# alipay/MMLRec-A-Unified-Multi-Task-and-Multi-Scenario-Learning-Benchmark-for-Recommendation

Hardware: AMD Instinct MI355X
Metric: train-step samples/sec, MMoE AliExpress-shape batch (higher is better)
Workload: dtype f32 (GEMMs: fp32-equivalent emulation on the 16-bit MFMA pipe with f32 accumulate -- two scaled fp16 planes per operand where the operand magnitudes travel with the tensors (batches >= 32 768), else three bf16 planes; max-norm error vs float64 3.3e-7 / 4.7e-7, fp32 MFMA 4.3e-7); 1 GPU; mmoe_ae30: 30 sparse fields, 12.49M rows (1e+07-row top table), E=8, mmoe 4 experts, experts [256, 128], gates [64], towers [64], adam lr 0.005; batch_per_gpu=65536, global_batch=65536, index_dist=zipf, table_update=dense_exact, dense_update_schedule=one launch after the scatter, gradients read for marked rows only, hip_graph=True, scatter_mode=deterministic, streams=1, early_fork=0, tables=single GPU

## Files before the change

include/mmlrec.h:

```cpp
#ifndef MMLREC_H
#define MMLREC_H

#include <stdint.h>

#ifdef __cplusplus
extern "C" {
#endif

#define MML_OK 0
#define MML_ERR_ARG (-1)
#define MML_ERR_HIP (-2)
#define MML_ERR_UNSUPPORTED (-3)

#define MML_MAX_FIELDS 64
#define MML_MAX_GROUP 16
#define MML_MAX_SRC 8
#define MML_MAX_EXPERTS 16
#define MML_MAX_GATES 8
#define MML_MAX_HEADS 8
#define MML_MAX_OPT_TENSORS 32
#define MML_AMAX_WORDS 8
#define MML_MAX_AMAX 64

typedef void* mml_stream_t;
// ... 277 lines not shown
  int64_t ldh, lddh;
  int32_t H;
  int32_t h_relu;
  int32_t n_bias2;
  int32_t mask_col;
  const float* gate;
  float* dgate;
  int64_t ldgate, lddgate;
  int32_t gate_act;
  int32_t kind;
} mml_head_desc;
typedef struct {
  int32_t n_heads;
  int32_t dh_bf16;
  int64_t B;
  float* prob;
  int64_t ldprob;
  const float* y;
  int64_t ldy;
  const float* mask;
  int64_t ldmask;
  float* loss;
  const float* dprob;
  int64_t lddprob;
  mml_head_desc head[MML_MAX_HEADS];
  uint32_t* amax_dH;
  uint32_t* amax_dG;
} mml_head_group;
int64_t mml_head_workspace_bytes(const mml_head_group* grp);
int mml_head_fwd(const mml_head_group* grp, mml_stream_t stream);
int mml_head_bce_fwd_bwd(const mml_head_group* grp, void* workspace, int64_t workspace_bytes, mml_stream_t stream);
int mml_head_bce_fwd_bwd_phase(const mml_head_group* grp, void* workspace, int64_t workspace_bytes, int32_t phase,
                               mml_stream_t stream);
#define MML_ROWS_REDUCE_HEAD 0
#define MML_ROWS_REDUCE_GATE 1
#define MML_ROWS_REDUCE_TOWER_HEAD 2
typedef struct {
  int32_t kind;
  int32_t pad_;
  const void* group;
  void* workspace;
  int64_t workspace_bytes;
} mml_rows_reduce_item;
int mml_rows_reduce_batch(const mml_rows_reduce_item* items, int32_t n, mml_stream_t stream);

typedef struct {
  const float* A;
  int64_t lda;
  const uint32_t* amax_a;
  const uint32_t* w_planes_fwd;
  const uint32_t* w_planes_bwd;
  int64_t ldpf, ldpb;
  const int32_t* kexp_fwd;
  const int32_t* kexp_bwd;
  const float* bias1;
  const float* w;
  const float* hbias;
  const float* hbias2;
  float* dH;
  float* dA;
  int64_t lddh, ldda;
  float* dw;
  float* dhbias;
  uint32_t* amax_dH;
  uint32_t* amax_dA;
  int32_t K, N, n_hbias2;
  int32_t mask_col;
  int32_t head;
  int32_t kind;
} mml_tower_head_desc;
typedef struct {
  int32_t n;
  int32_t pad_;
  int64_t M;
  float* prob;
  int64_t ldprob;
  const float* y;
  int64_t ldy;
  const float* mask;
  int64_t ldmask;
  float* loss;
  mml_tower_head_desc t[MML_MAX_HEADS];
} mml_tower_head_group;
int mml_tower_head_serves(const mml_tower_head_group* grp);
int64_t mml_tower_head_workspace_bytes(const mml_tower_head_group* grp);
int mml_tower_head_fwd_bwd(const mml_tower_head_group* grp, void* workspace, int64_t workspace_bytes, int32_t phase,
                           mml_stream_t stream);


typedef struct {
  const float* src;
  uint16_t* dst;
  int64_t rows, lds, ldd;
  int32_t cols, transpose;
} mml_cast16_desc;
int mml_cast16_batch(const mml_cast16_desc* descs, int32_t n, mml_stream_t stream);
int mml_gather16_fwd(const float* const* tables, const int64_t* vocab, const int32_t* col, int32_t F, int32_t E,
                     const float* X, int64_t ldX, int32_t dense_col0, int32_t Nd, int64_t B, uint16_t* out, int64_t ldo,
                     int32_t* status, mml_stream_t stream);
typedef struct {
  int32_t M, N;
  int32_t n_src;
  int32_t act;
  const uint16_t* A[MML_MAX_SRC];
  const uint16_t* B[MML_MAX_SRC];
  int64_t lda[MML_MAX_SRC], ldb[MML_MAX_SRC];
  int32_t K[MML_MAX_SRC];
  const float* bias;
  void* C;
  int64_t ldc;
  int32_t c_bf16;
  int32_t accumulate;
  uint32_t* mask_out;
  const uint32_t* mask_in;
  int64_t ldmask;
} mml_g16_tn_desc;
int mml_g16_tn(const mml_g16_tn_desc* descs, int32_t n, mml_stream_t stream);
typedef struct {
  const uint16_t* dC;
  const uint16_t* A;
  float* dW;
  float* dbias;
  int64_t lddc, lda, lddw;
  int32_t M, N, K;
  int32_t accumulate;
} mml_g16_wgrad_desc;
int64_t mml_g16_wgrad_workspace_bytes(const mml_g16_wgrad_desc* descs, int32_t n);
int mml_g16_wgrad(const mml_g16_wgrad_desc* descs, int32_t n, void* workspace, int64_t workspace_bytes, int32_t phase,
                  mml_stream_t stream);
const char* mml_g16_last_kernel(void);

int mml_ew_mul(const float* a, const float* b, float* out, int64_t n, mml_stream_t stream);
int mml_ew_mul_bwd(const float* dout, const float* a, const float* b, float* da, float* db, int32_t acc_a,
                   int32_t acc_b, int64_t n, mml_stream_t stream);
int mml_ew_mul_bwd_act(const float* dout, const float* a, const float* b, float* da, float* db, int32_t acc_a,
                       int32_t acc_b, int64_t n, int32_t act_a, int32_t act_b, mml_stream_t stream);
int mml_ew_add_n(const float* const* in, int32_t n_in, float* out, int64_t n, mml_stream_t stream);
#define MML_SUMPROD_TERMS 8
#define MML_SUMPROD_BATCH 16
typedef struct mml_sumprod_desc {
  float* out;
  const float* x[MML_SUMPROD_TERMS];
  const float* y[MML_SUMPROD_TERMS];
  int64_t n;
  int32_t n_terms;
  int32_t accumulate;
  const float* deriv_of;
  int32_t act;
  int32_t pad_;
  uint32_t* amax_out;
} mml_sumprod_desc;
int mml_sumprod_batch(const mml_sumprod_desc* d, int32_t n, mml_stream_t stream);
int mml_dropout(const float* x, int64_t ldx, float* out, int64_t ldo, int64_t rows, int32_t cols, int64_t row0, float p,
                uint64_t seed, uint32_t site, const int32_t* step_dev, int32_t step, int32_t accumulate,
                mml_stream_t stream);
int mml_copy2d(const float* src, int64_t lds, float* dst, int64_t ldd, int64_t rows, int32_t cols, int32_t accumulate,
               mml_stream_t stream);
typedef struct mml_copy2d_desc {
  const float* src;
  int64_t lds;
  float* dst;
  int64_t ldd;
  int64_t rows;
  int32_t cols;
  int32_t accumulate;
  uint32_t* amax_out;
} mml_copy2d_desc;
int mml_copy2d_batch(const mml_copy2d_desc* d, int32_t n, mml_stream_t stream);
int mml_copy_cols(const float* const* src, const int64_t* lds, float* const* dst, const int64_t* ldd,
                  const int32_t* width, int32_t n_seg, int64_t rows, int32_t accumulate, mml_stream_t stream);
int64_t mml_bn_workspace_bytes(int64_t B, int32_t n);
int mml_bn_fwd(const float* z, int64_t ldz, const float* gamma, const float* beta, float* running_mean, float* running_var,
               int64_t* num_batches_tracked, float* mean, float* rstd, float* y, int64_t ldy, int64_t B, int32_t n,
               int32_t act, int32_t training, float eps, float momentum, void* workspace, int64_t workspace_bytes,
               mml_stream_t stream);
int mml_bn_bwd(const float* dy, int64_t lddy, const float* z, int64_t ldz, const float* gamma, const float* mean,
               const float* rstd, float* dz, int64_t lddz, float* dgamma, float* dbeta, int32_t accumulate, int64_t B,
               int32_t n, void* workspace, int64_t workspace_bytes, mml_stream_t stream);
typedef struct mml_prelu_desc {
  const float* z;
  int64_t ldz;
  float* y;
  int64_t ldy;
  int64_t rows;
  int32_t cols;
  int32_t pad_;
  const float* alpha;
  uint32_t* amax_out;
} mml_prelu_desc;
typedef struct mml_prelu_bwd_desc {
  const float* dy;
  int64_t lddy;
  const float* z;
  int64_t ldz;
  float* dz;
  int64_t lddz;
  int64_t rows;
  int32_t cols;
  int32_t pad_;
  const float* alpha;
  float* dalpha;
  int32_t accumulate_dz;
  int32_t accumulate_dalpha;
  uint32_t* amax_out;
} mml_prelu_bwd_desc;
int32_t mml_prelu_max_batch(void);
int mml_prelu_batch_fwd(const mml_prelu_desc* d, int32_t n, mml_stream_t stream);
int64_t mml_prelu_workspace_bytes(int32_t n);
int mml_prelu_batch_bwd(const mml_prelu_bwd_desc* d, int32_t n, void* workspace, int64_t workspace_bytes,
                        mml_stream_t stream);
#define MML_PCGRAD_MAX_TASKS 8
typedef struct mml_pcgrad_seg {
  const float* bank[MML_PCGRAD_MAX_TASKS];
  float* out;
  int64_t rows;
  int64_t ld;
  int32_t cols;
  int32_t pad_;
  const uint8_t* row_marks;
} mml_pcgrad_seg;
int64_t mml_pcgrad_workspace_bytes(const mml_pcgrad_seg* s, int32_t n, int32_t T);
int mml_pcgrad_gram(const mml_pcgrad_seg* s, int32_t n, int32_t T, double* gram, void* workspace,
                    int64_t workspace_bytes, mml_stream_t stream);
int mml_pcgrad_weights(const double* gram, const int32_t* order, int32_t T, float* w, int32_t* fired,
                       mml_stream_t stream);
int mml_pcgrad_combine(const mml_pcgrad_seg* s, int32_t n, int32_t T, const float* w, mml_stream_t stream);
int mml_pcgrad_stash(const mml_pcgrad_seg* s, int32_t n, int32_t clear, mml_stream_t stream);
int mml_domain_bn_update(const float* x, int64_t ldx, const float* mask, int64_t ldm, int64_t B, int32_t n, int32_t D,
                         float* pop_mean, float* pop_var, float decay, mml_stream_t stream);
int mml_domain_bn_eval(const float* x, int64_t ldx, const float* mask, int64_t ldm, const float* pop_mean,
                       const float* pop_var, float* y, int64_t ldy, int64_t B, int32_t n, int32_t D, float eps,
                       mml_stream_t stream);
int mml_snr_gate_weights_fwd(const float* u, const float* alpha, const float* M, float* W, int32_t n_blocks,
                             int64_t block, int32_t zw, float beta, float gamma, float eps, mml_stream_t stream);
int mml_snr_gate_weights_bwd(const float* dW, const float* M, const float* u, const float* alpha, float* du,
                             float* dalpha, int32_t acc_u, int32_t acc_alpha, int32_t n_blocks, int64_t block,
                             int32_t zw, float beta, float gamma, float eps, float* workspace ,
                             mml_stream_t stream);
typedef struct mml_attn2_desc {
  const float* V[2];
  const float* K[2];
  const float* Q[2];
  int64_t ldv[2], ldk[2], ldq[2];
  float* out;
  int64_t ldo;
  float* A;
  const float* dout;
  int64_t lddo;
  float* dV[2];
  float* dK[2];
  float* dQ[2];
  int64_t lddv[2], lddk[2], lddq[2];
  int64_t B;
  int32_t H;
  float sqrt_h;
} mml_attn2_desc;
int mml_attn2_fwd(const mml_attn2_desc* d, mml_stream_t stream);
int mml_attn2_bwd(const mml_attn2_desc* d, mml_stream_t stream);
int mml_esmm_combine(const float* p_raw, int64_t ldr, const float* y, int64_t ldy, const float* d_out, int64_t lddo,
                     float* p_out, int64_t ldo, float* d_raw, int64_t lddr, float* loss, int64_t B, mml_stream_t stream);
int mml_apg_features_fwd(const float* o1, int64_t ldo1, const float* s, int64_t lds, float* z, int64_t ldz, int64_t B,
                         int32_t k, int32_t E, int32_t Kf, mml_stream_t stream);
int mml_apg_features_bwd(const float* dz, int64_t lddz, const float* s, int64_t lds, float* do1, int64_t lddo1,
                         int64_t B, int32_t k, int32_t E, int32_t accumulate, mml_stream_t stream);
int mml_apg_weights(float* Wkk, float* bkk, float* Wb, float* Wcat, int64_t ldw, int32_t k, int32_t E, int32_t dir,
                    int32_t acc_kk, int32_t acc_bkk, int32_t acc_wb, mml_stream_t stream);
int mml_escm_combine(const float* p_raw, int64_t ldr, const float* y, int64_t ldy, const float* d_out, int64_t lddo,
                     float* p_out, int64_t ldo, float* d_raw, int64_t lddr, float* loss, int64_t B, float cf_w,
                     float global_w, mml_stream_t stream);
int mml_auc_segments(const float* pred, int64_t ldp, const float* y, int64_t ldy, int64_t n, int32_t cols, int32_t seg,
                     double* auc, mml_stream_t stream);
int32_t mml_auc_sorted_tile(void);
int64_t mml_auc_sorted_workspace_bytes(int64_t n, int32_t cols, int64_t seg);
int mml_auc_sorted(const float* pred, int64_t ldp, const float* y, int64_t ldy, const float* mask, int64_t ldm,
                   int32_t mask_cols, int64_t n, int32_t cols, int64_t seg, void* workspace, int64_t workspace_bytes,
                   double* auc, int64_t* counts, int32_t* status, mml_stream_t stream);
int mml_act_bwd(const float* y, const float* dy, float* dst, int64_t n, int32_t act, mml_stream_t stream);

typedef struct {
  float* param; const float* grad;
  float* state1;
  float* state2;
  int64_t n;
  float l1, l2;
  const uint32_t* skip_rows;
  int32_t row_elems;
  int32_t zero_grads;
  uint8_t* grad_marks;
  int64_t* acc64;
  const uint32_t* acc_amax;
  int32_t acc_shift;
  int32_t acc_pad_;
  uint8_t* warm_rows;
} mml_opt_tensor;
typedef struct {
  int32_t kind;
  int32_t step;
  const int32_t* step_dev;
  float lr, beta1, beta2, eps, alpha;
  int32_t zero_grad;
  int32_t max_blocks;
  int32_t cold_loop;
} mml_opt_hyper;
int mml_opt_step_dense(const mml_opt_tensor* tensors, int32_t n, const mml_opt_hyper* hyper, mml_stream_t stream);
int mml_opt_step_rows(float* const* tables, float* const* grad_tables, float* const* state1, float* const* state2,
                      uint32_t* const* seen, const int64_t* rowbase, int32_t F, int32_t E,
                      const int32_t* touched, const int32_t* touched_count, int32_t touched_cap,
                      int32_t* const* last ,
                      const mml_opt_hyper* hyper, mml_stream_t stream);
int mml_opt_catchup_rows(float* const* tables, float* const* state1, float* const* state2, int32_t* const* last,
                         const int64_t* rowbase, int32_t F, int32_t E, const int32_t* touched,
                         const int32_t* touched_count, int32_t touched_cap, const mml_opt_hyper* hyper,
                         mml_stream_t stream);
int mml_opt_catchup_dense(float* table, float* state1, float* state2, int32_t* last, int64_t V, int32_t E,
                          const mml_opt_hyper* hyper, mml_stream_t stream);
int mml_counter_update(int32_t* counter, int32_t delta, int32_t reset, mml_stream_t stream);

#ifdef __cplusplus
}
#endif
#endif
```

mmlrec-a-unified-multi-task-and-multi-scenario-learning-benchmark-for-recommendation_amd/_lib.py:

```python
import ctypes as C
import os

import torch

from . import build as _build

MAX_FIELDS, MAX_GROUP, MAX_SRC, MAX_EXPERTS, MAX_GATES, MAX_HEADS, MAX_OPT_TENSORS = 64, 16, 8, 16, 8, 8, 32
OPT_STREAM_MIN_PARAMS, OPT_HUGE_MIN_PARAMS, OPT_STREAM_MAX_TENSORS = 1 << 24, 1 << 22, 4
MAX_POOLED, POOL_MAX_LEN = 16, 256
POOL_COMBINERS = {"sum": 0, "mean": 1, "max": 2}
ACT_NONE, ACT_RELU, ACT_SIGMOID, ACT_SIGMOID2 = 0, 1, 2, 3
HEAD_OUT_SIGMOID, HEAD_OUT_IDENTITY = 0, 1
HEAD_LOSS_BCE, HEAD_LOSS_MSE, HEAD_LOSS_MAE = 0, 1, 2


def head_kind(out=HEAD_OUT_SIGMOID, loss=HEAD_LOSS_BCE):
    return (int(loss) << 8) | int(out)


ERR_ARG = -1
SCATTER_DET_CLEAR_MARKS, SCATTER_DET_AMAX_SUPPLIED, SCATTER_DET_DEFER_TOTALS = 1, 2, 4
OPT_SGD, OPT_ADAM, OPT_ADAGRAD, OPT_RMSPROP = 0, 1, 2, 3
OPT_KINDS = {"sgd": OPT_SGD, "adam": OPT_ADAM, "adagrad": OPT_ADAGRAD, "rmsprop": OPT_RMSPROP}

fp = C.c_void_p
i32, i64 = C.c_int32, C.c_int64


class GemmFwdDesc(C.Structure):
    _fields_ = [("A", fp), ("W", fp), ("bias", fp), ("C", fp), ("lda", i64), ("ldw", i64), ("ldc", i64),
                ("M", i32), ("N", i32), ("K", i32), ("act", i32), ("w_kn", i32), ("pad_", i32),
                ("relu_mask", fp), ("ldmask", i64), ("amax_a", fp), ("amax_w", fp), ("amax_out", fp),
                ("w_planes", fp), ("w_kexp", fp),
                ("mul", fp), ("prod", fp), ("ldmul", i64), ("ldprod", i64), ("amax_prod", fp)]


class PoolDesc(C.Structure):
    _fields_ = [("n_tables", i32), ("E", i32), ("n_single", i32), ("n_pooled", i32),
                ("table", fp * MAX_FIELDS), ("vocab", i64 * MAX_FIELDS), ("s_col", i32 * MAX_FIELDS),
                ("s_table", i32 * MAX_FIELDS), ("p_col0", i32 * MAX_POOLED), ("p_maxlen", i32 * MAX_POOLED),
                ("p_len_col", i32 * MAX_POOLED), ("p_combiner", i32 * MAX_POOLED), ("p_table", i32 * MAX_POOLED)]


class AmaxDesc(C.Structure):
    _fields_ = [("x", fp), ("rows", i64), ("ld", i64), ("cols", i32), ("pad_", i32), ("slot", fp)]


class GemmDgradDesc(C.Structure):
    _fields_ = [("dA", fp), ("Y", fp), ("ldda", i64), ("ldy", i64), ("M", i32), ("K", i32), ("act", i32),
                ("n_src", i32), ("accumulate", i32), ("pad_", i32),
                ("dC", fp * MAX_SRC), ("W", fp * MAX_SRC), ("lddc", i64 * MAX_SRC), ("ldw", i64 * MAX_SRC),
                ("N", i32 * MAX_SRC), ("w_kn", i32 * MAX_SRC), ("relu_mask", fp), ("ldmask", i64),
                ("amax_dc", fp * MAX_SRC), ("amax_w", fp * MAX_SRC), ("amax_out", fp),
                ("w_planes", fp * MAX_SRC), ("w_kexp", fp * MAX_SRC),
                ("gate_h", fp), ("gate_g", fp), ("d_h", fp), ("d_g", fp),
                ("ld_h", i64), ("ld_g", i64), ("ld_dh", i64), ("ld_dg", i64),
                ("act_h", i32), ("act_g", i32), ("acc_h", i32), ("acc_g", i32), ("amax_dh", fp), ("amax_dg", fp)]


class PlanesDesc(C.Structure):
    _fields_ = [("W", fp), ("planes", fp), ("rows", i64), ("ld", i64), ("cols", i32), ("layout", i32),
                ("n_amax", i32), ("pad_", i32), ("amax", fp * MAX_SRC), ("kexp", fp), ("ldp", i64),
                ("W2", fp), ("ld2", i64)]


class GemmWgradDesc(C.Structure):
    _fields_ = [("dC", fp), ("A", fp), ("dW", fp), ("dbias", fp), ("lddc", i64), ("lda", i64), ("lddw", i64),
                ("M", i32), ("N", i32), ("K", i32), ("accumulate", i32), ("w_kn", i32), ("pad_", i32),
                ("amax_dc", fp), ("amax_a", fp)]


class Cast16Desc(C.Structure):
    _fields_ = [("src", fp), ("dst", fp), ("rows", i64), ("lds", i64), ("ldd", i64), ("cols", i32), ("transpose", i32)]


class G16TnDesc(C.Structure):
    _fields_ = [("M", i32), ("N", i32), ("n_src", i32), ("act", i32), ("A", fp * MAX_SRC), ("B", fp * MAX_SRC),
                ("lda", i64 * MAX_SRC), ("ldb", i64 * MAX_SRC), ("K", i32 * MAX_SRC), ("bias", fp), ("C", fp),
                ("ldc", i64), ("c_bf16", i32), ("accumulate", i32), ("mask_out", fp), ("mask_in", fp), ("ldmask", i64)]


class G16WgradDesc(C.Structure):
    _fields_ = [("dC", fp), ("A", fp), ("dW", fp), ("dbias", fp), ("lddc", i64), ("lda", i64), ("lddw", i64),
                ("M", i32), ("N", i32), ("K", i32), ("accumulate", i32)]


G16_MAX_GROUP = 8


class RowsReduceItem(C.Structure):
    _fields_ = [("kind", i32), ("pad_", i32), ("group", fp), ("workspace", fp), ("workspace_bytes", i64)]


ROWS_REDUCE_HEAD, ROWS_REDUCE_GATE, ROWS_REDUCE_TOWER_HEAD = 0, 1, 2
MAX_REDUCE_SEGS = 40
NT_MAX_GROUP = 48
GATE_MIX_BF16, GATE_DE_BF16, GATE_DG_BF16, GATE_E_BF16 = 1, 2, 4, 8


class GateDesc(C.Structure):
    _fields_ = [("G", fp), ("Wg", fp), ("P", fp), ("mix", fp), ("dmix", fp), ("dG", fp), ("dWg", fp),
                ("ldg", i64), ("ldp", i64), ("ldmix", i64), ("lddmix", i64), ("lddg", i64),
                ("Gd", i32), ("ne", i32), ("g_relu", i32), ("active", i32), ("expert", i32 * MAX_EXPERTS)]


class GateGroup(C.Structure):
    _fields_ = [("E", fp * MAX_EXPERTS), ("dE", fp * MAX_EXPERTS), ("lde", i64 * MAX_EXPERTS),
                ("ldde", i64 * MAX_EXPERTS), ("n_experts", i32), ("n_gates", i32), ("H", i32), ("e_relu", i32),
                ("B", i64), ("gate", GateDesc * MAX_GATES), ("amax_mix", fp), ("amax_dE", fp), ("amax_dG", fp),
                ("out_bf16", i32), ("pad_", i32)]


class HeadDesc(C.Structure):
    _fields_ = [("Hin", fp), ("w", fp), ("w2", fp), ("bias", fp), ("bias2", fp), ("dH", fp), ("dw", fp),
                ("dbias", fp), ("ldh", i64), ("lddh", i64), ("H", i32), ("h_relu", i32), ("n_bias2", i32),
                ("mask_col", i32), ("gate", fp), ("dgate", fp), ("ldgate", i64), ("lddgate", i64),
                ("gate_act", i32), ("kind", i32)]


class HeadGroup(C.Structure):
    _fields_ = [("n_heads", i32), ("dh_bf16", i32), ("B", i64), ("prob", fp), ("ldprob", i64), ("y", fp),
                ("ldy", i64), ("mask", fp), ("ldmask", i64), ("loss", fp), ("dprob", fp), ("lddprob", i64),
                ("head", HeadDesc * MAX_HEADS), ("amax_dH", fp), ("amax_dG", fp)]


class TowerHeadDesc(C.Structure):
    _fields_ = [("A", fp), ("lda", i64), ("amax_a", fp), ("w_planes_fwd", fp), ("w_planes_bwd", fp), ("ldpf", i64),
                ("ldpb", i64), ("kexp_fwd", fp), ("kexp_bwd", fp), ("bias1", fp), ("w", fp), ("hbias", fp),
                ("hbias2", fp), ("dH", fp), ("dA", fp), ("lddh", i64), ("ldda", i64), ("dw", fp), ("dhbias", fp),
                ("amax_dH", fp), ("amax_dA", fp), ("K", i32), ("N", i32), ("n_hbias2", i32), ("mask_col", i32),
                ("head", i32), ("kind", i32)]


class TowerHeadGroup(C.Structure):
    _fields_ = [("n", i32), ("pad_", i32), ("M", i64), ("prob", fp), ("ldprob", i64), ("y", fp), ("ldy", i64),
                ("mask", fp), ("ldmask", i64), ("loss", fp), ("t", TowerHeadDesc * MAX_HEADS)]


class OptTensor(C.Structure):
    _fields_ = [("param", fp), ("grad", fp), ("state1", fp), ("state2", fp), ("n", i64), ("l1", C.c_float),
                ("l2", C.c_float), ("skip_rows", fp), ("row_elems", i32), ("zero_grads", i32), ("grad_marks", fp),
                ("acc64", fp), ("acc_amax", fp), ("acc_shift", i32), ("acc_pad_", i32), ("warm_rows", fp)]


class Copy2dDesc(C.Structure):
    _fields_ = [("src", fp), ("lds", i64), ("dst", fp), ("ldd", i64), ("rows", i64), ("cols", i32),
                ("accumulate", i32), ("amax_out", fp)]


class PreluDesc(C.Structure):
    _fields_ = [("z", fp), ("ldz", i64), ("y", fp), ("ldy", i64), ("rows", i64), ("cols", i32), ("pad_", i32),
                ("alpha", fp), ("amax_out", fp)]


class PreluBwdDesc(C.Structure):
    _fields_ = [("dy", fp), ("lddy", i64), ("z", fp), ("ldz", i64), ("dz", fp), ("lddz", i64), ("rows", i64),
                ("cols", i32), ("pad_", i32), ("alpha", fp), ("dalpha", fp), ("accumulate_dz", i32),
                ("accumulate_dalpha", i32), ("amax_out", fp)]


PCGRAD_MAX_TASKS = 8


class PcgradSeg(C.Structure):
    _fields_ = [("bank", fp * PCGRAD_MAX_TASKS), ("out", fp), ("rows", i64), ("ld", i64), ("cols", i32), ("pad_", i32),
                ("row_marks", fp)]


class SumProdDesc(C.Structure):
    _fields_ = [("out", fp), ("x", fp * 8), ("y", fp * 8), ("n", i64), ("n_terms", i32), ("accumulate", i32),
                ("deriv_of", fp), ("act", i32), ("pad_", i32), ("amax_out", fp)]


class Attn2Desc(C.Structure):
    _fields_ = [("V", fp * 2), ("K", fp * 2), ("Q", fp * 2), ("ldv", i64 * 2), ("ldk", i64 * 2), ("ldq", i64 * 2),
                ("out", fp), ("ldo", i64), ("A", fp), ("dout", fp), ("lddo", i64), ("dV", fp * 2), ("dK", fp * 2),
                ("dQ", fp * 2), ("lddv", i64 * 2), ("lddk", i64 * 2), ("lddq", i64 * 2), ("B", i64), ("H", i32),
                ("sqrt_h", C.c_float)]


class OptHyper(C.Structure):
    _fields_ = [("kind", i32), ("step", i32), ("step_dev", fp), ("lr", C.c_float), ("beta1", C.c_float),
                ("beta2", C.c_float), ("eps", C.c_float), ("alpha", C.c_float), ("zero_grad", i32), ("max_blocks", i32),
                ("cold_loop", i32)]


_PP = C.POINTER
_SIGS = {
    "mml_version": (C.c_int, []),
    "mml_last_error": (C.c_char_p, []),
    "mml_device_caps": (C.c_int, [C.c_int, _PP(i64)]),
    "mml_stream_create_cu_range": (C.c_int, [C.c_int, C.c_int, C.c_int, _PP(C.c_void_p)]),
    "mml_stream_destroy": (C.c_int, [C.c_void_p]),
    "mml_gather_fwd": (C.c_int, [_PP(fp), _PP(i64), _PP(i32), i32, i32, fp, i64, i32, i32, i64, fp, i64, fp, fp]),
    "mml_gather_wgmax_len": (i64, [i32, i32, i32, i64]),
    "mml_gather_fwd_wgmax": (C.c_int, [_PP(fp), _PP(i64), _PP(i32), i32, i32, fp, i64, i32, i32, i64, fp, i64, fp, i64, fp, fp]),
    "mml_gather_fwd_mark": (C.c_int, [_PP(fp), _PP(i64), _PP(i32), i32, i32, fp, i64, i32, i32, i64, fp, i64, fp, fp, fp]),
    "mml_rows_compact": (C.c_int, [_PP(fp), _PP(i64), _PP(i64), i32, fp, fp, i32, fp, fp]),
    "mml_gather_fwd_idx32": (C.c_int, [_PP(fp), _PP(i64), i32, i32, fp, i64, fp, i64, i32, i64, fp, i64, fp, fp]),
    "mml_scatter_bwd": (C.c_int, [_PP(fp), _PP(i64), _PP(i32), i32, i32, fp, i64, i64, fp, i64, _PP(fp), _PP(i64),
                                  fp, fp, i32, fp, fp, fp]),
    "mml_scatter_bwd_det": (C.c_int, [_PP(fp), _PP(i64), _PP(i32), i32, i32, fp, i64, i64, fp, i64, _PP(fp), fp, fp, i32,
                                      fp, fp]),
    "mml_scatter_det_shift": (i32, [i64]),
    "mml_scatter_bwd_idx32": (C.c_int, [_PP(fp), _PP(i64), i32, i32, fp, i64, i64, fp, i64, _PP(fp), _PP(i64),
                                        fp, fp, i32, fp, fp, fp]),
    "mml_index_unique_idx32": (C.c_int, [_PP(i64), i32, i32, fp, i64, i64, _PP(fp), _PP(i64), fp, fp, i32, fp, fp, fp]),
    "mml_route_count": (C.c_int, [fp, i64, fp, i64, _PP(i32), _PP(i64), i32, i64, i32, fp, fp, fp]),
    "mml_route_place": (C.c_int, [fp, i64, fp, i64, _PP(i32), _PP(i64), _PP(i64), i32, i64, i32, fp, fp, fp, fp, fp]),
    "mml_rows_permute": (C.c_int, [fp, i64, fp, i32, i32, i64, fp, fp]),
    "mml_route_list_count": (C.c_int, [fp, fp, i32, _PP(i64), _PP(i64), i32, i32, fp, fp]),
    "mml_route_list_place": (C.c_int, [fp, fp, i32, _PP(i64), _PP(i64), _PP(i64), i32, i32, fp, fp, fp, fp]),
    "mml_lookup_slots": (C.c_int, [fp, i64, _PP(i32), _PP(i64), _PP(i64), i32, i64, fp, fp, fp, fp]),
    "mml_rows_clear": (C.c_int, [fp, fp, i32, _PP(i64), _PP(fp), i32, fp]),
    "mml_shard_rows": (C.c_int, [fp, i64, fp, i64, i32, i32, i32, i32, fp]),
    "mml_amax_batch": (C.c_int, [_PP(AmaxDesc), i32, fp]),
    "mml_amax_reset": (C.c_int, [fp, i64, fp]),
    "mml_gemm_planes_cut": (C.c_int, [C.POINTER(PlanesDesc), i32, fp]),
    "mml_gemm_set_mode": (C.c_int, [i32]),
    "mml_gemm_get_mode": (C.c_int, []),
    "mml_gemm_set_panel": (C.c_int, [i32]),
    "mml_gemm_set_ws": (C.c_int, [i32]),
    "mml_gemm_set_nt": (C.c_int, [i32]),
    "mml_gemm_nt_serves": (C.c_int, [_PP(GemmWgradDesc)]),
    "mml_gemm_os_serves": (C.c_int, [_PP(GemmDgradDesc), i32]),
    "mml_tower_head_serves": (C.c_int, [_PP(TowerHeadGroup)]),
    "mml_tower_head_workspace_bytes": (i64, [_PP(TowerHeadGroup)]),
    "mml_tower_head_fwd_bwd": (C.c_int, [_PP(TowerHeadGroup), fp, i64, i32, fp]),
    "mml_gemm_last_kernel": (C.c_char_p, []),
    "mml_gather_last_kernel": (C.c_char_p, []),
    "mml_gemm_set_wgrad_lds_pad": (C.c_int, [i32]),
    "mml_cast16_batch": (C.c_int, [_PP(Cast16Desc), i32, fp]),
    "mml_gather16_fwd": (C.c_int, [_PP(fp), _PP(i64), _PP(i32), i32, i32, fp, i64, i32, i32, i64, fp, i64, fp, fp]),
    "mml_g16_tn": (C.c_int, [_PP(G16TnDesc), i32, fp]),
    "mml_g16_wgrad_workspace_bytes": (i64, [_PP(G16WgradDesc), i32]),
    "mml_g16_wgrad": (C.c_int, [_PP(G16WgradDesc), i32, fp, i64, i32, fp]),
    "mml_g16_last_kernel": (C.c_char_p, []),
    "mml_gemm_grouped_fwd": (C.c_int, [_PP(GemmFwdDesc), i32, fp]),
    "mml_gemm_grouped_dgrad": (C.c_int, [_PP(GemmDgradDesc), i32, fp]),
    "mml_pep_gate_fwd": (C.c_int, [_PP(GemmFwdDesc), i32, fp]),
    "mml_pep_gate_bwd": (C.c_int, [_PP(GemmDgradDesc), i32, fp]),
    "mml_star_linear_fwd": (C.c_int, [_PP(GemmFwdDesc), i32, fp]),
    "mml_star_linear_bwd": (C.c_int, [_PP(GemmDgradDesc), i32, fp]),
    "mml_gemm_grouped_wgrad_workspace_bytes": (i64, [_PP(GemmWgradDesc), i32]),
    "mml_gemm_grouped_wgrad": (C.c_int, [_PP(GemmWgradDesc), i32, fp, i64, fp]),
    "mml_gemm_grouped_wgrad_phase": (C.c_int, [_PP(GemmWgradDesc), i32, fp, i64, i32, fp]),
    "mml_gate_mix_fwd": (C.c_int, [_PP(GateGroup), fp]),
    "mml_gate_mix_bwd_workspace_bytes": (i64, [_PP(GateGroup)]),
    "mml_gate_mix_bwd": (C.c_int, [_PP(GateGroup), fp, i64, fp]),
    "mml_gate_mix_bwd_phase": (C.c_int, [_PP(GateGroup), fp, i64, i32, fp]),
    "mml_head_workspace_bytes": (i64, [_PP(HeadGroup)]),
    "mml_head_fwd": (C.c_int, [_PP(HeadGroup), fp]),
    "mml_head_bce_fwd_bwd": (C.c_int, [_PP(HeadGroup), fp, i64, fp]),
    "mml_head_bce_fwd_bwd_phase": (C.c_int, [_PP(HeadGroup), fp, i64, i32, fp]),
    "mml_rows_reduce_batch": (C.c_int, [_PP(RowsReduceItem), i32, fp]),
    "mml_ew_mul": (C.c_int, [fp, fp, fp, i64, fp]),
    "mml_ew_mul_bwd": (C.c_int, [fp, fp, fp, fp, fp, i32, i32, i64, fp]),
    "mml_ew_mul_bwd_act": (C.c_int, [fp, fp, fp, fp, fp, i32, i32, i64, i32, i32, fp]),
    "mml_ew_add_n": (C.c_int, [_PP(fp), i32, fp, i64, fp]),
    "mml_sumprod_batch": (C.c_int, [_PP(SumProdDesc), i32, fp]),
    "mml_copy2d": (C.c_int, [fp, i64, fp, i64, i64, i32, i32, fp]),
    "mml_dropout": (C.c_int, [fp, i64, fp, i64, i64, i32, i64, C.c_float, C.c_uint64, C.c_uint32, fp, i32, i32, fp]),
    "mml_copy2d_batch": (C.c_int, [_PP(Copy2dDesc), i32, fp]),
    "mml_prelu_max_batch": (i32, []),
    "mml_prelu_batch_fwd": (C.c_int, [_PP(PreluDesc), i32, fp]),
    "mml_prelu_workspace_bytes": (i64, [i32]),
    "mml_prelu_batch_bwd": (C.c_int, [_PP(PreluBwdDesc), i32, fp, i64, fp]),
    "mml_pcgrad_workspace_bytes": (i64, [_PP(PcgradSeg), i32, i32]),
    "mml_pcgrad_gram": (C.c_int, [_PP(PcgradSeg), i32, i32, fp, fp, i64, fp]),
    "mml_pcgrad_weights": (C.c_int, [fp, fp, i32, fp, fp, fp]),
    "mml_pcgrad_combine": (C.c_int, [_PP(PcgradSeg), i32, i32, fp, fp]),
    "mml_pcgrad_stash": (C.c_int, [_PP(PcgradSeg), i32, i32, fp]),
    "mml_auc_segments": (C.c_int, [fp, i64, fp, i64, i64, i32, i32, fp, fp]),
    "mml_auc_sorted_tile": (i32, []),
    "mml_auc_sorted_workspace_bytes": (i64, [i64, i32, i64]),
    "mml_auc_sorted": (C.c_int, [fp, i64, fp, i64, fp, i64, i32, i64, i32, i64, fp, i64, fp, fp, fp, fp]),
    "mml_bn_workspace_bytes": (C.c_int64, [i64, i32]),
    "mml_bn_fwd": (C.c_int, [fp, i64, fp, fp, fp, fp, fp, fp, fp, fp, i64, i64, i32, i32, i32, C.c_float, C.c_float, fp,
                             i64, fp]),
    "mml_bn_bwd": (C.c_int, [fp, i64, fp, i64, fp, fp, fp, fp, i64, fp, fp, i32, i64, i32, fp, i64, fp]),
    "mml_domain_bn_update": (C.c_int, [fp, i64, fp, i64, i64, i32, i32, fp, fp, C.c_float, fp]),
    "mml_domain_bn_eval": (C.c_int, [fp, i64, fp, i64, fp, fp, fp, i64, i64, i32, i32, C.c_float, fp]),
    "mml_snr_gate_weights_fwd": (C.c_int, [fp, fp, fp, fp, i32, i64, i32, C.c_float, C.c_float, C.c_float, fp]),
    "mml_snr_gate_weights_bwd": (C.c_int, [fp, fp, fp, fp, fp, fp, i32, i32, i32, i64, i32, C.c_float, C.c_float,
                                           C.c_float, fp, fp]),
    "mml_attn2_fwd": (C.c_int, [_PP(Attn2Desc), fp]),
    "mml_attn2_bwd": (C.c_int, [_PP(Attn2Desc), fp]),
    "mml_esmm_combine": (C.c_int, [fp, i64, fp, i64, fp, i64, fp, i64, fp, i64, fp, i64, fp]),
    "mml_apg_features_fwd": (C.c_int, [fp, i64, fp, i64, fp, i64, i64, i32, i32, i32, fp]),
    "mml_apg_features_bwd": (C.c_int, [fp, i64, fp, i64, fp, i64, i64, i32, i32, i32, fp]),
    "mml_apg_weights": (C.c_int, [fp, fp, fp, fp, i64, i32, i32, i32, i32, i32, i32, fp]),
    "mml_escm_combine": (C.c_int, [fp, i64, fp, i64, fp, i64, fp, i64, fp, i64, fp, i64, C.c_float, C.c_float, fp]),
    "mml_act_bwd": (C.c_int, [fp, fp, fp, i64, i32, fp]),
    "mml_copy_cols": (C.c_int, [_PP(fp), _PP(i64), _PP(fp), _PP(i64), _PP(i32), i32, i64, i32, fp]),
    "mml_opt_step_dense": (C.c_int, [_PP(OptTensor), i32, _PP(OptHyper), fp]),
    "mml_opt_step_rows": (C.c_int, [_PP(fp), _PP(fp), _PP(fp), _PP(fp), _PP(fp), _PP(i64), i32, i32, fp, fp, i32,
                                    _PP(fp), _PP(OptHyper), fp]),
    "mml_opt_catchup_rows": (C.c_int, [_PP(fp), _PP(fp), _PP(fp), _PP(fp), _PP(i64), i32, i32, fp, fp, i32,
                                       _PP(OptHyper), fp]),
    "mml_opt_catchup_dense": (C.c_int, [fp, fp, fp, fp, i64, i32, _PP(OptHyper), fp]),
    "mml_index_unique": (C.c_int, [_PP(i64), _PP(i32), i32, i32, fp, i64, i64, _PP(fp), _PP(i64), fp, fp, i32, fp, fp,
                                   fp]),
    "mml_counter_update": (C.c_int, [fp, i32, i32, fp]),
    "mml_gather_pool_wgmax_len": (i64, [_PP(PoolDesc), i32, i64]),
    "mml_gather_pool_fwd": (C.c_int, [_PP(PoolDesc), fp, i64, i32, i32, i64, fp, i64, fp, i64, fp, i64, fp, fp]),
    "mml_scatter_pool_bwd": (C.c_int, [_PP(PoolDesc), fp, i64, i64, fp, i64, fp, i64, _PP(fp), _PP(i64), fp, fp, i32,
                                       fp, fp, fp]),
    "mml_index_unique_pool": (C.c_int, [_PP(PoolDesc), fp, i64, i64, _PP(fp), _PP(i64), fp, fp, i32, fp, fp, fp]),
}
EXPORTS = tuple(_SIGS)

_lib = None


class MMLError(RuntimeError):
    pass


def library_path():
    return _build.LIBPATH


def load():
    global _lib
    if _lib is not None:
        return _lib
    path = os.environ.get("MMLREC_LIB") or _build.LIBPATH
    if path == _build.LIBPATH and (not os.path.exists(path) or _build.needs_build()) and os.path.exists(_build.HIPCC):
        _build.build_library(verbose=False)
    if not os.path.exists(path):
        raise MMLError(f"HIP extension {path} is missing and cannot be built (no hipcc): the MI355X path has no "
                       "CPU fallback")
    lib = C.CDLL(path)
    for name, (res, args) in _SIGS.items():
        fn = getattr(lib, name)
        fn.restype = res
        fn.argtypes = args
    _lib = lib
    return lib


def check(rc, what=""):
    if rc != 0:
        msg = load().mml_last_error()
        raise MMLError(f"{what} failed with code {rc}: {msg.decode() if msg else ''}")


def ptr(t):
    return None if t is None else t.data_ptr()


def opt_dense_streams(numel, ntensors, all_marked):
    return numel >= OPT_STREAM_MIN_PARAMS and (ntensors <= OPT_STREAM_MAX_TENSORS or all_marked)


def opt_takes_det_totals(numels, all_marked, split=False):
    return (all_marked and not split and len(numels) <= MAX_OPT_TENSORS and
            opt_dense_streams(sum(numels), len(numels), True))
```

mmlrec-a-unified-multi-task-and-multi-scenario-learning-benchmark-for-recommendation_amd/csrc/optim_ew.hip:

```cpp
#include "common.hpp"
#include "fold_fixed.hpp"

#include <stdlib.h>

#ifndef MML_OPT_COLD_CB
#define MML_OPT_COLD_CB 8
#endif

namespace mml {

struct OptLaunch {
  mml_opt_tensor t[MML_MAX_OPT_TENSORS];
  int32_t n;
  int32_t variant;
  mml_opt_hyper h;
  int64_t chunk0[MML_MAX_OPT_TENSORS + 1];
  int32_t blk0[MML_MAX_OPT_TENSORS + 1];
  int32_t prop;
};
static_assert(sizeof(OptLaunch) <= 4096, "OptLaunch travels by value: the kernel-argument block holds 4 KB");

struct StepConsts {
  float step_size;
  float inv_bc2s;
};

__device__ __forceinline__ StepConsts step_consts(const mml_opt_hyper& h) {
  __shared__ StepConsts sc;
  if (threadIdx.x == 0) {
    StepConsts c{h.lr, 1.f};
    if (h.kind == MML_OPT_ADAM) {
      const int t = h.step_dev ? *h.step_dev : h.step;
      const double bc1 = 1.0 - pow((double)h.beta1, (double)t);
      const double bc2 = 1.0 - pow((double)h.beta2, (double)t);
      c.step_size = (float)((double)h.lr / bc1);
      c.inv_bc2s = (float)(1.0 / sqrt(bc2));
    }
    sc = c;
  }
  __syncthreads();
  return sc;
}

__device__ __forceinline__ void opt_update(const mml_opt_hyper& h, const StepConsts& c, float& p, float g, float& s1,
                                           float& s2) {
  switch (h.kind) {
    case MML_OPT_SGD:
      p -= h.lr * g;
      break;
    case MML_OPT_ADAM: {
      s1 = s1 + (1.f - h.beta1) * (g - s1);
      s2 = h.beta2 * s2 + (1.f - h.beta2) * g * g;
      const float denom = sqrtf(s2) * c.inv_bc2s + h.eps;
      p -= c.step_size * (s1 / denom);
      break;
    }
    case MML_OPT_ADAGRAD:
      s1 += g * g;
      p -= h.lr * (g / (sqrtf(s1) + h.eps));
      break;
    case MML_OPT_RMSPROP:
      s1 = h.alpha * s1 + (1.f - h.alpha) * g * g;
      p -= h.lr * (g / (sqrtf(s1) + h.eps));
      break;
  }
}

__device__ __forceinline__ float reg_grad(float g, float p, float l1, float l2) {
  if (l2 != 0.f) g += (2.f * l2) * p;
  if (l1 != 0.f) g += l1 * (p > 0.f ? 1.f : (p < 0.f ? -1.f : 0.f));
  return g;
}

enum { OPT_PLAIN = 0, OPT_UNROLL2 = 1, OPT_SKIP_U = 2, OPT_MARK_U = 3, OPT_MARK_ACC_U = 4 };
template <bool STREAM, int PATH, int U>
__global__ __launch_bounds__(256) void opt_dense_kernel(const OptLaunch L) {
  int ti = blockIdx.y, nblk = gridDim.x, lblk = blockIdx.x;
  if (L.prop) {
    ti = 0;
    while (ti + 1 < L.n && (int)blockIdx.x >= L.blk0[ti + 1]) ++ti;
    nblk = L.blk0[ti + 1] - L.blk0[ti];
    lblk = (int)blockIdx.x - L.blk0[ti];
  }
  const mml_opt_tensor& T = L.t[ti];
  const mml_opt_hyper& h = L.h;
  const StepConsts c = step_consts(h);
  const int64_t n4 = T.n >> 2;
  const bool vec = aligned16(T.param) && aligned16(T.grad) && (!T.state1 || aligned16(T.state1)) &&
                   (!T.state2 || aligned16(T.state2));
  const int64_t stride = (int64_t)nblk * blockDim.x;
  const int64_t tid = (int64_t)lblk * blockDim.x + threadIdx.x;
  float* gw = const_cast<float*>(T.grad);
  const bool reg = T.l1 != 0.f || T.l2 != 0.f;
  if (vec) {
    typedef float f4 __attribute__((ext_vector_type(4)));
    const bool nt = (L.variant & 1) != 0;
    f4* P = reinterpret_cast<f4*>(T.param);
    f4* G = reinterpret_cast<f4*>(gw);
    f4* S1 = reinterpret_cast<f4*>(T.state1);
    f4* S2 = reinterpret_cast<f4*>(T.state2);
    const f4 zero = {0.f, 0.f, 0.f, 0.f};
    auto ld = [&](const f4* q) { return nt ? __builtin_nontemporal_load(q) : *q; };
    auto st = [&](f4* q, const f4& v) {
      if (nt) __builtin_nontemporal_store(v, q);
      else *q = v;
    };
    auto one = [&](f4& p, const f4& g, f4& a, f4& b) {
#pragma unroll
      for (int e = 0; e < 4; ++e) {
        float pe = p[e], ae = a[e], be = b[e];
        opt_update(h, c, pe, reg ? reg_grad(g[e], pe, T.l1, T.l2) : g[e], ae, be);
        p[e] = pe;
        a[e] = ae;
        b[e] = be;
      }
    };
    const uint32_t* skip = T.skip_rows;
    const int re = T.row_elems > 0 ? T.row_elems : 1;
    const int rsh = (re & (re - 1)) == 0 ? __builtin_ctz((unsigned)re) : -1;
    auto row_of = [&](int64_t c) { return rsh >= 0 ? ((c << 2) >> rsh) : ((c << 2) / re); };
    auto skipped = [&](int64_t c) {
      const int64_t row = row_of(c);
      return (skip[row >> 5] >> (row & 31)) & 1u;
    };
    const bool zg = T.zero_grads != 0;
    uint8_t* const gm = T.grad_marks;
    typedef long long l2 __attribute__((ext_vector_type(2)));
    l2* const A64 = PATH == OPT_MARK_ACC_U ? reinterpret_cast<l2*>(T.acc64) : nullptr;
    const l2 lzero = {0, 0};
    int emax = 1;
    if (PATH == OPT_MARK_ACC_U && A64) {
      uint32_t m = 0;
      for (int w = 0; w < MML_AMAX_WORDS; ++w) m = T.acc_amax[w] > m ? T.acc_amax[w] : m;
      emax = (int)(m >> 23);
      emax = emax < 1 ? 1 : (emax > 254 ? 254 : emax);
    }
    auto add_totals = [&](f4& g, const l2& t0, const l2& t1, int64_t c) {
      if (t0.x) g.x += from_fixed(t0.x, emax, T.acc_shift);
      if (t0.y) g.y += from_fixed(t0.y, emax, T.acc_shift);
      if (t1.x) g.z += from_fixed(t1.x, emax, T.acc_shift);
      if (t1.y) g.w += from_fixed(t1.y, emax, T.acc_shift);
      if (t0.x | t0.y) A64[2 * c] = lzero;
      if (t1.x | t1.y) A64[2 * c + 1] = lzero;
    };
    int64_t i = tid;
    if (PATH == OPT_UNROLL2 && !skip && !gm) {
      for (; i + stride < n4; i += 2 * stride) {
        const int64_t j = i + stride;
        f4 p0 = ld(P + i), p1 = ld(P + j);
        const f4 g0 = ld(G + i), g1 = ld(G + j);
        f4 a0 = S1 ? ld(S1 + i) : zero, a1 = S1 ? ld(S1 + j) : zero;
        f4 b0 = S2 ? ld(S2 + i) : zero, b1 = S2 ? ld(S2 + j) : zero;
        one(p0, g0, a0, b0);
        one(p1, g1, a1, b1);
        st(P + i, p0);
        st(P + j, p1);
        if (S1) { st(S1 + i, a0); st(S1 + j, a1); }
        if (S2) { st(S2 + i, b0); st(S2 + j, b1); }
        if (h.zero_grad && (g0.x != 0.f || g0.y != 0.f || g0.z != 0.f || g0.w != 0.f)) G[i] = zero;
        if (h.zero_grad && (g1.x != 0.f || g1.y != 0.f || g1.z != 0.f || g1.w != 0.f)) G[j] = zero;
      }
    }
    if (PATH == OPT_SKIP_U && skip) {
      for (; i + (U - 1) * stride < n4; i += U * stride) {
        f4 p[U], a[U], b[U];
        uint32_t w[U];
#pragma unroll
        for (int k = 0; k < U; ++k) {
          const int64_t row = row_of(i + k * stride);
          w[k] = (skip[row >> 5] >> (row & 31)) & 1u;
        }
#pragma unroll
        for (int k = 0; k < U; ++k) {
          const int64_t j = i + k * stride;
          if (!w[k]) {
            p[k] = ld(P + j);
            a[k] = S1 ? ld(S1 + j) : zero;
            b[k] = S2 ? ld(S2 + j) : zero;
          }
        }
#pragma unroll
        for (int k = 0; k < U; ++k) {
          if (w[k]) continue;
          const int64_t j = i + k * stride;
          const f4 g = zg ? zero : ld(G + j);
          one(p[k], g, a[k], b[k]);
          st(P + j, p[k]);
          if (S1) st(S1 + j, a[k]);
          if (S2) st(S2 + j, b[k]);
          if (h.zero_grad && (g.x != 0.f || g.y != 0.f || g.z != 0.f || g.w != 0.f)) G[j] = zero;
        }
      }
    }
    uint8_t* const wr = gm ? T.warm_rows : nullptr;
    const bool compact = !(L.variant & 8) && wr &&
                         ((reinterpret_cast<uintptr_t>(gm) | reinterpret_cast<uintptr_t>(wr)) & 3) == 0;
    if ((PATH == OPT_MARK_U || PATH == OPT_MARK_ACC_U) && compact && !skip) {
      constexpr int RPL = 4, SPAN = 64 * RPL;
      constexpr int DENSE_PCT = 15;
      constexpr int WAVES = 4;
      __shared__ uint16_t live_rows[WAVES][SPAN];
      const int lane = threadIdx.x & 63;
      const int wv = __builtin_amdgcn_readfirstlane((int)(threadIdx.x >> 6));
      uint16_t* const lst = live_rows[wv];
      const int csh = rsh - 2;
      const int64_t rows = T.n >> rsh;
      const int64_t nspan = (rows + SPAN - 1) / SPAN, nwv = (int64_t)nblk * WAVES;
      auto nz80 = [](uint32_t x) { return (x | ((x & 0x7f7f7f7fu) + 0x7f7f7f7fu)) & 0x80808080u; };
      auto pack4 = [](uint32_t t) { return ((t >> 7) & 1u) | ((t >> 14) & 2u) | ((t >> 21) & 4u) | ((t >> 28) & 8u); };
      auto scan = [&](int64_t s, uint32_t& mk, uint32_t& wk) {
        const int64_t r0 = s * SPAN + lane * RPL;
        mk = wk = 0u;
        if (r0 + RPL <= rows) {
          mk = *reinterpret_cast<const uint32_t*>(gm + r0);
          wk = *reinterpret_cast<const uint32_t*>(wr + r0);
        } else {
#pragma unroll
          for (int k = 0; k < RPL; ++k)
            if (r0 + k < rows) {
              mk |= (uint32_t)gm[r0 + k] << (8 * k);
              wk |= (uint32_t)wr[r0 + k] << (8 * k);
            }
        }
      };
      int64_t s = (int64_t)lblk * WAVES + wv;
      uint32_t mk = 0, wk = 0;
      if (s < nspan) scan(s, mk, wk);
      for (; s < nspan; s += nwv) {
        uint32_t mkn = 0, wkn = 0;
        if (s + nwv < nspan) scan(s + nwv, mkn, wkn);
        const uint32_t lm = pack4(nz80(mk)), wm = pack4(nz80(wk));
        const uint32_t act = lm | wm;
        if (__builtin_amdgcn_ballot_w64(act != 0) != 0) {
          const int64_t row0 = s * SPAN;
          const uint32_t cnt = (uint32_t)__builtin_popcount(act);
          uint32_t pre = 0;
          int nlive = 0;
#pragma unroll
          for (int bit = 0; (1 << bit) <= RPL; ++bit) {
            const uint64_t bal = __builtin_amdgcn_ballot_w64(((cnt >> bit) & 1u) != 0);
            pre += __builtin_amdgcn_mbcnt_hi((uint32_t)(bal >> 32), __builtin_amdgcn_mbcnt_lo((uint32_t)bal, 0u)) << bit;
            nlive += __builtin_popcountll(bal) << bit;
          }
          const bool dense = nlive * 100 >= SPAN * DENSE_PCT;
          if (!dense) {
            __builtin_amdgcn_fence(__ATOMIC_RELEASE, "wavefront");
            __builtin_amdgcn_wave_barrier();
#pragma unroll
            for (int k = 0; k < RPL; ++k)
              if ((act >> k) & 1u)
                lst[pre++] = (uint16_t)((lane * RPL + k) | (((lm >> k) & 1u) << 14) | (((wm >> k) & 1u) << 15));
            __builtin_amdgcn_fence(__ATOMIC_RELEASE, "wavefront");
            __builtin_amdgcn_wave_barrier();
          }
          if (lm) {
            const int64_t r0 = row0 + lane * RPL;
            if (r0 + RPL <= rows) {
              *reinterpret_cast<uint32_t*>(gm + r0) = 0u;
              const uint32_t set = (nz80(mk) & ~nz80(wk)) >> 7;
              if (set) *reinterpret_cast<uint32_t*>(wr + r0) = wk | set;
            } else {
#pragma unroll
              for (int k = 0; k < RPL; ++k)
                if ((lm >> k) & 1u) {
                  gm[r0 + k] = 0;
                  if (!((wm >> k) & 1u)) wr[r0 + k] = 1;
                }
            }
          }
          const int items = (dense ? SPAN : nlive) << csh;
#pragma unroll 1
          for (int b0 = 0; b0 < items; b0 += 128) {
            f4 p[2], a[2], b[2], g[2];
            l2 t0[2], t1[2];
            int64_t jj[2];
            bool on[2], lv[2];
#pragma unroll
            for (int k = 0; k < 2; ++k) {
              const int it = b0 + 64 * k + lane;
              const int ent = it >> csh;
              on[k] = it < items;
              uint32_t e;
              if (dense) {
                const uint32_t src = (uint32_t)__shfl((int)(lm | (act << 16)), (ent / RPL) & 63);
                on[k] = on[k] && ((src >> (16 + (ent & (RPL - 1)))) & 1u);
                e = (uint32_t)ent | (((src >> (ent & (RPL - 1))) & 1u) << 14);
              } else {
                e = on[k] ? lst[ent] : 0u;
              }
              lv[k] = on[k] && ((e >> 14) & 1u);
              const int64_t j = ((row0 + (int64_t)(e & 0x3fffu)) << csh) | (int64_t)(it & ((1 << csh) - 1));
              jj[k] = j;
              p[k] = a[k] = b[k] = g[k] = zero;
              t0[k] = t1[k] = lzero;
              if (on[k]) {
                p[k] = ld(P + j);
                if (S1) a[k] = ld(S1 + j);
                if (S2) b[k] = ld(S2 + j);
              }
              if (lv[k]) {
                if (!zg) g[k] = ld(G + j);
                if (PATH == OPT_MARK_ACC_U && A64) {
                  t0[k] = A64[2 * j];
                  t1[k] = A64[2 * j + 1];
                }
              }
            }
#pragma unroll
            for (int k = 0; k < 2; ++k) {
              if (!on[k]) continue;
              const int64_t j = jj[k];
              f4 gs = g[k];
              if (PATH == OPT_MARK_ACC_U && A64 && lv[k]) add_totals(gs, t0[k], t1[k], j);
              one(p[k], gs, a[k], b[k]);
              st(P + j, p[k]);
              if (S1) st(S1 + j, a[k]);
              if (S2) st(S2 + j, b[k]);
              if (h.zero_grad && (g[k].x != 0.f || g[k].y != 0.f || g[k].z != 0.f || g[k].w != 0.f)) G[j] = zero;
            }
          }
        }
        mk = mkn;
        wk = wkn;
      }
      i = n4;
    }
    if ((PATH == OPT_MARK_U || PATH == OPT_MARK_ACC_U) && wr && !skip && !compact) {
      constexpr int CB = MML_OPT_COLD_CB;
      for (; i < n4; i += CB * stride) {
        uint32_t lm = 0, wm = 0;
#pragma unroll
        for (int k = 0; k < CB; ++k) {
          const int64_t j = i + k * stride;
          const bool in = j < n4;
          const int64_t row = row_of(in ? j : i);
          const uint8_t mk = gm[row], wk = wr[row];
          lm |= (uint32_t)(in && mk != 0) << k;
          wm |= (uint32_t)(in && wk != 0) << k;
        }
        const uint32_t act = lm | wm;
        if (__builtin_amdgcn_ballot_w64(act != 0) == 0) continue;
#pragma unroll 1
        for (int kk = 0; kk < CB; kk += 2) {
          if (__builtin_amdgcn_ballot_w64(((act >> kk) & 3u) != 0) == 0) continue;
          f4 p[2], a[2], b[2], g[2];
          l2 t0[2], t1[2];
#pragma unroll
          for (int k = 0; k < 2; ++k) {
            const int64_t j = i + (kk + k) * stride;
            const bool on = (act >> (kk + k)) & 1u, lv = (lm >> (kk + k)) & 1u;
            p[k] = a[k] = b[k] = g[k] = zero;
            t0[k] = t1[k] = lzero;
            if (on) {
              p[k] = ld(P + j);
              if (S1) a[k] = ld(S1 + j);
              if (S2) b[k] = ld(S2 + j);
            }
            if (lv) {
              if (!zg) g[k] = ld(G + j);
              if (PATH == OPT_MARK_ACC_U && A64) {
                t0[k] = A64[2 * j];
                t1[k] = A64[2 * j + 1];
              }
            }
          }
#pragma unroll
          for (int k = 0; k < 2; ++k) {
            const int64_t j = i + (kk + k) * stride;
            const bool on = (act >> (kk + k)) & 1u, lv = (lm >> (kk + k)) & 1u;
            if (!on) continue;
            f4 gs = g[k];
            if (PATH == OPT_MARK_ACC_U && A64 && lv) add_totals(gs, t0[k], t1[k], j);
            one(p[k], gs, a[k], b[k]);
            st(P + j, p[k]);
            if (S1) st(S1 + j, a[k]);
            if (S2) st(S2 + j, b[k]);
            if (h.zero_grad && (g[k].x != 0.f || g[k].y != 0.f || g[k].z != 0.f || g[k].w != 0.f)) G[j] = zero;
            const int64_t row = row_of(j);
            if (lv && (j << 2) == row * re) {
              gm[row] = 0;
              if (!((wm >> (kk + k)) & 1u)) wr[row] = 1;
            }
          }
        }
      }
    }
    if (PATH == OPT_MARK_U && gm && !skip) {
      for (; i + (U - 1) * stride < n4; i += U * stride) {
        f4 p[U], a[U], b[U], g[U];
        bool lv[U];
        int64_t rw[U];
#pragma unroll
        for (int k = 0; k < U; ++k) {
          rw[k] = row_of(i + k * stride);
          lv[k] = gm[rw[k]] != 0;
        }
#pragma unroll
        for (int k = 0; k < U; ++k) {
          const int64_t j = i + k * stride;
          p[k] = ld(P + j);
          a[k] = S1 ? ld(S1 + j) : zero;
          b[k] = S2 ? ld(S2 + j) : zero;
          g[k] = (zg || !lv[k]) ? zero : ld(G + j);
        }
#pragma unroll
        for (int k = 0; k < U; ++k) {
          const int64_t j = i + k * stride;
          one(p[k], g[k], a[k], b[k]);
          st(P + j, p[k]);
          if (S1) st(S1 + j, a[k]);
          if (S2) st(S2 + j, b[k]);
          if (h.zero_grad && (g[k].x != 0.f || g[k].y != 0.f || g[k].z != 0.f || g[k].w != 0.f)) G[j] = zero;
          if (lv[k] && (j << 2) == rw[k] * re) gm[rw[k]] = 0;
        }
      }
    }
    if (PATH == OPT_MARK_ACC_U && gm && !skip) {
      for (; i + (U - 1) * stride < n4; i += U * stride) {
        f4 p[U], a[U], b[U], g[U];
        l2 t0[U], t1[U];
        bool lv[U];
        int64_t rw[U];
#pragma unroll
        for (int k = 0; k < U; ++k) {
          rw[k] = row_of(i + k * stride);
          lv[k] = gm[rw[k]] != 0;
        }
#pragma unroll
        for (int k = 0; k < U; ++k) {
          const int64_t j = i + k * stride;
          p[k] = ld(P + j);
          a[k] = S1 ? ld(S1 + j) : zero;
          b[k] = S2 ? ld(S2 + j) : zero;
          g[k] = (zg || !lv[k]) ? zero : ld(G + j);
          t0[k] = (A64 && lv[k]) ? A64[2 * j] : lzero;
          t1[k] = (A64 && lv[k]) ? A64[2 * j + 1] : lzero;
        }
#pragma unroll
        for (int k = 0; k < U; ++k) {
          const int64_t j = i + k * stride;
          f4 gs = g[k];
          if (A64 && lv[k]) add_totals(gs, t0[k], t1[k], j);
          one(p[k], gs, a[k], b[k]);
          st(P + j, p[k]);
          if (S1) st(S1 + j, a[k]);
          if (S2) st(S2 + j, b[k]);
          if (h.zero_grad && (g[k].x != 0.f || g[k].y != 0.f || g[k].z != 0.f || g[k].w != 0.f)) G[j] = zero;
          if (lv[k] && (j << 2) == rw[k] * re) gm[rw[k]] = 0;
        }
      }
    }
    for (; i < n4; i += stride) {
      if (skip && skipped(i)) continue;
      bool live = true, warm = true;
      int64_t row = 0;
      if (gm) {
        row = row_of(i);
        live = gm[row] != 0;
        if (wr) {
          warm = wr[row] != 0;
          if (!live && !warm) continue;
        }
      }
      f4 p = ld(P + i);
      const f4 g = (zg || !live) ? zero : ld(G + i);
      f4 a = S1 ? ld(S1 + i) : zero;
      f4 b = S2 ? ld(S2 + i) : zero;
      if (PATH == OPT_MARK_ACC_U) {
        f4 gs = g;
        if (A64 && gm && live) add_totals(gs, A64[2 * i], A64[2 * i + 1], i);
        one(p, gs, a, b);
      } else {
        one(p, g, a, b);
      }
      st(P + i, p);
      if (S1) st(S1 + i, a);
      if (S2) st(S2 + i, b);
      if (h.zero_grad && (g.x != 0.f || g.y != 0.f || g.z != 0.f || g.w != 0.f)) G[i] = zero;
      if (gm && live && (i << 2) == row * re) {
        gm[row] = 0;
        if (!warm) wr[row] = 1;
      }
    }
  }
  const int64_t tail0 = vec ? (n4 << 2) : 0;
  for (int64_t i = tail0 + tid; i < T.n; i += stride) {
    if (T.skip_rows) {
      const int64_t row = i / (T.row_elems > 0 ? T.row_elems : 1);
      if ((T.skip_rows[row >> 5] >> (row & 31)) & 1u) continue;
    }
    float p = T.param[i], a = T.state1 ? T.state1[i] : 0.f, b = T.state2 ? T.state2[i] : 0.f;
    opt_update(h, c, p, reg_grad(T.zero_grads ? 0.f : T.grad[i], p, T.l1, T.l2), a, b);
    T.param[i] = p;
    if (T.state1) T.state1[i] = a;
    if (T.state2) T.state2[i] = b;
    if (h.zero_grad && T.grad[i] != 0.f) gw[i] = 0.f;
  }
}

__global__ __launch_bounds__(256) void opt_flat_kernel(const OptLaunch L) {
  __shared__ mml_opt_tensor ts[MML_MAX_OPT_TENSORS];
  __shared__ int64_t pre[MML_MAX_OPT_TENSORS + 1];
  for (int i = threadIdx.x; i < L.n; i += 256) ts[i] = L.t[i];
  for (int i = threadIdx.x; i <= L.n; i += 256) pre[i] = L.chunk0[i];
  const mml_opt_hyper& h = L.h;
  const StepConsts c = step_consts(h);
  const int64_t total = pre[L.n];
  const int64_t stride = (int64_t)gridDim.x * blockDim.x;
  for (int64_t ch = (int64_t)blockIdx.x * blockDim.x + threadIdx.x; ch < total; ch += stride) {
    int lo = 0, hi = L.n;
    while (hi - lo > 1) {
      const int mid = (lo + hi) >> 1;
      if (pre[mid] <= ch) lo = mid;
      else hi = mid;
    }
    const mml_opt_tensor T = ts[lo];
    const int64_t e0 = (ch - pre[lo]) << 2;
    float* gw = const_cast<float*>(T.grad);
    const int re = T.row_elems > 0 ? T.row_elems : 1;
    if (T.skip_rows && re % 4 == 0) {
      const int64_t row = e0 / re;
      if ((T.skip_rows[row >> 5] >> (row & 31)) & 1u) continue;
    }
    const bool vec = (e0 + 4 <= T.n) && aligned16(T.param) && aligned16(T.grad) && (!T.state1 || aligned16(T.state1)) &&
                     (!T.state2 || aligned16(T.state2));
    if (vec) {
      float4 p = *reinterpret_cast<float4*>(T.param + e0);
      const float4 g = T.zero_grads ? make_float4(0, 0, 0, 0) : *reinterpret_cast<const float4*>(T.grad + e0);
      float4 a = T.state1 ? *reinterpret_cast<float4*>(T.state1 + e0) : make_float4(0, 0, 0, 0);
      float4 b = T.state2 ? *reinterpret_cast<float4*>(T.state2 + e0) : make_float4(0, 0, 0, 0);
      opt_update(h, c, p.x, reg_grad(g.x, p.x, T.l1, T.l2), a.x, b.x);
      opt_update(h, c, p.y, reg_grad(g.y, p.y, T.l1, T.l2), a.y, b.y);
      opt_update(h, c, p.z, reg_grad(g.z, p.z, T.l1, T.l2), a.z, b.z);
      opt_update(h, c, p.w, reg_grad(g.w, p.w, T.l1, T.l2), a.w, b.w);
      *reinterpret_cast<float4*>(T.param + e0) = p;
      if (T.state1) *reinterpret_cast<float4*>(T.state1 + e0) = a;
      if (T.state2) *reinterpret_cast<float4*>(T.state2 + e0) = b;
      if (h.zero_grad && (g.x != 0.f || g.y != 0.f || g.z != 0.f || g.w != 0.f))
        *reinterpret_cast<float4*>(gw + e0) = make_float4(0, 0, 0, 0);
    } else {
      for (int64_t i = e0; i < e0 + 4 && i < T.n; ++i) {
        if (T.skip_rows) {
          const int64_t row = i / re;
          if ((T.skip_rows[row >> 5] >> (row & 31)) & 1u) continue;
        }
        float p = T.param[i], a = T.state1 ? T.state1[i] : 0.f, b = T.state2 ? T.state2[i] : 0.f;
        const float g = T.zero_grads ? 0.f : T.grad[i];
        opt_update(h, c, p, reg_grad(g, p, T.l1, T.l2), a, b);
        T.param[i] = p;
        if (T.state1) T.state1[i] = a;
        if (T.state2) T.state2[i] = b;
        if (h.zero_grad && g != 0.f) gw[i] = 0.f;
      }
    }
  }
}

struct RowsLaunch {
  float* tab[MML_MAX_FIELDS];
  float* grad[MML_MAX_FIELDS];
  float* s1[MML_MAX_FIELDS];
  float* s2[MML_MAX_FIELDS];
  uint32_t* seen[MML_MAX_FIELDS];
  int64_t rowbase[MML_MAX_FIELDS + 1];
  int32_t F, E;
  int32_t* last[MML_MAX_FIELDS];
  const int32_t* touched;
  const int32_t* touched_count;
  int32_t cap;
  int32_t pad_;
  mml_opt_hyper h;
};

__device__ __forceinline__ int field_of_row(const int64_t* rb_lds, int F, int64_t grow) {
  int lo = 0, hi = F;
  while (hi - lo > 1) {
    const int mid = (lo + hi) >> 1;
    if (rb_lds[mid] <= grow) lo = mid;
    else hi = mid;
  }
  return lo;
}

template <int VEC>
__global__ __launch_bounds__(256) void opt_rows_kernel(const RowsLaunch L) {
  const mml_opt_hyper& h = L.h;
  __shared__ int64_t rb_lds[MML_MAX_FIELDS + 1];
  __shared__ float* tab_l[MML_MAX_FIELDS];
  __shared__ float* grad_l[MML_MAX_FIELDS];
  __shared__ float* s1_l[MML_MAX_FIELDS];
  __shared__ float* s2_l[MML_MAX_FIELDS];
  __shared__ uint32_t* seen_l[MML_MAX_FIELDS];
  __shared__ int32_t* last_l[MML_MAX_FIELDS];
  for (int i = threadIdx.x; i <= L.F; i += 256) rb_lds[i] = L.rowbase[i];
  for (int i = threadIdx.x; i < L.F; i += 256) {
    tab_l[i] = L.tab[i]; grad_l[i] = L.grad[i]; s1_l[i] = L.s1[i]; s2_l[i] = L.s2[i]; seen_l[i] = L.seen[i];
    last_l[i] = L.last[i];
  }
  const StepConsts c = step_consts(h);
  int32_t cnt = *L.touched_count;
  if (cnt > L.cap) cnt = L.cap;
  const int per_row = L.E / VEC;
  const int64_t total = (int64_t)cnt * per_row;
  const int64_t stride = (int64_t)gridDim.x * blockDim.x;
  for (int64_t item = (int64_t)blockIdx.x * blockDim.x + threadIdx.x; item < total; item += stride) {
    const int32_t li = (int32_t)(item / per_row);
    const int e = (int)(item - (int64_t)li * per_row) * VEC;
    const int64_t grow = L.touched[li];
    const int f = field_of_row(rb_lds, L.F, grow);
    const int64_t row = grow - rb_lds[f];
    const int64_t o = row * L.E + e;
    float* const T_ = tab_l[f];
    float* const G_ = grad_l[f];
    float* const S1 = s1_l[f];
    float* const S2 = s2_l[f];
    float p[VEC], g[VEC], a[VEC], b[VEC];
    if (VEC == 4) {
      *reinterpret_cast<float4*>(p) = *reinterpret_cast<const float4*>(T_ + o);
      *reinterpret_cast<float4*>(g) = *reinterpret_cast<const float4*>(G_ + o);
      if (S1) *reinterpret_cast<float4*>(a) = *reinterpret_cast<const float4*>(S1 + o);
      if (S2) *reinterpret_cast<float4*>(b) = *reinterpret_cast<const float4*>(S2 + o);
    } else {
      p[0] = T_[o];
      g[0] = G_[o];
      if (S1) a[0] = S1[o];
      if (S2) b[0] = S2[o];
    }
#pragma unroll
    for (int k = 0; k < VEC; ++k) {
      if (!S1) a[k] = 0.f;
      if (!S2) b[k] = 0.f;
      opt_update(h, c, p[k], g[k], a[k], b[k]);
    }
    if (VEC == 4) {
      *reinterpret_cast<float4*>(T_ + o) = *reinterpret_cast<float4*>(p);
      if (S1) *reinterpret_cast<float4*>(S1 + o) = *reinterpret_cast<float4*>(a);
      if (S2) *reinterpret_cast<float4*>(S2 + o) = *reinterpret_cast<float4*>(b);
      *reinterpret_cast<float4*>(G_ + o) = make_float4(0.f, 0.f, 0.f, 0.f);
    } else {
      T_[o] = p[0];
      if (S1) S1[o] = a[0];
      if (S2) S2[o] = b[0];
      G_[o] = 0.f;
    }
    if (e == 0) {
      atomicAnd(seen_l[f] + (row >> 5), ~(1u << (row & 31)));
      if (last_l[f]) last_l[f][row] = h.step_dev ? *h.step_dev : h.step;
    }
  }
}

__device__ __forceinline__ void catchup_element(const mml_opt_hyper& h, int from, int to, float& p, float& m, float& v) {
  if (to <= from) return;
  if (h.kind == MML_OPT_ADAM) {
    if (m == 0.f) {
      v *= powf(h.beta2, (float)(to - from));
      return;
    }
    float b1p = powf(h.beta1, (float)from), b2p = powf(h.beta2, (float)from);
    int j = from;
    while (j < to) {
      ++j;
      b1p *= h.beta1;
      b2p *= h.beta2;
      StepConsts c;
      c.step_size = h.lr / (1.f - b1p);
      c.inv_bc2s = rsqrtf(1.f - b2p);
      const float before = p;
      opt_update(h, c, p, 0.f, m, v);
      if (p == before && j - from > 16) {
        const float rem = (float)(to - j);
        m *= powf(h.beta1, rem);
        v *= powf(h.beta2, rem);
        return;
      }
    }
  } else if (h.kind == MML_OPT_RMSPROP) {
    m *= powf(h.alpha, (float)(to - from));
  }
}

struct CatchupLaunch {
  float* tab[MML_MAX_FIELDS];
  float* s1[MML_MAX_FIELDS];
  float* s2[MML_MAX_FIELDS];
  int32_t* last[MML_MAX_FIELDS];
  int64_t rowbase[MML_MAX_FIELDS + 1];
  int32_t F, E;
  const int32_t* touched;
  const int32_t* touched_count;
  int32_t cap;
  int32_t dense;
  int64_t V;
  mml_opt_hyper h;
};

__global__ __launch_bounds__(256) void opt_catchup_kernel(const CatchupLaunch L) {
  __shared__ int64_t rb_lds[MML_MAX_FIELDS + 1];
  if (!L.dense) {
    for (int i = threadIdx.x; i <= L.F; i += 256) rb_lds[i] = L.rowbase[i];
    __syncthreads();
  }
  const mml_opt_hyper& h = L.h;
  const int target = (h.step_dev ? *h.step_dev : h.step) - (L.dense ? 0 : 1);
  int64_t nrows;
  if (L.dense) {
    nrows = L.V;
  } else {
    int32_t cnt = *L.touched_count;
    nrows = cnt > L.cap ? L.cap : cnt;
  }
  const int64_t total = nrows * L.E;
  const int64_t stride = (int64_t)gridDim.x * blockDim.x;
  for (int64_t item = (int64_t)blockIdx.x * blockDim.x + threadIdx.x; item < total; item += stride) {
    const int64_t li = item / L.E;
    const int e = (int)(item - li * L.E);
    int f = 0;
    int64_t row = li;
    if (!L.dense) {
      const int64_t grow = L.touched[li];
      f = field_of_row(rb_lds, L.F, grow);
      row = grow - rb_lds[f];
    }
    const int from = L.last[f][row];
    if (from >= target) continue;
    const int64_t o = row * L.E + e;
    float p = L.tab[f][o];
    float m = L.s1[f] ? L.s1[f][o] : 0.f, v = L.s2[f] ? L.s2[f][o] : 0.f;
    catchup_element(h, from, target, p, m, v);
    L.tab[f][o] = p;
    if (L.s1[f]) L.s1[f][o] = m;
    if (L.s2[f]) L.s2[f][o] = v;
    __builtin_amdgcn_wave_barrier();
    if (e == 0) L.last[f][row] = target;
  }
}

__global__ void counter_kernel(int32_t* c, int32_t delta, int32_t reset) {
  if (threadIdx.x == 0 && blockIdx.x == 0) *c = reset ? 0 : (*c + delta);
}

__global__ __launch_bounds__(256) void ew_mul_kernel(const float* a, const float* b, float* out, int64_t n) {
  const int64_t stride = (int64_t)gridDim.x * blockDim.x;
  for (int64_t i = (int64_t)blockIdx.x * blockDim.x + threadIdx.x; i < n; i += stride) out[i] = a[i] * b[i];
}

__device__ __forceinline__ float act_deriv_from_output(float y, int act) {
  if (act == MML_ACT_RELU) return y > 0.f ? 1.f : 0.f;
  if (act == MML_ACT_SIGMOID) return y * (1.f - y);
  if (act == MML_ACT_SIGMOID2) return y * (1.f - 0.5f * y);
  return 1.f;
}
__global__ __launch_bounds__(256) void ew_mul_bwd_kernel(const float* dout, const float* a, const float* b, float* da,
                                                         float* db, int acc_a, int acc_b, int64_t n, int act_a,
                                                         int act_b) {
  const int64_t stride = (int64_t)gridDim.x * blockDim.x;
  for (int64_t i = (int64_t)blockIdx.x * blockDim.x + threadIdx.x; i < n; i += stride) {
    const float d = dout[i];
    const float av = (db || act_a) ? a[i] : 0.f;
    const float bv = (da || act_b) ? b[i] : 0.f;
    if (da) {
      const float v = d * bv * act_deriv_from_output(av, act_a);
      da[i] = acc_a ? da[i] + v : v;
    }
    if (db) {
      const float v = d * av * act_deriv_from_output(bv, act_b);
      db[i] = acc_b ? db[i] + v : v;
    }
  }
}

struct AddN {
  const float* in[16];
  int32_t n_in;
};
__global__ __launch_bounds__(256) void ew_add_n_kernel(const AddN A, float* out, int64_t n) {
  const int64_t stride = (int64_t)gridDim.x * blockDim.x;
  for (int64_t i = (int64_t)blockIdx.x * blockDim.x + threadIdx.x; i < n; i += stride) {
    float s = 0.f;
    for (int k = 0; k < A.n_in; ++k) s += A.in[k][i];
    out[i] = s;
  }
}

struct SumProdBatch {
  mml_sumprod_desc d[MML_SUMPROD_BATCH];
};
__global__ __launch_bounds__(256) void sumprod_batch_kernel(const SumProdBatch Bt) {
  const mml_sumprod_desc& D = Bt.d[blockIdx.y];
  const int64_t stride = (int64_t)gridDim.x * blockDim.x;
  const int64_t tid = (int64_t)blockIdx.x * blockDim.x + threadIdx.x;
  bool vec = (D.n & 3) == 0 && aligned16(D.out) && (!D.deriv_of || aligned16(D.deriv_of));
  for (int k = 0; k < D.n_terms; ++k) vec = vec && aligned16(D.x[k]) && (!D.y[k] || aligned16(D.y[k]));
  float am = 0.f;
  if (vec) {
    const int64_t n4 = D.n >> 2;
    for (int64_t i = tid; i < n4; i += stride) {
      float4 s = D.accumulate ? reinterpret_cast<const float4*>(D.out)[i] : make_float4(0.f, 0.f, 0.f, 0.f);
      for (int k = 0; k < D.n_terms; ++k) {
        const float4 x = reinterpret_cast<const float4*>(D.x[k])[i];
        if (D.y[k]) {
          const float4 y = reinterpret_cast<const float4*>(D.y[k])[i];
          s.x += x.x * y.x; s.y += x.y * y.y; s.z += x.z * y.z; s.w += x.w * y.w;
        } else {
          s.x += x.x; s.y += x.y; s.z += x.z; s.w += x.w;
        }
      }
      if (D.act != MML_ACT_NONE) {
        const float4 o = reinterpret_cast<const float4*>(D.deriv_of)[i];
        s.x *= act_deriv_from_output(o.x, D.act); s.y *= act_deriv_from_output(o.y, D.act);
        s.z *= act_deriv_from_output(o.z, D.act); s.w *= act_deriv_from_output(o.w, D.act);
      }
      reinterpret_cast<float4*>(D.out)[i] = s;
      amax_acc(am, s);
    }
    amax_flush(am, D.amax_out);
    return;
  }
  for (int64_t i = tid; i < D.n; i += stride) {
    float s = D.accumulate ? D.out[i] : 0.f;
    for (int k = 0; k < D.n_terms; ++k) s += D.x[k][i] * (D.y[k] ? D.y[k][i] : 1.f);
    if (D.act != MML_ACT_NONE) s *= act_deriv_from_output(D.deriv_of[i], D.act);
    D.out[i] = s;
    amax_acc(am, s);
  }
  amax_flush(am, D.amax_out);
}

__global__ __launch_bounds__(256) void copy2d_kernel(const float* src, int64_t lds_, float* dst, int64_t ldd, int64_t rows,
                                                     int cols, int accumulate) {
  const int64_t total = rows * cols;
  const int64_t stride = (int64_t)gridDim.x * blockDim.x;
  for (int64_t i = (int64_t)blockIdx.x * blockDim.x + threadIdx.x; i < total; i += stride) {
    const int64_t r = i / cols;
    const int c = (int)(i - r * cols);
    const float v = src[r * lds_ + c];
    float* d = dst + r * ldd + c;
    *d = accumulate ? *d + v : v;
  }
}

constexpr int COPY2D_BATCH = 32;
struct Copy2dBatch {
  mml_copy2d_desc d[COPY2D_BATCH];
};
__global__ __launch_bounds__(256) void copy2d_batch_kernel(const Copy2dBatch Bt) {
  const mml_copy2d_desc& D = Bt.d[blockIdx.y];
  const int nb = D.amax_out ? ((int)gridDim.x < 256 ? (int)gridDim.x : 256) : (int)gridDim.x;
  const bool mine = (int)blockIdx.x < nb;
  float amf = 0.f;
  if (mine) {
    const int64_t stride = (int64_t)nb * 256;
    const int64_t tid = (int64_t)blockIdx.x * 256 + threadIdx.x;
    const bool vec = D.cols % 4 == 0 && D.lds % 4 == 0 && D.ldd % 4 == 0 && aligned16(D.src) && aligned16(D.dst);
    if (vec) {
      const int c4 = D.cols >> 2;
      const int64_t total = D.rows * c4;
      const bool small = total < 0x7fffffff;
      auto off = [&](int64_t i, int64_t& so, int64_t& dof) __attribute__((always_inline)) {
        const int64_t r = small ? (int64_t)((uint32_t)i / (uint32_t)c4) : i / c4;
        const int64_t c = (i - r * c4) << 2;
        so = r * D.lds + c;
        dof = r * D.ldd + c;
      };
      auto fin = [&](float4 v, int64_t dof) __attribute__((always_inline)) {
        float4* q = reinterpret_cast<float4*>(D.dst + dof);
        if (D.accumulate) {
          const float4 o = *q;
          v.x += o.x; v.y += o.y; v.z += o.z; v.w += o.w;
        }
        *q = v;
        amax_acc(amf, v);
      };
      int64_t i = tid;
      for (; i + 3 * stride < total; i += 4 * stride) {
        int64_t s0, s1, s2, s3, d0, d1, d2, d3;
        off(i, s0, d0); off(i + stride, s1, d1); off(i + 2 * stride, s2, d2); off(i + 3 * stride, s3, d3);
        const float4 v0 = *reinterpret_cast<const float4*>(D.src + s0), v1 = *reinterpret_cast<const float4*>(D.src + s1);
        const float4 v2 = *reinterpret_cast<const float4*>(D.src + s2), v3 = *reinterpret_cast<const float4*>(D.src + s3);
        fin(v0, d0); fin(v1, d1); fin(v2, d2); fin(v3, d3);
      }
      for (; i < total; i += stride) {
        int64_t s0, d0;
        off(i, s0, d0);
        fin(*reinterpret_cast<const float4*>(D.src + s0), d0);
      }
    } else {
      const int64_t total = D.rows * D.cols;
      for (int64_t i = tid; i < total; i += stride) {
        const int64_t r = i / D.cols;
        const int c = (int)(i - r * D.cols);
        float v = D.src[r * D.lds + c];
        float* q = D.dst + r * D.ldd + c;
        if (D.accumulate) v += *q;
        *q = v;
        amax_acc(amf, v);
      }
    }
  }
  amax_flush<true>(amf, mine ? D.amax_out : nullptr);
}

struct ColSegs {
  const float* src[MML_MAX_FIELDS];
  float* dst[MML_MAX_FIELDS];
  int64_t lds_[MML_MAX_FIELDS], ldd[MML_MAX_FIELDS];
  int32_t width[MML_MAX_FIELDS];
  int32_t start[MML_MAX_FIELDS + 1];
  int32_t n;
};
__global__ __launch_bounds__(256) void copy_cols_kernel(const ColSegs S, int64_t rows, int accumulate) {
  const int W = S.start[S.n];
  const int64_t total = rows * W;
  const int64_t stride = (int64_t)gridDim.x * blockDim.x;
  for (int64_t i = (int64_t)blockIdx.x * blockDim.x + threadIdx.x; i < total; i += stride) {
    const int64_t r = i / W;
    const int c = (int)(i - r * W);
    int s = 0;
    while (c >= S.start[s + 1]) ++s;
    const int cc = c - S.start[s];
    const float v = S.src[s][r * S.lds_[s] + cc];
    float* d = S.dst[s] + r * S.ldd[s] + cc;
    *d = accumulate ? *d + v : v;
  }
}

constexpr int COPY_COLS_MAX_W4 = 1024;
__global__ __launch_bounds__(256) void copy_cols_vec4_kernel(const ColSegs S, int64_t rows, int accumulate) {
  typedef float f4 __attribute__((ext_vector_type(4)));
  __shared__ const float* s_src[MML_MAX_FIELDS];
  __shared__ float* s_dst[MML_MAX_FIELDS];
  __shared__ int64_t s_lds[MML_MAX_FIELDS], s_ldd[MML_MAX_FIELDS];
  __shared__ int32_t s_start[MML_MAX_FIELDS + 1];
  __shared__ uint8_t seg_of[COPY_COLS_MAX_W4];
  const int W4 = S.start[S.n] >> 2;
  for (int k = threadIdx.x; k < S.n; k += 256) {
    s_src[k] = S.src[k]; s_dst[k] = S.dst[k]; s_lds[k] = S.lds_[k]; s_ldd[k] = S.ldd[k];
  }
  for (int k = threadIdx.x; k <= S.n; k += 256) s_start[k] = S.start[k];
  __syncthreads();
  for (int c = threadIdx.x; c < W4; c += 256) {
    int lo = 0, hi = S.n - 1;
    while (lo < hi) {
      const int mid = (lo + hi + 1) >> 1;
      if (s_start[mid] <= 4 * c) lo = mid; else hi = mid - 1;
    }
    seg_of[c] = (uint8_t)lo;
  }
  __syncthreads();
  const int64_t total = rows * W4;
  const int64_t stride = (int64_t)gridDim.x * blockDim.x;
  for (int64_t i = (int64_t)blockIdx.x * blockDim.x + threadIdx.x; i < total; i += stride) {
    int64_t r;
    int c;
    if (total < 0x7fffffff) {
      const uint32_t ri = (uint32_t)i / (uint32_t)W4;
      r = ri;
      c = (int)((uint32_t)i - ri * (uint32_t)W4);
    } else {
      r = i / W4;
      c = (int)(i - r * W4);
    }
    const int sg = seg_of[c];
    const int cc = 4 * c - s_start[sg];
    const f4 v = *reinterpret_cast<const f4*>(s_src[sg] + r * s_lds[sg] + cc);
    f4* d = reinterpret_cast<f4*>(s_dst[sg] + r * s_ldd[sg] + cc);
    *d = accumulate ? *d + v : v;
  }
}

__global__ __launch_bounds__(256) void act_bwd_kernel(const float* y, const float* dy, float* dst, int64_t n, int act) {
  const int64_t stride = (int64_t)gridDim.x * blockDim.x;
  for (int64_t i = (int64_t)blockIdx.x * blockDim.x + threadIdx.x; i < n; i += stride) {
    const float v = y[i];
    float d = 1.f;
    if (act == MML_ACT_RELU) d = v > 0.f ? 1.f : 0.f;
    else if (act == MML_ACT_SIGMOID) d = v * (1.f - v);
    else if (act == MML_ACT_SIGMOID2) d = v * (1.f - 0.5f * v);
    dst[i] = d * dy[i];
  }
}

static unsigned ew_grid(int64_t n) {
  int64_t b = cdiv(n, 256);
  if (b > 256 * 8) b = 256 * 8;
  if (b < 1) b = 1;
  return (unsigned)b;
}

}

using namespace mml;

static int check_hyper(const mml_opt_hyper* h, const char* who) {
  MML_REQUIRE(h, "%s: null hyper", who);
  MML_REQUIRE(h->kind >= MML_OPT_SGD && h->kind <= MML_OPT_RMSPROP, "%s: unknown optimizer kind %d", who, h->kind);
  MML_REQUIRE(h->kind != MML_OPT_ADAM || h->step_dev || h->step >= 1, "%s: Adam needs step >= 1", who);
  return MML_OK;
}

extern "C" int mml_opt_step_dense(const mml_opt_tensor* tensors, int32_t n, const mml_opt_hyper* hyper,
                                  mml_stream_t stream) {
  int rc = check_hyper(hyper, "mml_opt_step_dense");
  if (rc) return rc;
  MML_REQUIRE(n >= 0 && (n == 0 || tensors), "mml_opt_step_dense: bad tensor array");
  int i = 0;
  while (i < n) {
    OptLaunch L{};
    L.h = *hyper;
    int64_t total = 0, chunks = 0;
    while (i < n && L.n < MML_MAX_OPT_TENSORS) {
      const mml_opt_tensor& t = tensors[i];
      MML_REQUIRE(t.param && t.grad && t.n >= 0, "mml_opt_step_dense: tensor %d malformed", i);
      MML_REQUIRE(hyper->kind == MML_OPT_SGD || t.state1, "mml_opt_step_dense: tensor %d needs state1", i);
      MML_REQUIRE(hyper->kind != MML_OPT_ADAM || t.state2, "mml_opt_step_dense: tensor %d needs state2 (Adam)", i);
      MML_REQUIRE(!t.skip_rows || (t.row_elems > 0 && t.row_elems % 4 == 0 && t.n % t.row_elems == 0 &&
                                   aligned16(t.param)),
                  "mml_opt_step_dense: tensor %d: skip_rows needs row_elems %% 4 == 0 dividing n and a 16-byte aligned "
                  "parameter (16-byte chunks must lie inside one row)", i);
      if (t.acc64) {
        MML_REQUIRE(t.grad_marks && !t.skip_rows && t.acc_amax && aligned16(t.acc64) && t.acc_shift >= 4 &&
                        t.acc_shift <= 28,
                    "mml_opt_step_dense: tensor %d: acc64 (deferred totals of mml_scatter_bwd_det) needs grad_marks, no "
                    "skip_rows, a 16-byte aligned int64 array, acc_amax and acc_shift = mml_scatter_det_shift(B)", i);
      }
      if (t.grad_marks) {
        const int cpr = t.row_elems / 4;
        MML_REQUIRE(t.row_elems > 0 && t.row_elems % 4 == 0 && cpr <= 64 && (cpr & (cpr - 1)) == 0 &&
                        t.n % t.row_elems == 0 && !t.skip_rows && aligned16(t.param) && aligned16(t.grad) &&
                        (!t.state1 || aligned16(t.state1)) && (!t.state2 || aligned16(t.state2)),
                    "mml_opt_step_dense: tensor %d: grad_marks needs 16-byte aligned [rows, row_elems] tensors with "
                    "row_elems / 4 a power of two <= 64 and no skip_rows", i);
      }
      if (t.warm_rows) {
        MML_REQUIRE(t.grad_marks && t.l1 == 0.f && t.l2 == 0.f,
                    "mml_opt_step_dense: tensor %d: warm_rows needs grad_marks and no regulariser (a regulariser moves a "
                    "row whose moments and gradient are zero)", i);
      }
      L.chunk0[L.n] = chunks;
      L.t[L.n++] = t;
      total += t.n;
      chunks += cdiv(t.n, 4);
      ++i;
    }
    L.chunk0[L.n] = chunks;
    if (total == 0) continue;
    static int variant = -1;
    if (variant < 0) {
      const char* e = getenv("MMLREC_OPT_VARIANT");
      variant = e ? atoi(e) : 0;
    }
    L.variant = variant | (hyper->max_blocks > 0 ? 4 : 0) | (hyper->cold_loop == 1 ? 8 : 0);
    int64_t nmax = 0;
    for (int k = 0; k < L.n; ++k) nmax = L.t[k].n > nmax ? L.t[k].n : nmax;
    bool all_gm = true, all_skip = true, none = true, any_acc = false;
    for (int k = 0; k < L.n; ++k) {
      any_acc = any_acc || L.t[k].acc64;
      all_gm = all_gm && L.t[k].grad_marks && !L.t[k].skip_rows;
      all_skip = all_skip && L.t[k].skip_rows;
      none = none && !L.t[k].grad_marks && !L.t[k].skip_rows;
    }
    const bool many = L.n > 4 && all_gm;
    MML_REQUIRE(!any_acc || all_gm, "mml_opt_step_dense: a launch with acc64 tensors takes grad_marks on every tensor");
    if (total >= ((int64_t)1 << 24) && (L.n <= 4 || many)) {
      int64_t bx = cdiv(cdiv(nmax, 4), 256);
      if (bx > 256 * 8) bx = 256 * 8;
      if (hyper->max_blocks > 0 && bx * L.n > hyper->max_blocks) bx = cdiv(hyper->max_blocks, L.n);
      dim3 grid((unsigned)bx, (unsigned)L.n);
      bool all_warm = true;
      for (int k = 0; k < L.n; ++k) all_warm = all_warm && L.t[k].warm_rows;
      static int cold_wgs = -1;
      if (cold_wgs < 0) {
        const char* e = getenv("MMLREC_OPT_COLD_WGS");
        cold_wgs = e ? atoi(e) : 256 * 8;
        if (cold_wgs < 1 || cold_wgs > 256 * 8) cold_wgs = 256 * 8;
      }
      const int64_t wg_cap = all_warm ? cold_wgs : 256 * 8;
      if (many) {
        int64_t want = 0;
        for (int k = 0; k < L.n; ++k) {
          const int64_t need = cdiv(cdiv(L.t[k].n, 4), 256);
          want += need > wg_cap ? wg_cap : (need < 1 ? 1 : need);
        }
        const bool capped = hyper->max_blocks > 0 && want > hyper->max_blocks;
        int64_t tb = capped ? hyper->max_blocks : want;
        if (tb < L.n) tb = L.n;
        int64_t at = 0;
        for (int k = 0; k < L.n; ++k) {
          L.blk0[k] = (int32_t)at;
          const int64_t need = cdiv(cdiv(L.t[k].n, 4), 256);
          int64_t nb = capped ? tb * L.t[k].n / total : (need > wg_cap ? wg_cap : need);
          if (nb > need) nb = need;
          if (nb < 1) nb = 1;
          at += nb;
        }
        L.blk0[L.n] = (int32_t)at;
        L.prop = 1;
        grid = dim3((unsigned)at, 1);
      }
      static int u_mark = -1;
      if (u_mark < 0) {
        const char* e = getenv("MMLREC_OPT_U");
        u_mark = e ? atoi(e) : 2;
      }
      hipStream_t st = to_stream(stream);
      if (any_acc) {
        if (u_mark == 4) MML_LAUNCH((opt_dense_kernel<true, OPT_MARK_ACC_U, 4>), grid, dim3(256), 0, st, L);
        else MML_LAUNCH((opt_dense_kernel<true, OPT_MARK_ACC_U, 2>), grid, dim3(256), 0, st, L);
      } else if ((L.variant & 4) && all_gm) {
        if (u_mark == 4) MML_LAUNCH((opt_dense_kernel<true, OPT_MARK_U, 4>), grid, dim3(256), 0, st, L);
        else if (u_mark == 8) MML_LAUNCH((opt_dense_kernel<true, OPT_MARK_U, 8>), grid, dim3(256), 0, st, L);
        else MML_LAUNCH((opt_dense_kernel<true, OPT_MARK_U, 2>), grid, dim3(256), 0, st, L);
      } else if ((L.variant & 4) && all_skip) {
        MML_LAUNCH((opt_dense_kernel<true, OPT_SKIP_U, 4>), grid, dim3(256), 0, st, L);
      } else if ((L.variant & 2) && none) {
        MML_LAUNCH((opt_dense_kernel<true, OPT_UNROLL2, 1>), grid, dim3(256), 0, st, L);
      } else {
        MML_LAUNCH((opt_dense_kernel<true, OPT_PLAIN, 1>), grid, dim3(256), 0, st, L);
      }
    } else {
      for (int k = 0; k < L.n; ++k)
        MML_REQUIRE(!L.t[k].grad_marks, "mml_opt_step_dense: grad_marks (and acc64) is only honoured by the streaming "
                    "launch (>= 2^24 parameters in <= 4 tensors, or any number of marked tensors)");
      int64_t bx = cdiv(chunks, 256);
      if (bx > 256 * 8) bx = 256 * 8;
      if (hyper->max_blocks > 0 && bx > hyper->max_blocks) bx = hyper->max_blocks;
      MML_LAUNCH(opt_flat_kernel, dim3((unsigned)bx), dim3(256), 0, to_stream(stream), L);
    }
    rc = check_launch("mml_opt_step_dense");
    if (rc) return rc;
  }
  return MML_OK;
}

static int launch_catchup(CatchupLaunch& L, int64_t max_items, hipStream_t st, const char* who) {
  int64_t blocks = cdiv(max_items, 256);
  if (blocks > 256 * 8) blocks = 256 * 8;
  if (blocks < 1) blocks = 1;
  MML_LAUNCH(opt_catchup_kernel, dim3((unsigned)blocks), dim3(256), 0, st, L);
  return check_launch(who);
}

extern "C" int mml_opt_catchup_rows(float* const* tables, float* const* state1, float* const* state2,
                                    int32_t* const* last, const int64_t* rowbase, int32_t F, int32_t E,
                                    const int32_t* touched, const int32_t* touched_count, int32_t touched_cap,
                                    const mml_opt_hyper* hyper, mml_stream_t stream) {
  int rc = check_hyper(hyper, "mml_opt_catchup_rows");
  if (rc) return rc;
  MML_REQUIRE(F >= 1 && F <= MML_MAX_FIELDS && E > 0 && tables && last && rowbase && touched && touched_count &&
                  touched_cap > 0, "mml_opt_catchup_rows: bad arguments");
  if (hyper->kind == MML_OPT_SGD || hyper->kind == MML_OPT_ADAGRAD) return MML_OK;
  CatchupLaunch L{};
  for (int f = 0; f < F; ++f) {
    MML_REQUIRE(tables[f] && last[f] && state1 && state1[f], "mml_opt_catchup_rows: field %d null", f);
    MML_REQUIRE(hyper->kind != MML_OPT_ADAM || (state2 && state2[f]), "mml_opt_catchup_rows: field %d needs state2", f);
    L.tab[f] = tables[f]; L.s1[f] = state1[f]; L.s2[f] = state2 ? state2[f] : nullptr; L.last[f] = last[f];
    L.rowbase[f] = rowbase[f];
  }
  L.rowbase[F] = rowbase[F];
  L.F = F; L.E = E; L.touched = touched; L.touched_count = touched_count; L.cap = touched_cap; L.h = *hyper;
  return launch_catchup(L, (int64_t)touched_cap * E, to_stream(stream), "mml_opt_catchup_rows");
}

extern "C" int mml_opt_catchup_dense(float* table, float* state1, float* state2, int32_t* last, int64_t V, int32_t E,
                                     const mml_opt_hyper* hyper, mml_stream_t stream) {
  int rc = check_hyper(hyper, "mml_opt_catchup_dense");
  if (rc) return rc;
  MML_REQUIRE(table && last && V >= 0 && E > 0, "mml_opt_catchup_dense: bad arguments");
  if (V == 0 || hyper->kind == MML_OPT_SGD || hyper->kind == MML_OPT_ADAGRAD) return MML_OK;
  MML_REQUIRE(state1 && (hyper->kind != MML_OPT_ADAM || state2), "mml_opt_catchup_dense: optimizer state missing");
  CatchupLaunch L{};
  L.tab[0] = table; L.s1[0] = state1; L.s2[0] = state2; L.last[0] = last;
  L.F = 1; L.E = E; L.dense = 1; L.V = V; L.h = *hyper;
  return launch_catchup(L, V * E, to_stream(stream), "mml_opt_catchup_dense");
}

extern "C" int mml_opt_step_rows(float* const* tables, float* const* grad_tables, float* const* state1,
                                 float* const* state2, uint32_t* const* seen, const int64_t* rowbase, int32_t F,
                                 int32_t E, const int32_t* touched, const int32_t* touched_count, int32_t touched_cap,
                                 int32_t* const* last, const mml_opt_hyper* hyper, mml_stream_t stream) {
  int rc = check_hyper(hyper, "mml_opt_step_rows");
  if (rc) return rc;
  MML_REQUIRE(F >= 1 && F <= MML_MAX_FIELDS && E > 0, "mml_opt_step_rows: bad F/E");
  MML_REQUIRE(tables && grad_tables && seen && rowbase && touched && touched_count && touched_cap > 0,
              "mml_opt_step_rows: null argument");
  RowsLaunch L{};
  for (int f = 0; f < F; ++f) {
    MML_REQUIRE(tables[f] && grad_tables[f] && seen[f], "mml_opt_step_rows: field %d null", f);
    L.tab[f] = tables[f]; L.grad[f] = grad_tables[f]; L.seen[f] = seen[f];
    L.s1[f] = state1 ? state1[f] : nullptr;
    L.s2[f] = state2 ? state2[f] : nullptr;
    MML_REQUIRE(hyper->kind == MML_OPT_SGD || L.s1[f], "mml_opt_step_rows: field %d needs state1", f);
    MML_REQUIRE(hyper->kind != MML_OPT_ADAM || L.s2[f], "mml_opt_step_rows: field %d needs state2", f);
    L.rowbase[f] = rowbase[f];
    L.last[f] = last ? last[f] : nullptr;
  }
  L.rowbase[F] = rowbase[F];
  L.F = F; L.E = E; L.touched = touched; L.touched_count = touched_count; L.cap = touched_cap; L.h = *hyper;
  bool vec = (E % 4 == 0);
  for (int f = 0; f < F && vec; ++f)
    vec = aligned16(L.tab[f]) && aligned16(L.grad[f]) && (!L.s1[f] || aligned16(L.s1[f])) && (!L.s2[f] || aligned16(L.s2[f]));
  int64_t blocks = cdiv((int64_t)touched_cap * (vec ? E / 4 : E), 256);
  if (blocks > 256 * 8) blocks = 256 * 8;
  if (vec) MML_LAUNCH(opt_rows_kernel<4>, dim3((unsigned)blocks), dim3(256), 0, to_stream(stream), L);
  else MML_LAUNCH(opt_rows_kernel<1>, dim3((unsigned)blocks), dim3(256), 0, to_stream(stream), L);
  return check_launch("mml_opt_step_rows");
}

extern "C" int mml_counter_update(int32_t* counter, int32_t delta, int32_t reset, mml_stream_t stream) {
  MML_REQUIRE(counter, "mml_counter_update: null counter");
  MML_LAUNCH(counter_kernel, dim3(1), dim3(64), 0, to_stream(stream), counter, delta, reset);
  return check_launch("mml_counter_update");
}

extern "C" int mml_ew_mul(const float* a, const float* b, float* out, int64_t n, mml_stream_t stream) {
  MML_REQUIRE(n >= 0 && (n == 0 || (a && b && out)), "mml_ew_mul: null argument");
  if (n == 0) return MML_OK;
  MML_LAUNCH(ew_mul_kernel, dim3(ew_grid(n)), dim3(256), 0, to_stream(stream), a, b, out, n);
  return check_launch("mml_ew_mul");
}

extern "C" int mml_ew_mul_bwd_act(const float* dout, const float* a, const float* b, float* da, float* db,
                                  int32_t acc_a, int32_t acc_b, int64_t n, int32_t act_a, int32_t act_b,
                                  mml_stream_t stream) {
  MML_REQUIRE(n >= 0 && (n == 0 || dout), "mml_ew_mul_bwd: null dout");
  MML_REQUIRE(!da || b, "mml_ew_mul_bwd: da needs b");
  MML_REQUIRE(!db || a, "mml_ew_mul_bwd: db needs a");
  MML_REQUIRE(act_a >= MML_ACT_NONE && act_a <= MML_ACT_SIGMOID2 && act_b >= MML_ACT_NONE && act_b <= MML_ACT_SIGMOID2,
              "mml_ew_mul_bwd: unknown activation");
  MML_REQUIRE((!act_a || (a && da && !acc_a)) && (!act_b || (b && db && !acc_b)),
              "mml_ew_mul_bwd: a folded activation derivative needs the operand, its gradient, and no accumulation");
  if (n == 0) return MML_OK;
  MML_LAUNCH(ew_mul_bwd_kernel, dim3(ew_grid(n)), dim3(256), 0, to_stream(stream), dout, a, b, da, db, acc_a,
                     acc_b, n, act_a, act_b);
  return check_launch("mml_ew_mul_bwd");
}

extern "C" int mml_ew_mul_bwd(const float* dout, const float* a, const float* b, float* da, float* db, int32_t acc_a,
                              int32_t acc_b, int64_t n, mml_stream_t stream) {
  return mml_ew_mul_bwd_act(dout, a, b, da, db, acc_a, acc_b, n, MML_ACT_NONE, MML_ACT_NONE, stream);
}

extern "C" int mml_ew_add_n(const float* const* in, int32_t n_in, float* out, int64_t n, mml_stream_t stream) {
  MML_REQUIRE(in && n_in >= 1 && n_in <= 16 && out && n >= 0, "mml_ew_add_n: bad arguments");
  if (n == 0) return MML_OK;
  AddN A{};
  A.n_in = n_in;
  for (int i = 0; i < n_in; ++i) {
    MML_REQUIRE(in[i], "mml_ew_add_n: input %d null", i);
    A.in[i] = in[i];
  }
  MML_LAUNCH(ew_add_n_kernel, dim3(ew_grid(n)), dim3(256), 0, to_stream(stream), A, out, n);
  return check_launch("mml_ew_add_n");
}

extern "C" int mml_copy2d(const float* src, int64_t lds_, float* dst, int64_t ldd, int64_t rows, int32_t cols,
                          int32_t accumulate, mml_stream_t stream) {
  MML_REQUIRE(rows >= 0 && cols >= 0, "mml_copy2d: negative extent");
  if (rows == 0 || cols == 0) return MML_OK;
  MML_REQUIRE(src && dst && lds_ >= cols && ldd >= cols, "mml_copy2d: null pointer or leading dimension < cols");
  MML_LAUNCH(copy2d_kernel, dim3(ew_grid(rows * cols)), dim3(256), 0, to_stream(stream), src, lds_, dst, ldd,
                     rows, cols, accumulate);
  return check_launch("mml_copy2d");
}

extern "C" int mml_copy2d_batch(const mml_copy2d_desc* d, int32_t n, mml_stream_t stream) {
  MML_REQUIRE(n >= 0 && (n == 0 || d), "mml_copy2d_batch: null descriptor array");
  for (int i0 = 0; i0 < n; i0 += COPY2D_BATCH) {
    Copy2dBatch Bt{};
    int m = 0;
    int64_t most = 0;
    for (int i = i0; i < n && m < COPY2D_BATCH; ++i) {
      const mml_copy2d_desc& D = d[i];
      MML_REQUIRE(D.rows >= 0 && D.cols >= 0, "mml_copy2d_batch: item %d has a negative extent", i);
      if (D.rows == 0 || D.cols == 0) continue;
      MML_REQUIRE(D.src && D.dst && D.lds >= D.cols && D.ldd >= D.cols,
                  "mml_copy2d_batch: item %d: null pointer or leading dimension < cols", i);
      Bt.d[m++] = D;
      most = D.rows * D.cols > most ? D.rows * D.cols : most;
    }
    if (m == 0) continue;
    MML_LAUNCH(copy2d_batch_kernel, dim3(ew_grid(most), (unsigned)m), dim3(256), 0, to_stream(stream), Bt);
    int rc = check_launch("mml_copy2d_batch");
    if (rc) return rc;
  }
  return MML_OK;
}

extern "C" int mml_copy_cols(const float* const* src, const int64_t* lds_, float* const* dst, const int64_t* ldd,
                             const int32_t* width, int32_t n_seg, int64_t rows, int32_t accumulate,
                             mml_stream_t stream) {
  MML_REQUIRE(n_seg >= 0 && rows >= 0, "mml_copy_cols: negative extent");
  if (n_seg == 0 || rows == 0) return MML_OK;
  MML_REQUIRE(src && lds_ && dst && ldd && width, "mml_copy_cols: null array");
  for (int i0 = 0; i0 < n_seg; i0 += MML_MAX_FIELDS) {
    ColSegs S{};
    S.n = (n_seg - i0 < MML_MAX_FIELDS) ? (n_seg - i0) : MML_MAX_FIELDS;
    int acc = 0;
    for (int s = 0; s < S.n; ++s) {
      const int k = i0 + s;
      MML_REQUIRE(src[k] && dst[k] && width[k] > 0 && lds_[k] >= width[k] && ldd[k] >= width[k],
                  "mml_copy_cols: segment %d malformed", k);
      S.src[s] = src[k]; S.dst[s] = dst[k]; S.lds_[s] = lds_[k]; S.ldd[s] = ldd[k]; S.width[s] = width[k];
      S.start[s] = acc;
      acc += width[k];
    }
    S.start[S.n] = acc;
    bool v4 = (acc >> 2) <= COPY_COLS_MAX_W4;
    for (int s = 0; s < S.n && v4; ++s)
      v4 = S.width[s] % 4 == 0 && S.lds_[s] % 4 == 0 && S.ldd[s] % 4 == 0 && aligned16(S.src[s]) && aligned16(S.dst[s]);
    if (v4)
      MML_LAUNCH(copy_cols_vec4_kernel, dim3(ew_grid(rows * (acc >> 2))), dim3(256), 0, to_stream(stream), S, rows,
                 accumulate);
    else
      MML_LAUNCH(copy_cols_kernel, dim3(ew_grid(rows * acc)), dim3(256), 0, to_stream(stream), S, rows, accumulate);
    int rc = check_launch("mml_copy_cols");
    if (rc) return rc;
  }
  return MML_OK;
}

extern "C" int mml_act_bwd(const float* y, const float* dy, float* dst, int64_t n, int32_t act, mml_stream_t stream) {
  MML_REQUIRE(n >= 0 && (n == 0 || (y && dy && dst)), "mml_act_bwd: null argument");
  MML_REQUIRE(act >= MML_ACT_NONE && act <= MML_ACT_SIGMOID2, "mml_act_bwd: unknown activation %d", act);
  if (n == 0) return MML_OK;
  MML_LAUNCH(act_bwd_kernel, dim3(ew_grid(n)), dim3(256), 0, to_stream(stream), y, dy, dst, n, act);
  return check_launch("mml_act_bwd");
}

extern "C" int mml_sumprod_batch(const mml_sumprod_desc* d, int32_t n, mml_stream_t stream) {
  MML_REQUIRE(n >= 0 && (n == 0 || d), "mml_sumprod_batch: bad descriptor array");
  for (int i0 = 0; i0 < n; i0 += MML_SUMPROD_BATCH) {
    SumProdBatch Bt{};
    const int m = (n - i0 < MML_SUMPROD_BATCH) ? n - i0 : MML_SUMPROD_BATCH;
    int64_t nmax = 0;
    for (int i = 0; i < m; ++i) {
      const mml_sumprod_desc& D = d[i0 + i];
      MML_REQUIRE(D.out && D.n >= 0 && D.n_terms >= 0 && D.n_terms <= MML_SUMPROD_TERMS, "mml_sumprod_batch: item %d malformed", i0 + i);
      for (int k = 0; k < D.n_terms; ++k) MML_REQUIRE(D.x[k], "mml_sumprod_batch: item %d term %d is null", i0 + i, k);
      MML_REQUIRE(D.act >= MML_ACT_NONE && D.act <= MML_ACT_SIGMOID2 && (D.act == MML_ACT_NONE || (D.deriv_of && !D.accumulate)),
                  "mml_sumprod_batch: item %d: a folded activation derivative needs deriv_of and no accumulation", i0 + i);
      Bt.d[i] = D;
      nmax = D.n > nmax ? D.n : nmax;
    }
    if (nmax == 0) continue;
    unsigned gx = ew_grid(nmax);
    const unsigned cap = (unsigned)(2048 / m > 64 ? 2048 / m : 64);
    if (gx > cap) gx = cap;
    MML_LAUNCH(sumprod_batch_kernel, dim3(gx, (unsigned)m), dim3(256), 0, to_stream(stream), Bt);
    int rc = check_launch("mml_sumprod_batch");
    if (rc) return rc;
  }
  return MML_OK;
}
```

mmlrec-a-unified-multi-task-and-multi-scenario-learning-benchmark-for-recommendation_amd/ops.py:

```python
import ctypes as C

import os

import torch

from . import _lib as L

_workspaces = {}


def _stream():
    return torch.cuda.current_stream().cuda_stream


_masked_streams = {}


def cu_range_stream(device, cu_lo, cu_hi):
    idx = device.index if device.index is not None else torch.cuda.current_device()
    key = (idx, int(cu_lo), int(cu_hi))
    st = _masked_streams.get(key)
    if st is None:
        h = C.c_void_p()
        L.check(L.load().mml_stream_create_cu_range(idx, int(cu_lo), int(cu_hi), C.byref(h)))
# ... 604 lines not shown
def make_tower_head_group(tasks, prob, y, mask=None, loss=None):
    g = L.TowerHeadGroup()
    g.n, g.M = len(tasks), prob.shape[0]
    g.prob, g.ldprob = prob.data_ptr(), _ld(prob)
    g.y, g.ldy = y.data_ptr(), _ld(y)
    if mask is not None:
        g.mask, g.ldmask = mask.data_ptr(), _ld(mask)
    g.loss = L.ptr(loss)
    for t, q in enumerate(tasks):
        d = g.t[t]
        A = q["A"]
        d.A, d.lda, d.K = A.data_ptr(), _ld(A), A.shape[1]
        d.N = q["dH"].shape[1]
        d.amax_a = q["amax_a"].data_ptr()
        d.w_planes_fwd, d.ldpf, d.kexp_fwd = q["planes_fwd"].data_ptr(), _ld(q["planes_fwd"]), q["kexp_fwd"].data_ptr()
        d.w_planes_bwd, d.ldpb, d.kexp_bwd = q["planes_bwd"].data_ptr(), _ld(q["planes_bwd"]), q["kexp_bwd"].data_ptr()
        d.bias1 = L.ptr(q.get("bias1"))
        d.w, d.hbias = q["w"].data_ptr(), q["hbias"].data_ptr()
        b2 = q.get("hbias2")
        d.hbias2, d.n_hbias2 = L.ptr(b2), (0 if b2 is None else b2.numel())
        d.dH, d.lddh = q["dH"].data_ptr(), _ld(q["dH"])
        d.dA, d.ldda = q["dA"].data_ptr(), _ld(q["dA"])
        d.dw, d.dhbias = q["dw"].data_ptr(), q["dhbias"].data_ptr()
        d.amax_dH, d.amax_dA = L.ptr(q.get("amax_dH")), L.ptr(q.get("amax_dA"))
        d.mask_col, d.head = int(q.get("mask_col", -1)), int(q.get("head", t))
        d.kind = int(q.get("kind", 0))
    return g


def tower_head_fwd_bwd(group, device, phases=False):
    lib = L.load()
    n = int(lib.mml_tower_head_workspace_bytes(C.byref(group)))
    if n < 0:
        L.check(-1, "mml_tower_head_workspace_bytes")
    ws = torch.empty(max(n, 256), dtype=torch.uint8, device=device)
    for ph in ((1, 2) if phases else (0,)):
        L.check(lib.mml_tower_head_fwd_bwd(C.byref(group), ws.data_ptr(), ws.numel(), ph, _stream()), "mml_tower_head_fwd_bwd")
    return ws


def head_fwd(group):
    lib = L.load()
    L.check(lib.mml_head_fwd(C.byref(group), _stream()), "mml_head_fwd")


def head_bce_fwd_bwd(group, device, phases=False):
    lib = L.load()
    ws = workspace(lib.mml_head_workspace_bytes(C.byref(group)), device)
    if phases:
        for ph in (1, 2):
            L.check(lib.mml_head_bce_fwd_bwd_phase(C.byref(group), ws.data_ptr(), ws.numel(), ph, _stream()),
                    "mml_head_bce_fwd_bwd_phase")
        return
    L.check(lib.mml_head_bce_fwd_bwd(C.byref(group), ws.data_ptr(), ws.numel(), _stream()), "mml_head_bce_fwd_bwd")


def rows_phase1_then_batched_reduce(head_groups, gate_groups, device):
    lib = L.load()
    items = (L.RowsReduceItem * (len(head_groups) + len(gate_groups)))()
    keep, k = [], 0
    for kind, groups in ((L.ROWS_REDUCE_HEAD, head_groups), (L.ROWS_REDUCE_GATE, gate_groups)):
        for g in groups:
            if kind == L.ROWS_REDUCE_HEAD:
                ws = torch.empty(max(int(lib.mml_head_workspace_bytes(C.byref(g))), 256), dtype=torch.uint8, device=device)
                L.check(lib.mml_head_bce_fwd_bwd_phase(C.byref(g), ws.data_ptr(), ws.numel(), 1, _stream()),
                        "mml_head_bce_fwd_bwd_phase")
            else:
                ws = torch.empty(max(int(lib.mml_gate_mix_bwd_workspace_bytes(C.byref(g))), 256), dtype=torch.uint8,
                                 device=device)
                L.check(lib.mml_gate_mix_bwd_phase(C.byref(g), ws.data_ptr(), ws.numel(), 1, _stream()),
                        "mml_gate_mix_bwd_phase")
            keep.append(ws)
            items[k].kind, items[k].group = kind, C.addressof(g)
            items[k].workspace, items[k].workspace_bytes = ws.data_ptr(), ws.numel()
            k += 1
    L.check(lib.mml_rows_reduce_batch(items, k, _stream()), "mml_rows_reduce_batch")
    return keep


def ew_mul(a, b, out):
    L.check(L.load().mml_ew_mul(a.data_ptr(), b.data_ptr(), out.data_ptr(), out.numel(), _stream()), "mml_ew_mul")


def ew_mul_bwd(dout, a, b, da=None, db=None, acc_a=False, acc_b=False):
    L.check(L.load().mml_ew_mul_bwd(dout.data_ptr(), L.ptr(a), L.ptr(b), L.ptr(da), L.ptr(db), int(acc_a), int(acc_b),
                                    dout.numel(), _stream()), "mml_ew_mul_bwd")


def ew_add_n(inputs, out):
    L.check(L.load().mml_ew_add_n(_ptr_array(inputs), len(inputs), out.data_ptr(), out.numel(), _stream()),
            "mml_ew_add_n")


def dropout(x, out, p, seed, site=0, step=0, step_dev=None, accumulate=False, row0=0):
    L.check(L.load().mml_dropout(x.data_ptr(), _ld(x), out.data_ptr(), _ld(out), x.shape[0], x.shape[1], int(row0), float(p),
                                 int(seed) & ((1 << 64) - 1), int(site) & 0xffffffff, L.ptr(step_dev), int(step),
                                 int(accumulate), _stream()), "mml_dropout")


def copy2d(src, dst, accumulate=False):
    rows, cols = src.shape
    L.check(L.load().mml_copy2d(src.data_ptr(), _ld(src), dst.data_ptr(), _ld(dst), rows, cols, int(accumulate),
                                _stream()), "mml_copy2d")


def prelu_max_batch():
    return int(L.load().mml_prelu_max_batch())


def make_prelu_descs(items):
    arr = (L.PreluDesc * len(items))()
    for d, it in zip(arr, items):
        z, y = _f32_2d(it["z"], "prelu z"), _f32_2d(it["y"], "prelu y")
        if y.shape != z.shape or it["alpha"].dtype != torch.float32 or it["alpha"].numel() != 1:
            raise L.MMLError("prelu: y must have z's shape and alpha one float32 element")
        d.z, d.ldz, d.y, d.ldy, d.rows, d.cols = z.data_ptr(), _ld(z), y.data_ptr(), _ld(y), z.shape[0], z.shape[1]
        d.alpha, d.amax_out = it["alpha"].data_ptr(), L.ptr(it.get("amax"))
    return arr


def make_prelu_bwd_descs(items, seen=None):
    arr = (L.PreluBwdDesc * len(items))()
    for d, it in zip(arr, items):
        dy, z, dz = _f32_2d(it["dy"], "prelu dy"), _f32_2d(it["z"], "prelu z"), _f32_2d(it["dz"], "prelu dz")
        if dy.shape != z.shape or dz.shape != z.shape:
            raise L.MMLError("prelu backward: dy, z and dz must have one shape")
        for k in ("alpha", "dalpha"):
            if it[k].dtype != torch.float32 or it[k].numel() != 1:
                raise L.MMLError(f"prelu backward: {k} must be one float32 element")
        d.dy, d.lddy, d.z, d.ldz, d.dz, d.lddz = dy.data_ptr(), _ld(dy), z.data_ptr(), _ld(z), dz.data_ptr(), _ld(dz)
        d.rows, d.cols, d.alpha, d.dalpha = z.shape[0], z.shape[1], it["alpha"].data_ptr(), it["dalpha"].data_ptr()
        d.accumulate_dz = int(bool(it.get("acc_dz")))
        d.accumulate_dalpha = int(bool(it.get("acc_dalpha")) or (seen is not None and d.dalpha in seen))
        d.amax_out = L.ptr(it.get("amax"))
    return arr


def prelu_chunks(items):
    cap = prelu_max_batch()
    return [items[i:i + cap] for i in range(0, len(items), cap)]


def prelu_fwd(items):
    _need_gpu(*[it["z"] for it in items])
    for chunk in prelu_chunks(items):
        L.check(L.load().mml_prelu_batch_fwd(make_prelu_descs(chunk), len(chunk), _stream()), "mml_prelu_batch_fwd")


def prelu_bwd(items):
    _need_gpu(*[it["z"] for it in items])
    seen = set()
    for chunk in prelu_chunks(items):
        arr = make_prelu_bwd_descs(chunk, seen)
        first = {}
        for d in arr:
            d.accumulate_dalpha = first.setdefault(d.dalpha, d.accumulate_dalpha)
        nbytes = int(L.load().mml_prelu_workspace_bytes(len(chunk)))
        ws = workspace(nbytes, chunk[0]["z"].device)
        L.check(L.load().mml_prelu_batch_bwd(arr, len(chunk), ws.data_ptr(), nbytes, _stream()), "mml_prelu_batch_bwd")
        seen.update(d.dalpha for d in arr)


def make_pcgrad_segs(segs, T, need_out=False):
    arr = (L.PcgradSeg * max(len(segs), 1))()
    for d, sg in zip(arr, segs):
        banks = list(sg["banks"])
        if len(banks) != T:
            raise L.MMLError(f"pcgrad: a segment has {len(banks)} banks for T = {T}")
        have = [b for b in banks if b is not None] + ([sg["out"]] if sg.get("out") is not None else [])
        if not have:
            raise L.MMLError("pcgrad: a segment whose banks are all None")
        _need_gpu(*have)
        ref = have[0]
        for b in have:
            if (b.dtype != torch.float32 or b.dim() not in (1, 2) or b.shape != ref.shape or b.stride() != ref.stride() or
                    (b.shape[-1] > 1 and b.stride(-1) != 1)):
                raise L.MMLError("pcgrad: banks and out of a segment must be float32 views of one shape and pitch")
        rows, cols = (1, ref.shape[0]) if ref.dim() == 1 else ref.shape
        for k, b in enumerate(banks):
            d.bank[k] = b.data_ptr() if b is not None else None
        d.out = L.ptr(sg.get("out"))
        d.rows, d.cols, d.ld = rows, cols, (cols if ref.dim() == 1 else _ld(ref))
        marks = sg.get("marks")
        if marks is not None and (marks.dtype != torch.uint8 or marks.numel() < rows or not marks.is_contiguous()):
            raise L.MMLError("pcgrad: marks must be a contiguous uint8 tensor with one byte per row")
        d.row_marks = L.ptr(marks)
        if need_out and sg.get("out") is None:
            raise L.MMLError("pcgrad combine: a segment without `out`")
    return arr


def pcgrad_gram(segs, T, gram=None):
    arr = make_pcgrad_segs(segs, T)
    dev = next(b for b in segs[0]["banks"] if b is not None).device
    if gram is None:
        gram = torch.empty((T, T), dtype=torch.float64, device=dev)
    nbytes = int(L.load().mml_pcgrad_workspace_bytes(arr, len(segs), T))
    ws = workspace(nbytes, dev)
    L.check(L.load().mml_pcgrad_gram(arr, len(segs), T, gram.data_ptr(), ws.data_ptr(), nbytes, _stream()),
            "mml_pcgrad_gram")
    return gram


def pcgrad_weights(gram, order, w=None, fired=None):
    _need_gpu(gram, order)
    T = gram.shape[0]
    if gram.dtype != torch.float64 or order.dtype != torch.int32 or order.numel() != T * T or gram.numel() != T * T \
            or not gram.is_contiguous() or not order.is_contiguous():
        raise L.MMLError("pcgrad_weights: gram [T, T] float64 and order [T, T] int32, contiguous")
    if w is None:
        w = torch.empty(2 * T, dtype=torch.float32, device=gram.device)
    if fired is None:
        fired = torch.empty((T, T), dtype=torch.int32, device=gram.device)
    L.check(L.load().mml_pcgrad_weights(gram.data_ptr(), order.data_ptr(), T, w.data_ptr(), fired.data_ptr(), _stream()),
            "mml_pcgrad_weights")
    return w, fired


def pcgrad_combine(segs, T, w):
    _need_gpu(w)
    arr = make_pcgrad_segs(segs, T, need_out=True)
    L.check(L.load().mml_pcgrad_combine(arr, len(segs), T, w.data_ptr(), _stream()), "mml_pcgrad_combine")


def act_bwd(y, dy, dst, act):
    L.check(L.load().mml_act_bwd(y.data_ptr(), dy.data_ptr(), dst.data_ptr(), y.numel(), act, _stream()), "mml_act_bwd")


def make_hyper(kind, lr, step=1, step_dev=None, zero_grad=False, max_blocks=0, cold_loop=0):
    h = L.OptHyper()
    h.cold_loop = int(cold_loop)
    h.kind = L.OPT_KINDS[kind] if isinstance(kind, str) else int(kind)
    h.step = int(step)
    h.step_dev = L.ptr(step_dev)
    h.lr = float(lr)
    h.beta1, h.beta2 = 0.9, 0.999
    h.eps = {L.OPT_ADAM: 1e-8, L.OPT_ADAGRAD: 1e-10, L.OPT_RMSPROP: 1e-8}.get(h.kind, 0.0)
    h.alpha = 0.99
    h.zero_grad = int(zero_grad)
    h.max_blocks = int(max_blocks)
    return h


def make_opt_tensors(entries):
    arr = (L.OptTensor * len(entries))()
    for d, ent in zip(arr, entries):
        p, g, s1, s2 = ent[:4]
        d.param, d.grad, d.state1, d.state2, d.n = p.data_ptr(), g.data_ptr(), L.ptr(s1), L.ptr(s2), p.numel()
        d.l1, d.l2 = ent[4] if len(ent) > 4 and ent[4] else (0.0, 0.0)
        if len(ent) > 5 and ent[5] is not None:
            d.skip_rows, d.row_elems, d.zero_grads = ent[5].data_ptr(), p.shape[1], 1
        if len(ent) > 6 and ent[6] is not None:
            d.grad_marks, d.row_elems = ent[6].data_ptr(), p.shape[1]
        if len(ent) > 7 and ent[7] is not None:
            d.acc64, d.acc_amax, d.acc_shift = ent[7][0].data_ptr(), ent[7][1].data_ptr(), int(ent[7][2])
        if len(ent) > 8 and ent[8] is not None:
            d.warm_rows = ent[8].data_ptr()
    return arr


def opt_step_dense(entries, hyper):
    arr = make_opt_tensors(entries)
    L.check(L.load().mml_opt_step_dense(arr, len(entries), C.byref(hyper), _stream()), "mml_opt_step_dense")


def opt_step_rows(tables, grad_tables, state1, state2, seen, rowbase, touched, touched_count, hyper, last=None):
    F, E = len(tables), tables[0].shape[1]
    rb = (L.i64 * (F + 1))(*rowbase)
    L.check(L.load().mml_opt_step_rows(_ptr_array(tables), _ptr_array(grad_tables),
                                       _ptr_array(state1) if state1 is not None else None,
                                       _ptr_array(state2) if state2 is not None else None,
                                       _ptr_array(seen), rb, F, E, touched.data_ptr(), touched_count.data_ptr(),
                                       touched.numel(), _ptr_array(last) if last is not None else None,
                                       C.byref(hyper), _stream()), "mml_opt_step_rows")


def index_unique(vocab, cols, E, X, seen, rowbase, touched, touched_count, status=None, marks=None):
    F = len(vocab)
    L.check(L.load().mml_index_unique((L.i64 * F)(*vocab), (L.i32 * F)(*cols), F, E, X.data_ptr(), _ld(X), X.shape[0],
                                      _ptr_array(seen), (L.i64 * (F + 1))(*rowbase), touched.data_ptr(),
                                      touched_count.data_ptr(), touched.numel(), L.ptr(marks), L.ptr(status), _stream()),
            "mml_index_unique")


def opt_catchup_rows(tables, state1, state2, last, rowbase, touched, touched_count, hyper):
    F, E = len(tables), tables[0].shape[1]
    L.check(L.load().mml_opt_catchup_rows(_ptr_array(tables), _ptr_array(state1),
                                          _ptr_array(state2) if state2 is not None else None, _ptr_array(last),
                                          (L.i64 * (F + 1))(*rowbase), F, E, touched.data_ptr(),
                                          touched_count.data_ptr(), touched.numel(), C.byref(hyper), _stream()),
            "mml_opt_catchup_rows")


def opt_catchup_dense(table, state1, state2, last, hyper):
    L.check(L.load().mml_opt_catchup_dense(table.data_ptr(), L.ptr(state1), L.ptr(state2), last.data_ptr(),
                                           table.shape[0], table.shape[1], C.byref(hyper), _stream()),
            "mml_opt_catchup_dense")


def counter_update(counter, delta=1, reset=False):
    L.check(L.load().mml_counter_update(counter.data_ptr(), int(delta), int(reset), _stream()), "mml_counter_update")


def auc_segments(pred, y, seg):
    lib = L.load()
    n, c = pred.shape
    out = torch.empty(((n + seg - 1) // seg, c), dtype=torch.float64, device=pred.device)
    L.check(lib.mml_auc_segments(pred.data_ptr(), pred.stride(0), y.data_ptr(), y.stride(0), n, c, int(seg),
                                 out.data_ptr(), _stream()), "mml_auc_segments")
    return out


AUC_STATUS_NONFINITE = 16


def auc_key_image(score):
    import struct
    u, = struct.unpack("<I", struct.pack("<f", float(score)))
    if u == 0x80000000:
        u = 0
    return (~u & 0xffffffff) if u & 0x80000000 else (u | 0x80000000)


_auc_workspaces = {}


def _auc_workspace(device, n, cols, seg):
    nbytes = L.load().mml_auc_sorted_workspace_bytes(int(n), int(cols), int(seg))
    if nbytes < 0:
        raise L.MMLError(f"mml_auc_sorted: n * cols = {n} * {cols} keys, the call takes fewer than 2^31")
    if torch.cuda.is_current_stream_capturing():
        return torch.empty(max(int(nbytes), 8), dtype=torch.uint8, device=device)
    key = (device.type, device.index, _stream(), int(n), int(cols), int(seg))
    ws = _auc_workspaces.get(key)
    if ws is None:
        if len(_auc_workspaces) >= 8:
            _auc_workspaces.pop(next(iter(_auc_workspaces)))
        ws = torch.empty(max(int(nbytes), 8), dtype=torch.uint8, device=device)
        _auc_workspaces[key] = ws
    return ws


def auc_sorted(pred, y, seg=0, mask=None, return_counts=False, status=None):
    _need_gpu(pred, y, mask, status)
    lib = L.load()
    pred, y = _f32_2d(pred, "pred"), _f32_2d(y, "y")
    n, c = pred.shape
    if tuple(y.shape) != (n, c):
        raise L.MMLError(f"auc_sorted: pred {tuple(pred.shape)} and y {tuple(y.shape)} differ")
    seg = int(seg)
    if seg <= 0 or seg >= n:
        seg = 0
    nseg = 1 if seg == 0 else (n + seg - 1) // seg
    mask_cols = 0
    if mask is not None:
        mask = _f32_2d(mask, "mask")
        mask_cols = mask.shape[1]
        if mask.shape[0] != n:
            raise L.MMLError(f"auc_sorted: mask has {mask.shape[0]} rows, pred {n}")
    out = torch.empty((nseg, c), dtype=torch.float64, device=pred.device)
    counts = torch.empty((nseg, c, 3), dtype=torch.int64, device=pred.device) if return_counts else None
    if status is None:
        status = torch.zeros(1, dtype=torch.int32, device=pred.device)
    ws = _auc_workspace(pred.device, n, c, seg)
    L.check(lib.mml_auc_sorted(pred.data_ptr(), _ld(pred), y.data_ptr(), _ld(y), L.ptr(mask),
                               _ld(mask) if mask is not None else 0, mask_cols, n, c, seg, ws.data_ptr(), ws.numel(),
                               out.data_ptr(), L.ptr(counts), status.data_ptr(), _stream()), "mml_auc_sorted")
    return (out, counts) if return_counts else out


def _is16(t):
    return t.dtype == torch.bfloat16


def _need16(t, name):
    if t.dtype != torch.bfloat16 or t.dim() != 2 or t.stride(1) != 1:
        raise L.MMLError(f"{name}: expected a bf16 2-D tensor with unit inner stride, got {t.dtype} {tuple(t.shape)}")
    return t


def make_cast16_descs(items):
    arr = (L.Cast16Desc * len(items))()
    for d, (src, dst, tr) in zip(arr, items):
        _f32_2d(src, "cast16 source")
        _need16(dst, "cast16 destination")
        want = (src.shape[1], src.shape[0]) if tr else tuple(src.shape)
        if tuple(dst.shape) != want:
            raise L.MMLError(f"cast16: destination shape {tuple(dst.shape)}, expected {want}")
        d.src, d.dst, d.rows, d.cols = src.data_ptr(), dst.data_ptr(), src.shape[0], src.shape[1]
        d.lds, d.ldd, d.transpose = _ld(src), _ld(dst), int(bool(tr))
    return arr


def cast16(src, transpose=False, out=None):
    _need_gpu(src)
    if out is None:
        shape = (src.shape[1], src.shape[0]) if transpose else tuple(src.shape)
        out = torch.empty(shape, dtype=torch.bfloat16, device=src.device)
    arr = make_cast16_descs([(src, out, transpose)])
    L.check(L.load().mml_cast16_batch(arr, 1, _stream()), "mml_cast16_batch")
    return out


def gather16_fwd(tables, X, cols, dense_col0=0, nd=0, out=None, status=None):
    lib = L.load()
    _need_gpu(X, *tables)
    X = _f32_2d(X, "X")
    F, E, B = len(tables), tables[0].shape[1], X.shape[0]
    if out is None:
        out = torch.empty((B, F * E + nd), dtype=torch.bfloat16, device=X.device)
    vocab = (L.i64 * F)(*[t.shape[0] for t in tables])
    col = (L.i32 * F)(*cols)
    L.check(lib.mml_gather16_fwd(_ptr_array(tables), vocab, col, F, E, X.data_ptr(), _ld(X), dense_col0, nd, B,
                                 out.data_ptr(), _ld(out), L.ptr(status), _stream()), "mml_gather16_fwd")
    return out


def make_g16_tn_descs(problems):
    arr = (L.G16TnDesc * len(problems))()
    for d, q in zip(arr, problems):
        Cm = q["C"]
        d.M, d.N = Cm.shape
        d.n_src = len(q["srcs"])
        if not 1 <= d.n_src <= L.MAX_SRC:
            raise L.MMLError("g16_tn: 1 .. MAX_SRC sources")
        for s, (A, Bm) in enumerate(q["srcs"]):
            _need16(A, "g16_tn A")
            _need16(Bm, "g16_tn B")
            if A.shape[0] != d.M or Bm.shape[0] != d.N or A.shape[1] != Bm.shape[1]:
                raise L.MMLError(f"g16_tn: source {s} shapes {tuple(A.shape)} x {tuple(Bm.shape)} for C {tuple(Cm.shape)}")
            d.A[s], d.B[s], d.lda[s], d.ldb[s], d.K[s] = A.data_ptr(), Bm.data_ptr(), _ld(A), _ld(Bm), A.shape[1]
        d.act = int(q.get("act", L.ACT_NONE))
        d.bias = L.ptr(q.get("bias"))
        d.C, d.ldc, d.c_bf16 = Cm.data_ptr(), _ld(Cm), int(_is16(Cm))
        if not d.c_bf16 and Cm.dtype != torch.float32:
            raise L.MMLError("g16_tn: C must be bf16 or fp32")
        d.accumulate = int(q.get("accumulate", 0))
        mo, mi = q.get("mask_out"), q.get("mask_in")
        d.mask_out, d.mask_in = L.ptr(mo), L.ptr(mi)
        m = mo if mo is not None else mi
        d.ldmask = _ld(m) if m is not None else 0
    return arr


def g16_tn(problems):
    arr = make_g16_tn_descs(problems)
    L.check(L.load().mml_g16_tn(arr, len(problems), _stream()), "mml_g16_tn")


def make_g16_wgrad_descs(problems):
    arr = (L.G16WgradDesc * len(problems))()
    for d, q in zip(arr, problems):
        dC, A, dW = _need16(q["dC"], "g16_wgrad dC"), _need16(q["A"], "g16_wgrad A"), _f32_2d(q["dW"], "g16_wgrad dW")
        d.M, d.N, d.K = dC.shape[0], dC.shape[1], A.shape[1]
        if A.shape[0] != d.M or tuple(dW.shape) != (d.N, d.K):
            raise L.MMLError("g16_wgrad: shape mismatch")
        d.dC, d.A, d.dW, d.dbias = dC.data_ptr(), A.data_ptr(), dW.data_ptr(), L.ptr(q.get("dbias"))
        d.lddc, d.lda, d.lddw = _ld(dC), _ld(A), _ld(dW)
        d.accumulate = int(q.get("accumulate", 0))
    return arr


def g16_wgrad(problems, phases=False):
    lib = L.load()
    arr = make_g16_wgrad_descs(problems)
    n = int(lib.mml_g16_wgrad_workspace_bytes(arr, len(problems)))
    if n < 0:
        L.check(-1, "mml_g16_wgrad_workspace_bytes")
    ws = torch.empty(max(n, 16), dtype=torch.uint8, device=problems[0]["dW"].device)
    for ph in ((1, 2) if phases else (0,)):
        L.check(lib.mml_g16_wgrad(arr, len(problems), ws.data_ptr(), ws.numel(), ph, _stream()), "mml_g16_wgrad")
```

mmlrec-a-unified-multi-task-and-multi-scenario-learning-benchmark-for-recommendation_amd/optimizer.py:

```python
import ctypes as C
import dataclasses
import os
import typing

import torch

from . import _lib as L
from . import engine as E
from . import ops


@dataclasses.dataclass(frozen=True)
class OptKnobs:
    lazy_min_params: int = 1 << 22
    auto_table_update: str = "lazy_exact"
    early_blocks: int = 0
    tail_blocks: int = 1 << 20
    opt_u: typing.Optional[int] = None
    one_launch: bool = False
    variant: int = 0
    scatter_old: bool = False
    cold_rows: bool = True
    cold_compact: bool = True

    @classmethod
    def from_env(cls, env=None):
        env = os.environ if env is None else env
        u = env.get("MMLREC_OPT_U")
        return cls(lazy_min_params=int(env.get("MMLREC_LAZY_MIN_PARAMS", str(1 << 22))),
                   auto_table_update=env.get("MMLREC_AUTO_TABLE_UPDATE", "lazy_exact"),
                   early_blocks=int(env.get("MMLREC_EARLY_BLOCKS", "0")),
                   tail_blocks=int(env.get("MMLREC_TAIL_BLOCKS", str(1 << 20))),
                   opt_u=int(u) if u is not None else None,
                   one_launch=env.get("MMLREC_OPT_ONE_LAUNCH", "0") == "1",
                   variant=int(env.get("MMLREC_OPT_VARIANT", "0")),
                   scatter_old=bool(env.get("MMLREC_SCATTER_OLD")),
                   cold_rows=env.get("MMLREC_OPT_COLD_ROWS", "1") != "0",
                   cold_compact=env.get("MMLREC_OPT_COLD_COMPACT", "1") != "0")


TABLE_UPDATES = ("dense_exact", "sparse_rows", "lazy_exact")
BYTES_PER_PARAM = {"sgd": 12, "adam": 28, "adagrad": 20, "rmsprop": 20}


def resolve_table_update(kind, requested, widths, one_table_per_field, table_params, table_reg, knobs):
    mode = requested
    if requested == "auto":
        if kind in ("sgd", "adagrad"):
            mode = "sparse_rows"
        else:
            ok = (len(widths) == 1 and widths <= {4, 8, 16} and one_table_per_field and
                  table_params > knobs.lazy_min_params and knobs.auto_table_update == "lazy_exact")
            mode = "lazy_exact" if ok else "dense_exact"
        if table_reg:
            mode = "dense_exact"
    if mode == "lazy_exact" and kind in ("sgd", "adagrad"):
        mode = "sparse_rows"
    if mode not in TABLE_UPDATES:
        raise ValueError("table_update must be auto, dense_exact, sparse_rows or lazy_exact")
    return mode


def opt_dense_symbol(numel, ntensors, form=0, opt_u=None):
    if not L.opt_dense_streams(numel, ntensors, form in (3, 4)):
        return "opt_flat_kernel"
    u = {0: 1, 1: 1, 2: 4, 3: 2 if opt_u is None else opt_u, 4: 4 if opt_u == 4 else 2}[form]
    return "opt_dense_kernel<true, %d, %d>" % (form, u)


class DenseLaunch(typing.NamedTuple):
    tables: tuple
    marked: bool
    form: int
    bytes: float
    kernel: str


def dense_table_launches(kind, numels, rows, marks, split_dense, cap, det_deferred, knobs, det_exact=True):
    n = len(numels)
    big = [i for i in range(n) if numels[i] >= L.OPT_HUGE_MIN_PARAMS]
    if len(big) > L.OPT_STREAM_MAX_TENSORS or sum(numels[i] for i in big) < L.OPT_STREAM_MIN_PARAMS:
        big = []
    small = [i for i in range(n) if i not in big]
    one_launch = bool(big and small and cap > 0 and n <= L.MAX_OPT_TENSORS and not split_dense and all(marks) and
                      knobs.one_launch)
    if det_deferred:
        if not (det_exact and L.opt_takes_det_totals(numels, all(marks), split_dense)):
            raise L.MMLError("the deterministic scatter deferred its totals to a marked dense update of exactly its "
                             "tables")
        one_launch = True
    if one_launch:
        big, small = small + big, []
    per = BYTES_PER_PARAM[kind] - (4 if split_dense else 0)
    out = []
    for grp in (big, small):
        if not grp:
            continue
        marked = grp is big and all(marks[i] for i in grp)
        numel = sum(numels[i] for i in grp)
        nbytes = float(per) * numel
        form = (4 if det_deferred else 3 if (cap > 0 and marked) else 2 if (cap > 0 and split_dense) else
                1 if (knobs.variant & 2 and not marked and not split_dense) else 0)
        if marked:
            nbytes += sum(rows[i] - 4.0 * numels[i] for i in grp)
        out.append(DenseLaunch(tuple(grp), marked, form, nbytes, opt_dense_symbol(numel, len(grp), form, knobs.opt_u)))
    return out


WARM_KINDS = ("adam", "rmsprop", "adagrad")


def launch_trusts_warm_map(kind, marked, table_reg, knobs, sharded=False):
    return bool(marked and kind in WARM_KINDS and not table_reg and knobs.cold_rows and not sharded)


def cold_loop_of(knobs):
    return 0 if knobs.cold_compact else 1


class TableRows:

    def __init__(self, vocab, device, cap):
        self.rowbase = [0]
        for v in vocab:
            self.rowbase.append(self.rowbase[-1] + int(v))
        self.seen = [torch.zeros((int(v) + 31) // 32, dtype=torch.int32, device=device) for v in vocab]
        self.marks = torch.zeros(ops.marks_bytes(vocab), dtype=torch.uint8, device=device)
        self.touched = torch.zeros(max(int(cap), 1), dtype=torch.int32, device=device)
        self.count = torch.zeros(1, dtype=torch.int32, device=device)


class ParamStore:

    def __init__(self, model, device):
        self.device = device
        self.model = model
        tables, dense = [], []
        for name, p in model.named_parameters():
            (tables if name.startswith("embedding_dict.") else dense).append((name, p))
        self.sig = tuple(p.data_ptr() for _, p in tables + dense)
        total = sum(p.numel() for _, p in dense)
        self.arena = torch.zeros(max(total, 1), dtype=torch.float32, device=device)
        self.pvals = {}
        off = 0
        for name, p in dense:
            g = self.arena[off:off + p.numel()].view(p.shape)
            off += p.numel()
            self.pvals[name] = E.PVal(p.data, g, name)
            self.pvals[name].stable = True
        self.table_names = [n for n, _ in tables]
        for name, p in tables:
            self.pvals[name] = E.PVal(p.data, None, name, is_table=True)
        par = getattr(model, "_parallel", None)
        if par is not None and par.mode == "row_sharded":
            self.pvals["embedding_shard"] = E.PVal(par.shard, None, "embedding_shard", is_table=True)
            self.table_names = ["embedding_shard"]
        self.table_grads_ready = False
        self.opt = None
        self.rows = None
        self.rows_names = None
        self._grad_marks_key = self._det_key = None
        self.extra = {}

    def ensure_table_grads(self):
        if not self.table_grads_ready:
            for n in self.table_names:
                pv = self.pvals[n]
                pv.grad = torch.zeros_like(pv.data)
                pv.needs_grad = True
            self.table_grads_ready = True

    def ensure_rows(self, cap, names=None):
        names = list(self.table_names if names is None else names)
        if self.rows is None or self.rows.touched.numel() < cap or self.rows_names != names:
            self.rows = TableRows([self.pvals[n].data.shape[0] for n in names], self.device, cap)
            self.rows_names = names
        return self.rows

    def ensure_grad_marks(self, tables):
        vocab = [int(t.data.shape[0]) for t in tables]
        key = tuple(t.data.data_ptr() for t in tables)
        if self._grad_marks_key != key:
            self.grad_marks = torch.zeros(ops.marks_bytes(vocab), dtype=torch.uint8, device=self.device)
            self._grad_marks_key = key
        base, off = [], 0
        for v in vocab:
            base.append(off)
            off += (v + 31) // 32 * 32
        return self.grad_marks, base

    def grad_marks_by_table(self, gop):
        gm = getattr(gop, "grad_marks", None)
        if gm is None:
            return {}
        _, base = self.ensure_grad_marks(gop.tables)
        return {id(t): gm[base[f]:base[f] + t.data.shape[0]] for f, t in enumerate(gop.tables)}

    def ensure_det(self, tables):
        key = tuple(t.data.data_ptr() for t in tables)
        if self._det_key != key:
            uniq = {}
            for t in tables:
                uniq.setdefault(t.data.data_ptr(), torch.zeros(t.data.shape, dtype=torch.int64, device=self.device))
            self._det = dict(acc64=[uniq[t.data.data_ptr()] for t in tables],
                             marks=torch.zeros(ops.marks_bytes([int(t.data.shape[0]) for t in tables]), dtype=torch.uint8,
                                               device=self.device),
                             slot=ops.amax_slots(1, self.device)[0])
            self._det_key = key
        return self._det

    def stale(self):
        return self.sig != tuple(p.data_ptr() for _, p in self.model.named_parameters())

    def reset_written(self):
        for pv in self.pvals.values():
            pv.written = 0
        for pv in self.extra.values():
            pv.written = 0


class _OptState(dict):

    def __init__(self, store, kind):
        super().__init__()
        self.store, self.kind = store, kind
        self.warm = {}

    def __missing__(self, name):
        pv = self.store.pvals[name]
        s1 = torch.zeros_like(pv.data) if self.kind != "sgd" else None
        s2 = torch.zeros_like(pv.data) if self.kind == "adam" else None
        dict.__setitem__(self, name, (s1, s2))
        if pv.is_table and s1 is not None:
            self.warm[name] = torch.zeros(pv.data.shape[0], dtype=torch.uint8, device=pv.data.device)
        return (s1, s2)

    def __setitem__(self, name, value):
        self.warm.pop(name, None)
        dict.__setitem__(self, name, value)

    def __delitem__(self, name):
        self.warm.pop(name, None)
        dict.__delitem__(self, name)


class Optimizer:

    def __init__(self, store, kind, lr, table_update="auto"):
        self.store, self.kind, self.lr = store, kind, float(lr)
        if kind not in L.OPT_KINDS:
            raise NotImplementedError(kind)
        self.auto = table_update == "auto"
        tabs = [p for n, p in store.model.named_parameters() if n.startswith("embedding_dict.")]
        cols = store.model._sparse_cols() if hasattr(store.model, "_sparse_cols") else []
        self.table_update = resolve_table_update(
            kind, table_update, widths={int(p.shape[1]) for p in tabs},
            one_table_per_field=len({f.embedding_name for f in cols}) == len(cols),
            table_params=sum(p.numel() for p in tabs), table_reg=self.table_reg() if self.auto else None,
            knobs=OptKnobs.from_env())
        self.last = None
        self.dirty = False
        dev = store.device
        self.step_dev = torch.zeros(1, dtype=torch.int32, device=dev)
        self.state = _OptState(store, kind)
        self.warm = self.state.warm
        self.steps_done = 0

    def warm_map(self, name):
        self.state[name]
        return self.warm.get(name)

    def all_rows_warm(self, names):
        for n in names:
            self.state[n]
            if n in self.warm:
                self.warm[n].fill_(1)

    def calls(self, plan):
        c = self.calls_split(plan)
        return c["pre"] + c["early"] + c["mlp"] + c["tables"]

    def split_dense_ok(self, widths):
        return (self.table_update == "dense_exact" and not self.table_reg() and
                all(w <= 16 and w % 4 == 0 for w in widths))

    def can_split_dense(self, plan):
        gop = plan.ops[0] if plan.ops else None
        if not isinstance(gop, E.GatherOp) or isinstance(gop, E.PooledGatherOp):
            return False
        return self.split_dense_ok([t.data.shape[1] for t in gop.tables])

    def calls_split(self, plan, split_dense=False):
        knobs = OptKnobs.from_env()
        pre = [(L.load().mml_counter_update, (self.step_dev.data_ptr(), 1, 0))]
        if self.table_update == "lazy_exact":
            pre += self._lazy_pre_calls(plan)
        split_dense = bool(split_dense) and self.can_split_dense(plan)
        if split_dense and getattr(plan.ops[0], "mark_rows", None) is None:
            pre += self.index_pre_calls(plan)
        reg = self._reg_map()
        treg = self.table_reg(reg)
        names = [n for n in self.store.table_names if self.store.pvals[n].written]
        if treg and self.table_update != "dense_exact":
            raise NotImplementedError("l2_reg_embedding / l1 on the tables makes every row's gradient non-zero: use "
                                      "table_update='dense_exact' (the reference's own dense optimizer)")
        hyper = ops.make_hyper(self.kind, self.lr, step=0, step_dev=self.step_dev, zero_grad=False)
        plan.keep.append(hyper)
        mlp = self._mlp_calls(plan, reg, hyper)
        early, tables = [], []
        if names and self.table_update == "dense_exact":
            (early if split_dense else tables).extend(self._dense_table_calls(plan, names, treg, split_dense, knobs))
        if names and (self.table_update != "dense_exact" or split_dense):
            tables += self._row_update_calls(plan, names, hyper, knobs)
        return {"pre": pre, "early": early, "mlp": mlp, "tables": tables}

    def _mlp_calls(self, plan, reg, hyper):
        dense = [(pv, n) for n, pv in self.store.pvals.items()
                 if not pv.is_table and pv.grad is not None and (pv.written or pv.data.data_ptr() in reg)]
        if not dense:
            return []
        arr = ops.make_opt_tensors([(pv.data, pv.grad) + self.state[n] + (reg.get(pv.data.data_ptr()),)
                                    for pv, n in dense])
        plan.keep.append(arr)
        numel = sum(pv.data.numel() for pv, _ in dense)
        return [(L.load().mml_opt_step_dense, (arr, len(dense), C.byref(hyper)),
                 dict(kernel=opt_dense_symbol(numel, len(dense)), bytes=float(BYTES_PER_PARAM[self.kind]) * numel))]

    def _dense_table_calls(self, plan, names, treg, split_dense, knobs):
        st = self.store
        tabs = [st.pvals[n] for n in names]
        cap = knobs.early_blocks if split_dense else knobs.tail_blocks
        hz = ops.make_hyper(self.kind, self.lr, step=0, step_dev=self.step_dev, zero_grad=not split_dense,
                            max_blocks=cap, cold_loop=cold_loop_of(knobs))
        plan.keep.append(hz)
        seen_of = dict(zip(st.rows_names, st.rows.seen)) if split_dense else {}
        gop = plan.ops[0] if plan.ops else None
        marks_of = {} if split_dense else st.grad_marks_by_table(gop)
        dd = getattr(gop, "det_deferred", None)
        launches = dense_table_launches(
            self.kind, [t.data.numel() for t in tabs], [t.data.shape[0] for t in tabs],
            [id(t) in marks_of for t in tabs], split_dense, cap, dd is not None, knobs,
            det_exact=dd is None or {id(t) for t in tabs} == {id(t) for t in gop.tables})
        acc_of = {id(t): a for t, a in zip(gop.tables, gop.deterministic["acc64"])} if dd else {}
        calls = []
        for ln in launches:
            trust = launch_trusts_warm_map(self.kind, ln.marked, treg, knobs, sharded=not isinstance(gop, E.GatherOp))
            if not trust:
                self.all_rows_warm([names[i] for i in ln.tables])
            arr = ops.make_opt_tensors([(tabs[i].data, tabs[i].grad) + self.state[names[i]] +
                                        (treg, seen_of.get(names[i]), marks_of[id(tabs[i])] if ln.marked else None,
                                         (acc_of[id(tabs[i])], dd["slot"], dd["shift"]) if dd else None,
                                         self.warm_map(names[i]) if trust else None)
                                        for i in ln.tables])
            plan.keep.append(arr)
            m = dict(kernel=ln.kernel, bytes=ln.bytes)
            if dd:
                m.update(det_acc64=True, ptrs=[dd["slot"].data_ptr()] + [a.data_ptr() for a in acc_of.values()])
            calls.append((L.load().mml_opt_step_dense, (arr, len(ln.tables), C.byref(hz)), m))
        return calls

    def _row_update_calls(self, plan, names, hyper, knobs):
        rows = self.store.rows
        a = self._row_arrays(plan, names, grads=True, last=self.table_update == "lazy_exact")
        self.all_rows_warm(names)
        calls = [(L.load().mml_opt_step_rows, (a["param"], a["grad"], a["s1"], a["s2"], a["seen"], a["rowbase"], a["F"],
                                               a["E"], rows.touched.data_ptr(), rows.count.data_ptr(),
                                               rows.touched.numel(), a["last"], C.byref(hyper)),
                  dict(kernel="opt_rows_kernel"))]
        if a["E"] not in (4, 8, 16) or knobs.scatter_old:
            calls.append((L.load().mml_counter_update, (rows.count.data_ptr(), 0, 1)))
        return calls

    def _row_arrays(self, plan, names, grads=False, state=True, last=False):
        st, rows = self.store, self.store.rows
        tabs = [st.pvals[n] for n in names]
        F = len(tabs)
        a = dict(F=F, E=tabs[0].data.shape[1], vocab=(L.i64 * F)(*[t.data.shape[0] for t in tabs]),
                 param=ops._ptr_array([t.data for t in tabs]), seen=ops._ptr_array(rows.seen),
                 rowbase=(L.i64 * (F + 1))(*rows.rowbase),
                 grad=ops._ptr_array([t.grad for t in tabs]) if grads else None,
                 s1=ops._ptr_array([self.state[n][0] for n in names]) if state and self.kind != "sgd" else None,
                 s2=ops._ptr_array([self.state[n][1] for n in names]) if state and self.kind == "adam" else None,
                 last=ops._ptr_array([self.last[n] for n in names]) if last else None)
        plan.keep += [v for v in a.values() if isinstance(v, C.Array)]
        return a

    def _index_unique_call(self, plan, gop, a):
        rows = self.store.rows
        X, nrows = gop.index_view(plan)
        col = (L.i32 * a["F"])(*gop.cols)
        plan.keep.append(col)
        return (L.load().mml_index_unique, (a["vocab"], col, a["F"], a["E"], X.data_ptr(), ops._ld(X), nrows, a["seen"],
                                            a["rowbase"], rows.touched.data_ptr(), rows.count.data_ptr(),
                                            rows.touched.numel(), rows.marks.data_ptr(), plan.status.data_ptr()),
                dict(kernel="mark_rows_kernel+rows_compact_kernel", bytes=float(nrows) * a["F"] * 5))

    def index_pre_calls(self, plan):
        st, gop = self.store, plan.ops[0]
        if st.rows is None or list(st.rows_names) != list(st.table_names):
            raise L.MMLError("split dense update needs ParamStore.ensure_rows over every table")
        unique = self._index_unique_call(plan, gop, self._row_arrays(plan, st.table_names, state=False))
        return gop.pre_index_calls(plan) + [unique]

    def _reg_map(self):
        out = {}
        for weight_list, l1, l2 in getattr(self.store.model, "regularization_weight", []):
            if not (l1 > 0 or l2 > 0):
                continue
            for w in weight_list:
                p = w[1] if isinstance(w, tuple) else w
                a, b = out.get(p.data_ptr(), (0.0, 0.0))
                out[p.data_ptr()] = (a + float(l1), b + float(l2))
        return out

    def table_reg(self, reg=None):
        reg = self._reg_map() if reg is None else reg
        vals = {reg[p.data_ptr()] for n, p in self.store.model.named_parameters()
                if n.startswith("embedding_dict.") and p.data_ptr() in reg}
        if not vals:
            return None
        if len(vals) > 1:
            raise NotImplementedError("different regularisers on different embedding tables")
        return vals.pop()

    def _lazy_pre_calls(self, plan):
        lib, st = L.load(), self.store
        gop = plan.ops[0]
        names = st.table_names
        rows = st.rows
        if self.last is None:
            self.last = {n: torch.zeros(st.pvals[n].data.shape[0], dtype=torch.int32, device=st.device) for n in names}
        a = self._row_arrays(plan, names, last=True)
        self.all_rows_warm(names)
        hyper = ops.make_hyper(self.kind, self.lr, step=0, step_dev=self.step_dev)
        plan.keep.append(hyper)
        catchup = (lib.mml_opt_catchup_rows, (a["param"], a["s1"], a["s2"], a["last"], a["rowbase"], a["F"], a["E"],
                                              rows.touched.data_ptr(), rows.count.data_ptr(), rows.touched.numel(),
                                              C.byref(hyper)), dict(kernel="opt_catchup_kernel"))
        if getattr(gop, "owns_lazy", False):
            if a["F"] != 1:
                raise L.MMLError("row-sharded lazy_exact expects the single flat shard")

            def launch(keys_ptr, n, stream):
                if n:
                    L.check(lib.mml_index_unique_idx32(a["vocab"], 1, a["E"], keys_ptr, 1, n, a["seen"], a["rowbase"],
                                                       rows.touched.data_ptr(), rows.count.data_ptr(),
                                                       rows.touched.numel(), rows.marks.data_ptr(),
                                                       plan.status.data_ptr(), stream), "mml_index_unique_idx32")
                    L.check(catchup[0](*catchup[1], stream), "mml_opt_catchup_rows")
            gop.lazy_launch = launch
            return []
        if not isinstance(gop, E.GatherOp):
            raise L.MMLError("lazy_exact table updates are not available on the table-wise sharded path")
        if isinstance(gop, E.PooledGatherOp):
            return gop.pre_index_calls(plan) + gop.unique_calls(plan, rows) + [catchup]
        unique = self._index_unique_call(plan, gop, a)
        return gop.pre_index_calls(plan) + [unique, catchup]

    def flush(self):
        if self.table_update != "lazy_exact" or not self.dirty or self.last is None:
            return
        hyper = ops.make_hyper(self.kind, self.lr, step=0, step_dev=self.step_dev)
        self.all_rows_warm(self.store.table_names)
        for n in self.store.table_names:
            s1, s2 = self.state[n]
            ops.opt_catchup_dense(self.store.pvals[n].data, s1, s2 if self.kind == "adam" else None, self.last[n], hyper)
        self.dirty = False
```

Before: 60.35 million samples/s.

## Precompute Adam step constants once and run marked-row optimizer as resident grid

```diff
diff --git a/include/mmlrec.h b/include/mmlrec.h
--- a/include/mmlrec.h
+++ b/include/mmlrec.h
@@ -603,6 +603,15 @@
   int32_t max_blocks;
   int32_t cold_loop;
 } mml_opt_hyper;
+typedef struct {
+  int32_t step;
+  float step_size;
+  float inv_bc2s;
+  int32_t pad_;
+} mml_opt_step_consts;
+int mml_opt_step_begin(int32_t* step_dev, int32_t delta, const mml_opt_hyper* hyper, mml_opt_step_consts* consts,
+                       mml_stream_t stream);
+int mml_opt_step_unbind(const int32_t* step_dev);
 int mml_opt_step_dense(const mml_opt_tensor* tensors, int32_t n, const mml_opt_hyper* hyper, mml_stream_t stream);
 int mml_opt_step_rows(float* const* tables, float* const* grad_tables, float* const* state1, float* const* state2,
                       uint32_t* const* seen, const int64_t* rowbase, int32_t F, int32_t E,
diff --git a/mmlrec-a-unified-multi-task-and-multi-scenario-learning-benchmark-for-recommendation_amd/_lib.py b/mmlrec-a-unified-multi-task-and-multi-scenario-learning-benchmark-for-recommendation_amd/_lib.py
--- a/mmlrec-a-unified-multi-task-and-multi-scenario-learning-benchmark-for-recommendation_amd/_lib.py
+++ b/mmlrec-a-unified-multi-task-and-multi-scenario-learning-benchmark-for-recommendation_amd/_lib.py
@@ -183,6 +183,10 @@
     _fields_ = [("kind", i32), ("step", i32), ("step_dev", fp), ("lr", C.c_float), ("beta1", C.c_float),
                 ("beta2", C.c_float), ("eps", C.c_float), ("alpha", C.c_float), ("zero_grad", i32), ("max_blocks", i32),
                 ("cold_loop", i32)]
+
+
+class OptStepConsts(C.Structure):
+    _fields_ = [("step", i32), ("step_size", C.c_float), ("inv_bc2s", C.c_float), ("pad_", i32)]
 
 
 _PP = C.POINTER
@@ -302,6 +306,8 @@
     "mml_index_unique": (C.c_int, [_PP(i64), _PP(i32), i32, i32, fp, i64, i64, _PP(fp), _PP(i64), fp, fp, i32, fp, fp,
                                    fp]),
     "mml_counter_update": (C.c_int, [fp, i32, i32, fp]),
+    "mml_opt_step_begin": (C.c_int, [fp, i32, _PP(OptHyper), fp, fp]),
+    "mml_opt_step_unbind": (C.c_int, [fp]),
     "mml_gather_pool_wgmax_len": (i64, [_PP(PoolDesc), i32, i64]),
     "mml_gather_pool_fwd": (C.c_int, [_PP(PoolDesc), fp, i64, i32, i32, i64, fp, i64, fp, i64, fp, i64, fp, fp]),
     "mml_scatter_pool_bwd": (C.c_int, [_PP(PoolDesc), fp, i64, i64, fp, i64, fp, i64, _PP(fp), _PP(i64), fp, fp, i32,
diff --git a/mmlrec-a-unified-multi-task-and-multi-scenario-learning-benchmark-for-recommendation_amd/csrc/optim_ew.hip b/mmlrec-a-unified-multi-task-and-multi-scenario-learning-benchmark-for-recommendation_amd/csrc/optim_ew.hip
--- a/mmlrec-a-unified-multi-task-and-multi-scenario-learning-benchmark-for-recommendation_amd/csrc/optim_ew.hip
+++ b/mmlrec-a-unified-multi-task-and-multi-scenario-learning-benchmark-for-recommendation_amd/csrc/optim_ew.hip
@@ -2,6 +2,9 @@
 #include "fold_fixed.hpp"
 
 #include <stdlib.h>
+
+#include <mutex>
+#include <vector>
 
 #ifndef MML_OPT_COLD_CB
 #define MML_OPT_COLD_CB 8
@@ -17,6 +20,7 @@
   int64_t chunk0[MML_MAX_OPT_TENSORS + 1];
   int32_t blk0[MML_MAX_OPT_TENSORS + 1];
   int32_t prop;
+  const mml_opt_step_consts* sc;
 };
 static_assert(sizeof(OptLaunch) <= 4096, "OptLaunch travels by value: the kernel-argument block holds 4 KB");
 
@@ -25,19 +29,33 @@
   float inv_bc2s;
 };
 
-__device__ __forceinline__ StepConsts step_consts(const mml_opt_hyper& h) {
+__device__ __forceinline__ StepConsts step_consts_of(const mml_opt_hyper& h, int t) {
+  StepConsts c{h.lr, 1.f};
+  if (h.kind == MML_OPT_ADAM) {
+    const double bc1 = 1.0 - pow((double)h.beta1, (double)t);
+    const double bc2 = 1.0 - pow((double)h.beta2, (double)t);
+    c.step_size = (float)((double)h.lr / bc1);
+    c.inv_bc2s = (float)(1.0 / sqrt(bc2));
+  }
+  return c;
+}
+
+__device__ __forceinline__ StepConsts step_consts(const mml_opt_hyper& h, const mml_opt_step_consts* bound = nullptr) {
+  bool have = false;
+  StepConsts r{h.lr, 1.f};
+  if (bound) {
+    if (h.kind != MML_OPT_ADAM) {
+      have = true;
+    } else if (bound->step == *h.step_dev) {
+      r.step_size = bound->step_size;
+      r.inv_bc2s = bound->inv_bc2s;
+      have = true;
+    }
+  }
+  if (have) return r;
   __shared__ StepConsts sc;
-  if (threadIdx.x == 0) {
-    StepConsts c{h.lr, 1.f};
-    if (h.kind == MML_OPT_ADAM) {
-      const int t = h.step_dev ? *h.step_dev : h.step;
-      const double bc1 = 1.0 - pow((double)h.beta1, (double)t);
-      const double bc2 = 1.0 - pow((double)h.beta2, (double)t);
-      c.step_size = (float)((double)h.lr / bc1);
-      c.inv_bc2s = (float)(1.0 / sqrt(bc2));
-    }
-    sc = c;
-  }
+  if (threadIdx.x == 0)
+    sc = step_consts_of(h, h.kind != MML_OPT_ADAM ? 0 : h.step_dev ? *h.step_dev : h.step);
   __syncthreads();
   return sc;
 }
@@ -72,11 +90,227 @@
   return g;
 }
 
+typedef float vf4 __attribute__((ext_vector_type(4)));
+typedef long long vl2 __attribute__((ext_vector_type(2)));
+constexpr int COLD_RPL = 4, COLD_SPAN = 64 * COLD_RPL;
+constexpr int COLD_DENSE_PCT = 15;
+constexpr int COLD_WAVES = 4;
+
+struct ColdTensor {
+  vf4 *P, *G, *S1, *S2;
+  vl2* A64;
+  uint8_t *gm, *wr;
+  int64_t rows;
+  int csh;
+  int emax, acc_shift;
+  bool zg;
+};
+
+template <int WITH_ACC>
+__device__ __forceinline__ ColdTensor cold_tensor(const mml_opt_tensor& T) {
+  ColdTensor X;
+  X.P = reinterpret_cast<vf4*>(T.param);
+  X.G = reinterpret_cast<vf4*>(const_cast<float*>(T.grad));
+  X.S1 = reinterpret_cast<vf4*>(T.state1);
+  X.S2 = reinterpret_cast<vf4*>(T.state2);
+  X.A64 = WITH_ACC ? reinterpret_cast<vl2*>(T.acc64) : nullptr;
+  X.gm = T.grad_marks;
+  X.wr = T.warm_rows;
+  const int rsh = __builtin_ctz((unsigned)T.row_elems);
+  X.rows = T.n >> rsh;
+  X.csh = rsh - 2;
+  X.emax = 1;
+  if (WITH_ACC && X.A64) {
+    uint32_t m = 0;
+    for (int w = 0; w < MML_AMAX_WORDS; ++w) m = T.acc_amax[w] > m ? T.acc_amax[w] : m;
+    X.emax = (int)(m >> 23);
+    X.emax = X.emax < 1 ? 1 : (X.emax > 254 ? 254 : X.emax);
+  }
+  X.acc_shift = T.acc_shift;
+  X.zg = T.zero_grads != 0;
+  return X;
+}
+
+__device__ __forceinline__ void cold_scan(const uint8_t* gm, const uint8_t* wr, int64_t rows, int64_t s, int lane,
+                                          uint32_t& mk, uint32_t& wk) {
+  const int64_t r0 = s * COLD_SPAN + lane * COLD_RPL;
+  mk = wk = 0u;
+  if (r0 + COLD_RPL <= rows) {
+    mk = *reinterpret_cast<const uint32_t*>(gm + r0);
+    wk = *reinterpret_cast<const uint32_t*>(wr + r0);
+  } else {
+#pragma unroll
+    for (int k = 0; k < COLD_RPL; ++k)
+      if (r0 + k < rows) {
+        mk |= (uint32_t)gm[r0 + k] << (8 * k);
+        wk |= (uint32_t)wr[r0 + k] << (8 * k);
+      }
+  }
+}
+
+template <int WITH_ACC>
+__device__ __forceinline__ void cold_span(const mml_opt_hyper& h, const StepConsts& c, bool nt, const ColdTensor& X,
+                                          int64_t s, int lane, uint16_t* lst, uint32_t mk, uint32_t wk) {
+  constexpr int RPL = COLD_RPL, SPAN = COLD_SPAN;
+  const vf4 zero = {0.f, 0.f, 0.f, 0.f};
+  const vl2 lzero = {0, 0};
+  auto nz80 = [](uint32_t x) { return (x | ((x & 0x7f7f7f7fu) + 0x7f7f7f7fu)) & 0x80808080u; };
+  auto pack4 = [](uint32_t t) { return ((t >> 7) & 1u) | ((t >> 14) & 2u) | ((t >> 21) & 4u) | ((t >> 28) & 8u); };
+  const uint32_t lm = pack4(nz80(mk)), wm = pack4(nz80(wk));
+  const uint32_t act = lm | wm;
+  if (__builtin_amdgcn_ballot_w64(act != 0) == 0) return;
+  auto ld = [&](const vf4* q) { return nt ? __builtin_nontemporal_load(q) : *q; };
+  auto st = [&](vf4* q, const vf4& v) {
+    if (nt) __builtin_nontemporal_store(v, q);
+    else *q = v;
+  };
+  const int csh = X.csh;
+  const int64_t rows = X.rows, row0 = s * SPAN;
+  const uint32_t cnt = (uint32_t)__builtin_popcount(act);
+  uint32_t pre = 0;
+  int nlive = 0;
+#pragma unroll
+  for (int bit = 0; (1 << bit) <= RPL; ++bit) {
+    const uint64_t bal = __builtin_amdgcn_ballot_w64(((cnt >> bit) & 1u) != 0);
+    pre += __builtin_amdgcn_mbcnt_hi((uint32_t)(bal >> 32), __builtin_amdgcn_mbcnt_lo((uint32_t)bal, 0u)) << bit;
+    nlive += __builtin_popcountll(bal) << bit;
+  }
+  const bool dense = nlive * 100 >= SPAN * COLD_DENSE_PCT;
+  if (!dense) {
+    __builtin_amdgcn_fence(__ATOMIC_RELEASE, "wavefront");
+    __builtin_amdgcn_wave_barrier();
+#pragma unroll
+    for (int k = 0; k < RPL; ++k)
+      if ((act >> k) & 1u)
+        lst[pre++] = (uint16_t)((lane * RPL + k) | (((lm >> k) & 1u) << 14) | (((wm >> k) & 1u) << 15));
+    __builtin_amdgcn_fence(__ATOMIC_RELEASE, "wavefront");
+    __builtin_amdgcn_wave_barrier();
+  }
+  if (lm) {
+    const int64_t r0 = row0 + lane * RPL;
+    if (r0 + RPL <= rows) {
+      *reinterpret_cast<uint32_t*>(X.gm + r0) = 0u;
+      const uint32_t set = (nz80(mk) & ~nz80(wk)) >> 7;
+      if (set) *reinterpret_cast<uint32_t*>(X.wr + r0) = wk | set;
+    } else {
+#pragma unroll
+      for (int k = 0; k < RPL; ++k)
+        if ((lm >> k) & 1u) {
+          X.gm[r0 + k] = 0;
+          if (!((wm >> k) & 1u)) X.wr[r0 + k] = 1;
+        }
+    }
+  }
+  const int items = (dense ? SPAN : nlive) << csh;
+#pragma unroll 1
+  for (int b0 = 0; b0 < items; b0 += 128) {
+    vf4 p[2], a[2], b[2], g[2];
+    vl2 t0[2], t1[2];
+    int64_t jj[2];
+    bool on[2], lv[2];
+#pragma unroll
+    for (int k = 0; k < 2; ++k) {
+      const int it = b0 + 64 * k + lane;
+      const int ent = it >> csh;
+      on[k] = it < items;
+      uint32_t e;
+      if (dense) {
+        const uint32_t src = (uint32_t)__shfl((int)(lm | (act << 16)), (ent / RPL) & 63);
+        on[k] = on[k] && ((src >> (16 + (ent & (RPL - 1)))) & 1u);
+        e = (uint32_t)ent | (((src >> (ent & (RPL - 1))) & 1u) << 14);
+      } else {
+        e = on[k] ? lst[ent] : 0u;
+      }
+      lv[k] = on[k] && ((e >> 14) & 1u);
+      const int64_t j = ((row0 + (int64_t)(e & 0x3fffu)) << csh) | (int64_t)(it & ((1 << csh) - 1));
+      jj[k] = j;
+      p[k] = a[k] = b[k] = g[k] = zero;
+      t0[k] = t1[k] = lzero;
+      if (on[k]) {
+        p[k] = ld(X.P + j);
+        if (X.S1) a[k] = ld(X.S1 + j);
+        if (X.S2) b[k] = ld(X.S2 + j);
+      }
+      if (lv[k]) {
+        if (!X.zg) g[k] = ld(X.G + j);
+        if (WITH_ACC && X.A64) {
+          t0[k] = X.A64[2 * j];
+          t1[k] = X.A64[2 * j + 1];
+        }
+      }
+    }
+#pragma unroll
+    for (int k = 0; k < 2; ++k) {
+      if (!on[k]) continue;
+      const int64_t j = jj[k];
+      vf4 gs = g[k];
+      if (WITH_ACC && X.A64 && lv[k]) {
+        const vl2 u0 = t0[k], u1 = t1[k];
+        if (u0.x) gs.x += from_fixed(u0.x, X.emax, X.acc_shift);
+        if (u0.y) gs.y += from_fixed(u0.y, X.emax, X.acc_shift);
+        if (u1.x) gs.z += from_fixed(u1.x, X.emax, X.acc_shift);
+        if (u1.y) gs.w += from_fixed(u1.y, X.emax, X.acc_shift);
+        if (u0.x | u0.y) X.A64[2 * j] = lzero;
+        if (u1.x | u1.y) X.A64[2 * j + 1] = lzero;
+      }
+#pragma unroll
+      for (int e = 0; e < 4; ++e) {
+        float pe = p[k][e], ae = a[k][e], be = b[k][e];
+        opt_update(h, c, pe, gs[e], ae, be);
+        p[k][e] = pe;
+        a[k][e] = ae;
+        b[k][e] = be;
+      }
+      st(X.P + j, p[k]);
+      if (X.S1) st(X.S1 + j, a[k]);
+      if (X.S2) st(X.S2 + j, b[k]);
+      if (h.zero_grad && (g[k].x != 0.f || g[k].y != 0.f || g[k].z != 0.f || g[k].w != 0.f)) X.G[j] = zero;
+    }
+  }
+}
+
+template <int WITH_ACC>
+__device__ __forceinline__ void cold_resident(const OptLaunch& L, const StepConsts& c, uint16_t (*live_rows)[COLD_SPAN]) {
+  const mml_opt_hyper& h = L.h;
+  const bool nt = (L.variant & 1) != 0;
+  const int lane = threadIdx.x & 63;
+  const int wv = __builtin_amdgcn_readfirstlane((int)(threadIdx.x >> 6));
+  uint16_t* const lst = live_rows[wv];
+  const int nspan = L.blk0[L.n], nwv = (int)gridDim.x * COLD_WAVES;
+  int s = (int)blockIdx.x * COLD_WAVES + wv;
+  if (s >= nspan) return;
+  int ti = 0;
+  while (s >= L.blk0[ti + 1]) ++ti;
+  ColdTensor X = cold_tensor<WITH_ACC>(L.t[ti]);
+  uint32_t mk, wk;
+  cold_scan(X.gm, X.wr, X.rows, s - L.blk0[ti], lane, mk, wk);
+  for (;;) {
+    const int sn = s + nwv;
+    int tn = ti;
+    uint32_t mkn = 0, wkn = 0;
+    if (sn < nspan) {
+      while (sn >= L.blk0[tn + 1]) ++tn;
+      const mml_opt_tensor& Tn = L.t[tn];
+      cold_scan(Tn.grad_marks, Tn.warm_rows, Tn.n >> __builtin_ctz((unsigned)Tn.row_elems), sn - L.blk0[tn], lane, mkn,
+                wkn);
+    }
+    cold_span<WITH_ACC>(h, c, nt, X, s - L.blk0[ti], lane, lst, mk, wk);
+    if (sn >= nspan) break;
+    if (tn != ti) {
+      ti = tn;
+      X = cold_tensor<WITH_ACC>(L.t[ti]);
+    }
+    s = sn;
+    mk = mkn;
+    wk = wkn;
+  }
+}
+
 enum { OPT_PLAIN = 0, OPT_UNROLL2 = 1, OPT_SKIP_U = 2, OPT_MARK_U = 3, OPT_MARK_ACC_U = 4 };
 template <bool STREAM, int PATH, int U>
 __global__ __launch_bounds__(256) void opt_dense_kernel(const OptLaunch L) {
   int ti = blockIdx.y, nblk = gridDim.x, lblk = blockIdx.x;
-  if (L.prop) {
+  if (L.prop == 1) {
     ti = 0;
     while (ti + 1 < L.n && (int)blockIdx.x >= L.blk0[ti + 1]) ++ti;
     nblk = L.blk0[ti + 1] - L.blk0[ti];
@@ -84,7 +318,12 @@
   }
   const mml_opt_tensor& T = L.t[ti];
   const mml_opt_hyper& h = L.h;
-  const StepConsts c = step_consts(h);
+  const StepConsts c = step_consts(h, L.sc);
+  __shared__ uint16_t live_rows[(PATH == OPT_MARK_U || PATH == OPT_MARK_ACC_U) ? COLD_WAVES : 1][COLD_SPAN];
+  if ((PATH == OPT_MARK_U || PATH == OPT_MARK_ACC_U) && L.prop == 2) {
+    cold_resident<PATH == OPT_MARK_ACC_U>(L, c, live_rows);
+    return;
+  }
   const int64_t n4 = T.n >> 2;
   const bool vec = aligned16(T.param) && aligned16(T.grad) && (!T.state1 || aligned16(T.state1)) &&
                    (!T.state2 || aligned16(T.state2));
@@ -196,130 +435,17 @@
     const bool compact = !(L.variant & 8) && wr &&
                          ((reinterpret_cast<uintptr_t>(gm) | reinterpret_cast<uintptr_t>(wr)) & 3) == 0;
     if ((PATH == OPT_MARK_U || PATH == OPT_MARK_ACC_U) && compact && !skip) {
-      constexpr int RPL = 4, SPAN = 64 * RPL;
-      constexpr int DENSE_PCT = 15;
-      constexpr int WAVES = 4;
-      __shared__ uint16_t live_rows[WAVES][SPAN];
       const int lane = threadIdx.x & 63;
       const int wv = __builtin_amdgcn_readfirstlane((int)(threadIdx.x >> 6));
-      uint16_t* const lst = live_rows[wv];
-      const int csh = rsh - 2;
-      const int64_t rows = T.n >> rsh;
-      const int64_t nspan = (rows + SPAN - 1) / SPAN, nwv = (int64_t)nblk * WAVES;
-      auto nz80 = [](uint32_t x) { return (x | ((x & 0x7f7f7f7fu) + 0x7f7f7f7fu)) & 0x80808080u; };
-      auto pack4 = [](uint32_t t) { return ((t >> 7) & 1u) | ((t >> 14) & 2u) | ((t >> 21) & 4u) | ((t >> 28) & 8u); };
-      auto scan = [&](int64_t s, uint32_t& mk, uint32_t& wk) {
-        const int64_t r0 = s * SPAN + lane * RPL;
-        mk = wk = 0u;
-        if (r0 + RPL <= rows) {
-          mk = *reinterpret_cast<const uint32_t*>(gm + r0);
-          wk = *reinterpret_cast<const uint32_t*>(wr + r0);
-        } else {
-#pragma unroll
-          for (int k = 0; k < RPL; ++k)
-            if (r0 + k < rows) {
-              mk |= (uint32_t)gm[r0 + k] << (8 * k);
-              wk |= (uint32_t)wr[r0 + k] << (8 * k);
-            }
-        }
-      };
-      int64_t s = (int64_t)lblk * WAVES + wv;
+      const ColdTensor X = cold_tensor<PATH == OPT_MARK_ACC_U>(T);
+      const int64_t nspan = (X.rows + COLD_SPAN - 1) / COLD_SPAN, nwv = (int64_t)nblk * COLD_WAVES;
+      int64_t s = (int64_t)lblk * COLD_WAVES + wv;
       uint32_t mk = 0, wk = 0;
-      if (s < nspan) scan(s, mk, wk);
+      if (s < nspan) cold_scan(gm, wr, X.rows, s, lane, mk, wk);
       for (; s < nspan; s += nwv) {
         uint32_t mkn = 0, wkn = 0;
-        if (s + nwv < nspan) scan(s + nwv, mkn, wkn);
-        const uint32_t lm = pack4(nz80(mk)), wm = pack4(nz80(wk));
-        const uint32_t act = lm | wm;
-        if (__builtin_amdgcn_ballot_w64(act != 0) != 0) {
-          const int64_t row0 = s * SPAN;
-          const uint32_t cnt = (uint32_t)__builtin_popcount(act);
-          uint32_t pre = 0;
-          int nlive = 0;
-#pragma unroll
-          for (int bit = 0; (1 << bit) <= RPL; ++bit) {
-            const uint64_t bal = __builtin_amdgcn_ballot_w64(((cnt >> bit) & 1u) != 0);
-            pre += __builtin_amdgcn_mbcnt_hi((uint32_t)(bal >> 32), __builtin_amdgcn_mbcnt_lo((uint32_t)bal, 0u)) << bit;
-            nlive += __builtin_popcountll(bal) << bit;
-          }
-          const bool dense = nlive * 100 >= SPAN * DENSE_PCT;
-          if (!dense) {
-            __builtin_amdgcn_fence(__ATOMIC_RELEASE, "wavefront");
-            __builtin_amdgcn_wave_barrier();
-#pragma unroll
-            for (int k = 0; k < RPL; ++k)
-              if ((act >> k) & 1u)
-                lst[pre++] = (uint16_t)((lane * RPL + k) | (((lm >> k) & 1u) << 14) | (((wm >> k) & 1u) << 15));
-            __builtin_amdgcn_fence(__ATOMIC_RELEASE, "wavefront");
-            __builtin_amdgcn_wave_barrier();
-          }
-          if (lm) {
-            const int64_t r0 = row0 + lane * RPL;
-            if (r0 + RPL <= rows) {
-              *reinterpret_cast<uint32_t*>(gm + r0) = 0u;
-              const uint32_t set = (nz80(mk) & ~nz80(wk)) >> 7;
-              if (set) *reinterpret_cast<uint32_t*>(wr + r0) = wk | set;
-            } else {
-#pragma unroll
-              for (int k = 0; k < RPL; ++k)
-                if ((lm >> k) & 1u) {
-                  gm[r0 + k] = 0;
-                  if (!((wm >> k) & 1u)) wr[r0 + k] = 1;
-                }
-            }
-          }
-          const int items = (dense ? SPAN : nlive) << csh;
-#pragma unroll 1
-          for (int b0 = 0; b0 < items; b0 += 128) {
-            f4 p[2], a[2], b[2], g[2];
-            l2 t0[2], t1[2];
-            int64_t jj[2];
-            bool on[2], lv[2];
-#pragma unroll
-            for (int k = 0; k < 2; ++k) {
-              const int it = b0 + 64 * k + lane;
-              const int ent = it >> csh;
-              on[k] = it < items;
-              uint32_t e;
-              if (dense) {
-                const uint32_t src = (uint32_t)__shfl((int)(lm | (act << 16)), (ent / RPL) & 63);
-                on[k] = on[k] && ((src >> (16 + (ent & (RPL - 1)))) & 1u);
-                e = (uint32_t)ent | (((src >> (ent & (RPL - 1))) & 1u) << 14);
-              } else {
-                e = on[k] ? lst[ent] : 0u;
-              }
-              lv[k] = on[k] && ((e >> 14) & 1u);
-              const int64_t j = ((row0 + (int64_t)(e & 0x3fffu)) << csh) | (int64_t)(it & ((1 << csh) - 1));
-              jj[k] = j;
-              p[k] = a[k] = b[k] = g[k] = zero;
-              t0[k] = t1[k] = lzero;
-              if (on[k]) {
-                p[k] = ld(P + j);
-                if (S1) a[k] = ld(S1 + j);
-                if (S2) b[k] = ld(S2 + j);
-              }
-              if (lv[k]) {
-                if (!zg) g[k] = ld(G + j);
-                if (PATH == OPT_MARK_ACC_U && A64) {
-                  t0[k] = A64[2 * j];
-                  t1[k] = A64[2 * j + 1];
-                }
-              }
-            }
-#pragma unroll
-            for (int k = 0; k < 2; ++k) {
-              if (!on[k]) continue;
-              const int64_t j = jj[k];
-              f4 gs = g[k];
-              if (PATH == OPT_MARK_ACC_U && A64 && lv[k]) add_totals(gs, t0[k], t1[k], j);
-              one(p[k], gs, a[k], b[k]);
-              st(P + j, p[k]);
-              if (S1) st(S1 + j, a[k]);
-              if (S2) st(S2 + j, b[k]);
-              if (h.zero_grad && (g[k].x != 0.f || g[k].y != 0.f || g[k].z != 0.f || g[k].w != 0.f)) G[j] = zero;
-            }
-          }
-        }
+        if (s + nwv < nspan) cold_scan(gm, wr, X.rows, s + nwv, lane, mkn, wkn);
+        cold_span<PATH == OPT_MARK_ACC_U>(h, c, nt, X, s, lane, live_rows[wv], mk, wk);
         mk = mkn;
         wk = wkn;
       }
@@ -504,7 +630,8 @@
   for (int i = threadIdx.x; i < L.n; i += 256) ts[i] = L.t[i];
   for (int i = threadIdx.x; i <= L.n; i += 256) pre[i] = L.chunk0[i];
   const mml_opt_hyper& h = L.h;
-  const StepConsts c = step_consts(h);
+  __syncthreads();
+  const StepConsts c = step_consts(h, L.sc);
   const int64_t total = pre[L.n];
   const int64_t stride = (int64_t)gridDim.x * blockDim.x;
   for (int64_t ch = (int64_t)blockIdx.x * blockDim.x + threadIdx.x; ch < total; ch += stride) {
@@ -570,6 +697,7 @@
   int32_t cap;
   int32_t pad_;
   mml_opt_hyper h;
+  const mml_opt_step_consts* sc;
 };
 
 __device__ __forceinline__ int field_of_row(const int64_t* rb_lds, int F, int64_t grow) {
@@ -597,7 +725,8 @@
     tab_l[i] = L.tab[i]; grad_l[i] = L.grad[i]; s1_l[i] = L.s1[i]; s2_l[i] = L.s2[i]; seen_l[i] = L.seen[i];
     last_l[i] = L.last[i];
   }
-  const StepConsts c = step_consts(h);
+  __syncthreads();
+  const StepConsts c = step_consts(h, L.sc);
   int32_t cnt = *L.touched_count;
   if (cnt > L.cap) cnt = L.cap;
   const int per_row = L.E / VEC;
@@ -738,6 +867,18 @@
 
 __global__ void counter_kernel(int32_t* c, int32_t delta, int32_t reset) {
   if (threadIdx.x == 0 && blockIdx.x == 0) *c = reset ? 0 : (*c + delta);
+}
+
+__global__ void step_begin_kernel(int32_t* c, int32_t delta, const mml_opt_hyper h, mml_opt_step_consts* out) {
+  if (threadIdx.x == 0 && blockIdx.x == 0) {
+    const int t = *c + delta;
+    *c = t;
+    const StepConsts k = step_consts_of(h, t);
+    out->step_size = k.step_size;
+    out->inv_bc2s = k.inv_bc2s;
+    out->pad_ = 0;
+    out->step = t;
+  }
 }
 
 __global__ __launch_bounds__(256) void ew_mul_kernel(const float* a, const float* b, float* out, int64_t n) {
@@ -999,15 +1140,79 @@
   return MML_OK;
 }
 
+namespace {
+struct StepBinding {
+  const int32_t* step_dev;
+  const mml_opt_step_consts* consts;
+  int32_t kind;
+  float lr, beta1, beta2;
+};
+std::mutex g_step_mu;
+std::vector<StepBinding> g_step_bindings;
+
+void step_unbind(const int32_t* step_dev) {
+  std::lock_guard<std::mutex> lk(g_step_mu);
+  for (size_t i = 0; i < g_step_bindings.size(); ++i)
+    if (g_step_bindings[i].step_dev == step_dev) {
+      g_step_bindings[i] = g_step_bindings.back();
+      g_step_bindings.pop_back();
+      return;
+    }
+}
+
+const mml_opt_step_consts* step_bound(const mml_opt_hyper& h) {
+  if (!h.step_dev) return nullptr;
+  std::lock_guard<std::mutex> lk(g_step_mu);
+  for (const StepBinding& b : g_step_bindings)
+    if (b.step_dev == h.step_dev)
+      return (b.kind == h.kind && b.lr == h.lr && b.beta1 == h.beta1 && b.beta2 == h.beta2) ? b.consts : nullptr;
+  return nullptr;
+}
+
+int device_cus() {
+  static int cus = 0;
+  if (cus == 0) {
+    int dev = 0, nn = 0;
+    if (hipGetDevice(&dev) != hipSuccess ||
+        hipDeviceGetAttribute(&nn, hipDeviceAttributeMultiprocessorCount, dev) != hipSuccess || nn <= 0)
+      nn = 256;
+    cus = nn;
+  }
+  return cus;
+}
+}
+
+extern "C" int mml_opt_step_begin(int32_t* step_dev, int32_t delta, const mml_opt_hyper* hyper,
+                                  mml_opt_step_consts* consts, mml_stream_t stream) {
+  MML_REQUIRE(hyper, "mml_opt_step_begin: null hyper");
+  MML_REQUIRE(hyper->kind >= MML_OPT_SGD && hyper->kind <= MML_OPT_RMSPROP, "mml_opt_step_begin: unknown optimizer kind %d",
+              hyper->kind);
+  MML_REQUIRE(step_dev && consts && aligned16(consts), "mml_opt_step_begin: needs a counter and a 16-byte aligned buffer");
+  MML_LAUNCH(step_begin_kernel, dim3(1), dim3(64), 0, to_stream(stream), step_dev, delta, *hyper, consts);
+  const int rc = check_launch("mml_opt_step_begin");
+  if (rc) return rc;
+  step_unbind(step_dev);
+  std::lock_guard<std::mutex> lk(g_step_mu);
+  g_step_bindings.push_back(StepBinding{step_dev, consts, hyper->kind, hyper->lr, hyper->beta1, hyper->beta2});
+  return MML_OK;
+}
+
+extern "C" int mml_opt_step_unbind(const int32_t* step_dev) {
+  step_unbind(step_dev);
+  return MML_OK;
+}
+
 extern "C" int mml_opt_step_dense(const mml_opt_tensor* tensors, int32_t n, const mml_opt_hyper* hyper,
                                   mml_stream_t stream) {
   int rc = check_hyper(hyper, "mml_opt_step_dense");
   if (rc) return rc;
+  const mml_opt_step_consts* const bound = step_bound(*hyper);
   MML_REQUIRE(n >= 0 && (n == 0 || tensors), "mml_opt_step_dense: bad tensor array");
   int i = 0;
   while (i < n) {
     OptLaunch L{};
     L.h = *hyper;
+    L.sc = bound;
     int64_t total = 0, chunks = 0;
     while (i < n && L.n < MML_MAX_OPT_TENSORS) {
       const mml_opt_tensor& t = tensors[i];
@@ -1075,7 +1280,15 @@
         cold_wgs = e ? atoi(e) : 256 * 8;
         if (cold_wgs < 1 || cold_wgs > 256 * 8) cold_wgs = 256 * 8;
       }
-      const int64_t wg_cap = all_warm ? cold_wgs : 256 * 8;
+      bool resident = all_warm && all_gm && (any_acc || (L.variant & 4)) && (hyper->cold_loop == 0 || hyper->cold_loop == 3);
+      int64_t nspan = 0;
+      for (int k = 0; k < L.n && resident; ++k) {
+        const mml_opt_tensor& t = L.t[k];
+        resident = ((reinterpret_cast<uintptr_t>(t.grad_marks) | reinterpret_cast<uintptr_t>(t.warm_rows)) & 3) == 0;
+        nspan += cdiv(t.n / t.row_elems, COLD_SPAN);
+      }
+      resident = resident && nspan < ((int64_t)1 << 30);
+      const int64_t wg_cap = (all_warm && !resident) ? cold_wgs : 256 * 8;
       if (many) {
         int64_t want = 0;
         for (int k = 0; k < L.n; ++k) {
@@ -1097,6 +1310,25 @@
         L.blk0[L.n] = (int32_t)at;
         L.prop = 1;
         grid = dim3((unsigned)at, 1);
+      }
+      if (resident) {
+        int64_t wgs = (int64_t)grid.x * grid.y;
+        static int per_cu = -1;
+        if (per_cu < 0) {
+          const char* e = getenv("MMLREC_OPT_RESIDENT_PER_CU");
+          per_cu = e ? atoi(e) : 8;
+          if (per_cu < 1 || per_cu > 64) per_cu = 8;
+        }
+        const int64_t fit = (int64_t)(hyper->cold_loop == 3 ? 4 : per_cu) * device_cus();
+        if (wgs > fit) wgs = fit;
+        int64_t at = 0;
+        for (int k = 0; k < L.n; ++k) {
+          L.blk0[k] = (int32_t)at;
+          at += cdiv(L.t[k].n / L.t[k].row_elems, COLD_SPAN);
+        }
+        L.blk0[L.n] = (int32_t)at;
+        L.prop = 2;
+        grid = dim3((unsigned)(wgs < 1 ? 1 : wgs), 1);
       }
       static int u_mark = -1;
       if (u_mark < 0) {
@@ -1197,6 +1429,7 @@
   }
   L.rowbase[F] = rowbase[F];
   L.F = F; L.E = E; L.touched = touched; L.touched_count = touched_count; L.cap = touched_cap; L.h = *hyper;
+  L.sc = step_bound(*hyper);
   bool vec = (E % 4 == 0);
   for (int f = 0; f < F && vec; ++f)
     vec = aligned16(L.tab[f]) && aligned16(L.grad[f]) && (!L.s1[f] || aligned16(L.s1[f])) && (!L.s2[f] || aligned16(L.s2[f]));
@@ -1209,6 +1442,7 @@
 
 extern "C" int mml_counter_update(int32_t* counter, int32_t delta, int32_t reset, mml_stream_t stream) {
   MML_REQUIRE(counter, "mml_counter_update: null counter");
+  step_unbind(counter);
   MML_LAUNCH(counter_kernel, dim3(1), dim3(64), 0, to_stream(stream), counter, delta, reset);
   return check_launch("mml_counter_update");
 }
diff --git a/mmlrec-a-unified-multi-task-and-multi-scenario-learning-benchmark-for-recommendation_amd/ops.py b/mmlrec-a-unified-multi-task-and-multi-scenario-learning-benchmark-for-recommendation_amd/ops.py
--- a/mmlrec-a-unified-multi-task-and-multi-scenario-learning-benchmark-for-recommendation_amd/ops.py
+++ b/mmlrec-a-unified-multi-task-and-multi-scenario-learning-benchmark-for-recommendation_amd/ops.py
@@ -930,6 +930,20 @@
     L.check(L.load().mml_counter_update(counter.data_ptr(), int(delta), int(reset), _stream()), "mml_counter_update")
 
 
+def step_counter(device):
+    buf = torch.zeros(8, dtype=torch.int32, device=device)
+    return buf[:1], buf[4:8]
+
+
+def opt_step_begin(step_dev, hyper, consts, delta=1):
+    L.check(L.load().mml_opt_step_begin(step_dev.data_ptr(), int(delta), C.byref(hyper), consts.data_ptr(), _stream()),
+            "mml_opt_step_begin")
+
+
+def opt_step_unbind(step_dev):
+    L.check(L.load().mml_opt_step_unbind(step_dev.data_ptr()), "mml_opt_step_unbind")
+
+
 def auc_segments(pred, y, seg):
     lib = L.load()
     n, c = pred.shape
diff --git a/mmlrec-a-unified-multi-task-and-multi-scenario-learning-benchmark-for-recommendation_amd/optimizer.py b/mmlrec-a-unified-multi-task-and-multi-scenario-learning-benchmark-for-recommendation_amd/optimizer.py
--- a/mmlrec-a-unified-multi-task-and-multi-scenario-learning-benchmark-for-recommendation_amd/optimizer.py
+++ b/mmlrec-a-unified-multi-task-and-multi-scenario-learning-benchmark-for-recommendation_amd/optimizer.py
@@ -22,6 +22,8 @@
     scatter_old: bool = False
     cold_rows: bool = True
     cold_compact: bool = True
+    resident: int = 1
+    step_consts: bool = True
 
     @classmethod
     def from_env(cls, env=None):
@@ -36,7 +38,9 @@
                    variant=int(env.get("MMLREC_OPT_VARIANT", "0")),
                    scatter_old=bool(env.get("MMLREC_SCATTER_OLD")),
                    cold_rows=env.get("MMLREC_OPT_COLD_ROWS", "1") != "0",
-                   cold_compact=env.get("MMLREC_OPT_COLD_COMPACT", "1") != "0")
+                   cold_compact=env.get("MMLREC_OPT_COLD_COMPACT", "1") != "0",
+                   resident=int(env.get("MMLREC_OPT_RESIDENT", "1")),
+                   step_consts=env.get("MMLREC_OPT_STEP_CONSTS", "1") != "0")
 
 
 TABLE_UPDATES = ("dense_exact", "sparse_rows", "lazy_exact")
@@ -115,7 +119,15 @@
 
 
 def cold_loop_of(knobs):
-    return 0 if knobs.cold_compact else 1
+    if not knobs.cold_compact:
+        return 1
+    return {0: 2, 2: 3}.get(knobs.resident, 0)
+
+
+def step_pre_entry(lib, step_dev_ptr, consts_ptr, hyper):
+    if consts_ptr is None:
+        return (lib.mml_counter_update, (step_dev_ptr, 1, 0))
+    return (lib.mml_opt_step_begin, (step_dev_ptr, 1, C.byref(hyper), consts_ptr))
 
 
 class TableRows:
@@ -261,10 +273,16 @@
         self.last = None
         self.dirty = False
         dev = store.device
-        self.step_dev = torch.zeros(1, dtype=torch.int32, device=dev)
+        self.step_dev, self.step_consts = ops.step_counter(dev)
         self.state = _OptState(store, kind)
         self.warm = self.state.warm
         self.steps_done = 0
+
+    def __del__(self):
+        try:
+            ops.opt_step_unbind(self.step_dev)
+        except Exception:
+            pass
 
     def warm_map(self, name):
         self.state[name]
@@ -292,7 +310,10 @@
 
     def calls_split(self, plan, split_dense=False):
         knobs = OptKnobs.from_env()
-        pre = [(L.load().mml_counter_update, (self.step_dev.data_ptr(), 1, 0))]
+        hyper = ops.make_hyper(self.kind, self.lr, step=0, step_dev=self.step_dev, zero_grad=False)
+        plan.keep.append(hyper)
+        pre = [step_pre_entry(L.load(), self.step_dev.data_ptr(),
+                              self.step_consts.data_ptr() if knobs.step_consts else None, hyper)]
         if self.table_update == "lazy_exact":
             pre += self._lazy_pre_calls(plan)
         split_dense = bool(split_dense) and self.can_split_dense(plan)
@@ -304,8 +325,6 @@
         if treg and self.table_update != "dense_exact":
             raise NotImplementedError("l2_reg_embedding / l1 on the tables makes every row's gradient non-zero: use "
                                       "table_update='dense_exact' (the reference's own dense optimizer)")
-        hyper = ops.make_hyper(self.kind, self.lr, step=0, step_dev=self.step_dev, zero_grad=False)
-        plan.keep.append(hyper)
         mlp = self._mlp_calls(plan, reg, hyper)
         early, tables = [], []
         if names and self.table_update == "dense_exact":
```

New measurement: 62.34 million samples/s, median of 6. +3.3%, better.
